# ouyangjiahong/representation-disentanglement

Hardware: AMD Instinct MI355X
Metric: MR slices/sec (train step, recon+adv+latent losses) (higher is better)
Workload: dtype f32

## Files before the change

include/mrdis.h:

```cpp
#ifndef MRDIS_H
#define MRDIS_H

#include <stddef.h>
#include <stdint.h>

#ifdef __cplusplus
extern "C" {
#endif

#define MRDIS_OK            0
#define MRDIS_EINVAL       -1
#define MRDIS_EUNSUPPORTED -2
#define MRDIS_EWORKSPACE   -3
#define MRDIS_ELAUNCH      -4
#define MRDIS_EALIGN       -5

#define MRDIS_MAX_TAPS 16

#define MRDIS_EPI_NONE   0
#define MRDIS_EPI_LRELU  1

const char* mrdis_strerror(int code);
int mrdis_version(void);

// ... 177 lines not shown
int mrdis_synth_finish(float* acc, const int* cnt, float* out, int D, int H, int W, float fill, void* stream);

#define MRDIS_SEG2D_MAX_SETS 16
#define MRDIS_SEG2D_MAX_VIEWS 2
int mrdis_seg2d_label_planes(const float* const* views, int n_sets, int n_views, const int* flips, unsigned char* planes, int B, int C, int H,
                             int W, int D, int s0, int relabel, void* stream);
int mrdis_seg2d_finish(const unsigned char* planes, unsigned char* out, int n_sets, int D, int H, int W, void* stream);

#define MRDIS_FUSE_MAX_SRC 8
#define MRDIS_FUSE_MEAN 0
#define MRDIS_FUSE_MAX 1
#define MRDIS_FUSE_MEAN_MAX_MIN 2
int mrdis_fuse_present_fwd(const float* const* srcs, const int* ld_srcs, int K, const float* mask, int method, float* out, int ldo, int B,
                           long long HW, int C, void* stream);
int mrdis_fuse_present_bwd(const float* dout, int lddo, const float* const* srcs, const int* ld_srcs, int K, const float* mask, int method,
                           float* const* dsrcs, const int* ld_dsrcs, int B, long long HW, int C, void* stream);

#define MRDIS_EDT_FAR (1 << 30)
#define MRDIS_EDT_MAX_SRC 8
#define MRDIS_SURF_MAX_REGIONS 4
int mrdis_region_surfaces(const unsigned char* labels, const void* targets, const int* region_masks, int R, unsigned char* flags, int* counts,
                          int B, int H, int W, int D, void* stream);
size_t mrdis_edt_workspace(int S, int B, int H, int W, int D);
int mrdis_edt_sq(const unsigned char* src, const unsigned char* src_masks, int S, int* out, void* workspace, size_t workspace_bytes, int B,
                 int H, int W, int D, void* stream);
int mrdis_surface_hist(const unsigned char* flags, int R, int* hist, long long bins, void* workspace, size_t workspace_bytes, int B, int H,
                       int W, int D, void* stream);

int mrdis_cc_label(const unsigned char* labels, int fg_mask, int connectivity, int* comp, int* size, int B, int H, int W, int D, void* stream);
size_t mrdis_cc_clean_workspace(int B);
int mrdis_cc_clean(const unsigned char* labels, const int* comp, const int* size, int min_voxels, int keep_largest, int et_label,
                   int et_min_voxels, int et_replace, unsigned char* out, int* stats, void* workspace, size_t workspace_bytes, int B, int H,
                   int W, int D, void* stream);

#define MRDIS_DILATE_MAX_ITERATIONS 8
int mrdis_region_planes(const unsigned char* labels, const void* targets, const int* region_masks, int R, unsigned char* planes, int B, int H,
                        int W, int D, void* stream);
size_t mrdis_dilate_workspace(int iterations, int B, int H, int W, int D);
int mrdis_dilate(const unsigned char* src, unsigned char* dst, int connectivity, int iterations, void* workspace, size_t workspace_bytes, int B,
                 int H, int W, int D, void* stream);
int mrdis_lesion_match(const unsigned char* planes, const int* comp_l, const int* rank_l, const int* comp_p, const int* rank_p,
                       const int* first_p, int words, int n_lesions, int* bits, int* tcount, int* root, int* item, int B, int R, int H, int W,
                       int D, void* stream);
int mrdis_lesion_expand(const unsigned char* planes, const int* comp_l, const int* rank_l, const int* comp_p, const int* rank_p,
                        const int* first_p, const int* bits, int words, const int* item, int n_lesions, int j0, int n, unsigned char* stack_s,
                        unsigned char* stack_t, int B, int R, int H, int W, int D, void* stream);

int mrdis_maxpool_fwd(const float* x, int ldx, float* y, int32_t* argmax, int N, int H, int W, int C,
                      int k, void* stream);
int mrdis_maxpool_bwd(const float* dy, const int32_t* argmax, float* dx, int lddx, int N, int H, int W,
                      int C, int k, void* stream);

size_t mrdis_sumsq_workspace(void);
int mrdis_sumsq_finite(const float* g, long long n, float* out, void* workspace, size_t workspace_bytes,
                       void* stream);
int mrdis_adam_amsgrad_step(float* p, const float* g, float* m, float* v, float* vmax,
                            long long n, float lr, float beta1, float beta2, float eps,
                            float weight_decay, int step_count, float* step_state, const float* norm_finite,
                            float max_norm, float grad_scale, const long long* gate_ranges, const int* gate_flag_index,
                            int n_gates, const float* gate_flags, float* gate_steps, int n_flags, void* stream);


int mrdis_conv3d_fwd(const float* x, int ldx, const float* w_tck, const float* bias, const float* residual, int ldres,
                     float* y, int ldy, int N, int D, int H, int W, int Ci, int Co,
                     int k, int stride, int pad, void* stream);
int mrdis_conv3d_bwd_data(const float* dy, int lddy, const float* w_tkc, float* dx, int lddx,
                          int N, int D, int H, int W, int Ci, int Co, int k, int stride, int pad, void* stream);
size_t mrdis_conv3d_bwd_weight_workspace(int N, int D, int H, int W, int Ci, int Co, int k, int stride, int pad);
int mrdis_conv3d_bwd_weight(const float* x, int ldx, const float* dy, int lddy, float* dw_tck, float* dbias,
                            void* workspace, size_t workspace_bytes,
                            int N, int D, int H, int W, int Ci, int Co, int k, int stride, int pad, void* stream);

size_t mrdis_groupnorm_workspace(int N, long long P, int C, int G);
int mrdis_groupnorm_relu_fwd(const float* x, int ldx, float* y, int ldy, const float* gamma, const float* beta,
                             float* save_mean, float* save_rstd, void* workspace, size_t workspace_bytes,
                             int N, long long P, int C, int G, float eps, int relu, void* stream);
int mrdis_groupnorm_relu_bwd(const float* dy, int lddy, const float* x, int ldx, const float* gamma, const float* beta,
                             const float* save_mean, const float* save_rstd, float* dx, int lddx,
                             float* dgamma, float* dbeta, void* workspace, size_t workspace_bytes,
                             int N, long long P, int C, int G, int relu, void* stream);
int mrdis_groupnorm_relu_bwd_add(const float* dy, int lddy, const float* x, int ldx, const float* gamma, const float* beta,
                                 const float* save_mean, const float* save_rstd, float* dx, int lddx,
                                 float* dgamma, float* dbeta, const float* add, int ldadd, void* workspace, size_t workspace_bytes,
                                 int N, long long P, int C, int G, int relu, void* stream);

int mrdis_upsample2x_add_fwd(const float* x, const float* skip, float* y, int N, int D, int H, int W, int C, void* stream);
int mrdis_upsample2x_bwd(const float* dy, float* dx, int N, int D, int H, int W, int C, void* stream);

size_t mrdis_cosine_top1_workspace(int N, int D, int Q);
int mrdis_cosine_top1(const float* gallery, long long ldg, const int* gallery_label, int N, int D,
                      const float* query, const int* query_label, int Q,
                      int* out_idx, float* out_cos, void* workspace, size_t workspace_bytes, void* stream);

int mrdis_conv2d_2src_fwd(const float* x, int ldx, int Cx, const float* s, int lds, int Cs, const float* w_tck, const float* bias,
                          float* y, int ldy, int N, int H, int W, int Co, int kh, int kw, int stride, int pad, int lrelu, void* stream);
int mrdis_conv2d_2src_bwd_data(const float* dy, int lddy, const float* w_tkc, float* dx, int lddx, int Cx, float* ds, int ldds, int Cs,
                               int N, int H, int W, int Co, int kh, int kw, int stride, int pad, void* stream);
size_t mrdis_conv2d_2src_bwd_weight_workspace(int N, int H, int W, int Cx, int Cs, int Co, int kh, int kw, int stride, int pad);
int mrdis_conv2d_2src_bwd_weight(const float* x, int ldx, int Cx, const float* s, int lds, int Cs, const float* dy, int lddy,
                                 float* dw_tck, float* dbias, int accumulate_bias, void* workspace, size_t workspace_bytes,
                                 int N, int H, int W, int Co, int kh, int kw, int stride, int pad, void* stream);
int mrdis_softplus_fwd(const float* x, int ldx, float* y, int ldy, long long P, int C, void* stream);
int mrdis_softplus_bwd(const float* dy, int lddy, const float* x, int ldx, float* dx, int lddx, long long P, int C, void* stream);
int mrdis_softmax_fwd(const float* s, int lds, float* out, int ldo, long long P, int C, void* stream);
int mrdis_softmax_bwd(const float* dout, int lddo, const float* out, int ldo, float* ds, int ldds, long long P, int C, void* stream);

#define MRDIS_KL_MAXM 8
int mrdis_kl_fwd(const float* const* mu, const float* const* lv, int ldmu, int ldlv, const float* pmu, const float* plv, long long ldp_m,
                 int ldp_b, const float* weight, float* loss, int M, int B, int Z, void* stream);
int mrdis_kl_bwd(const float* dloss, const float* const* mu, const float* const* lv, int ldmu, int ldlv, const float* pmu, const float* plv,
                 long long ldp_m, int ldp_b, const float* weight, float* const* dmu, float* const* dlv, int lddmu, int lddlv,
                 float* dpmu, float* dplv, int M, int B, int Z, void* stream);
int mrdis_avgpool_fwd(const float* x, int ldx, float* y, int N, int H, int W, int C, int k, void* stream);
int mrdis_avgpool_bwd(const float* dy, float* dx, int lddx, int N, int H, int W, int C, int k, void* stream);

size_t mrdis_chatt_workspace(int B, long long HW, int C, int Hd);
int mrdis_chatt_fwd(const float* x, int ldx, const float* s, int lds, const float* wd, const float* bd, const float* wu, const float* bu,
                    float* out, int ldo, float* pool, float* hid, float* a, void* ws, size_t ws_bytes, int B, long long HW, int C, int Hd,
                    void* stream);
int mrdis_chatt_bwd(const float* dy, int lddy, const float* x, int ldx, const float* a, const float* hid, const float* pool,
                    const float* wd, const float* wu, float* dx, int lddx, float* dwd, float* dbd, float* dwu, float* dbu,
                    void* ws, size_t ws_bytes, int B, long long HW, int C, int Hd, void* stream);
int mrdis_symdiff_fwd(const float* g, int ldg, float* gd, int ldo, int B, int H, int W, int C, void* stream);
int mrdis_symdiff_bwd(const float* dgd, int lddgd, const float* g, int ldg, float* dg, int lddg, int B, int H, int W, int C, void* stream);
int mrdis_rgate_fwd(const float* x, int ldx, const float* alpha, float* out, int ldo, int B, int H, int W, int C, void* stream);
int mrdis_rgate_bwd(const float* dy, int lddy, const float* x, int ldx, const float* alpha, float* dx, int lddx, float* rsum,
                    int B, int H, int W, int C, void* stream);

#define MRDIS_PREP_U8 2
#define MRDIS_PREP_I16 4
#define MRDIS_PREP_I32 8
#define MRDIS_PREP_F32 16
#define MRDIS_PREP_F64 64
#define MRDIS_PREP_U16 512
#define MRDIS_PREP_ZSCORE 0
#define MRDIS_PREP_MEAN 1
#define MRDIS_PREP_LABEL 2
#define MRDIS_PREP_DHW 0
#define MRDIS_PREP_HWD 1
size_t mrdis_prep_workspace(int H, int W, int D);
int mrdis_prep_stats(const void* raw, int dtype, long long stride_h, long long stride_w, long long stride_d, int H, int W, int D,
                     int h0, int h1, int w0, int w1, int d_lo, int d_hi, double slope, double inter, double* stats,
                     void* workspace, size_t workspace_bytes, void* stream);
int mrdis_prep_write(const void* raw, int dtype, long long stride_h, long long stride_w, long long stride_d, int H, int W, int D,
                     int h0, int h1, int w0, int w1, double slope, double inter, const double* stats, int kind, int layout,
                     float* out, void* stream);

#define MRDIS_EXPORT_COPY 0
#define MRDIS_EXPORT_UNZSCORE 1
#define MRDIS_EXPORT_UNMEAN 2
int mrdis_export_volume(const void* src, int src_dtype, int layout, int Hc, int Wc, int D, int h0, int h1, int w0, int w1, int B,
                        int kind, const double* stats, double fill, void* dst, int dst_dtype, void* stream);

#ifdef __cplusplus
}
#endif
#endif
```

representation-disentanglement_amd/__init__.py:

```python
from . import hip, ops, model, model3d, trainer
from .hip import MrdisError, MrdisLibraryError, LIB_PATH
from .model import (CondConv2d, Conv2d, HipConv2d, BatchNorm2d, Conv_BN_Act_New,
                    Act_Deconv_BN_Concat_New, AnatomyEncoderEncNew, AnatomyEncoderDecNew,
                    ModalityEncoderNew, SPADEBlockNew, SPADENewShared, SPADENewNotShared, SPADENew,
                    Discriminator, MultimodalModel, expand_type)
from .trainer import (TrainStep, GraphedTrainStep, make_train_step, regular_mask, EvalStep, ZGallery, build_z_gallery, nn_source_contrast, ArenaAdam, GradAllReduce, DEFAULT_CONFIG, load_config_yaml,
                      derive_config, build_model, synthetic_batch, fit_to_model, forward_losses,
                      save_checkpoint, load_checkpoint_model, LOSS_KEYS)

from .model3d import BasicBlock, VAEBranch, UNet3D, NVNet3D, HipConv3d, nvnet_loss, nvnet_loss_hip, seg_metrics, seg_metrics_from_counts, window_offsets, predict_volumes
from .data import VolumeStore, SliceDataset, BatchLoader, load_idx_list
from .data3d import VolumeStore3D, VolumeDataset3D, VolumeLoader3D, VolumeData3D, load_subj_list
from . import patch3d
from .patch3d import fg_block_counts, fg_prefix, patch_origins, patch_gather, patch_warp, warp_matrix
from .synth import synthesize_volumes, synth_plan, synth_source, synth_targets, SYNTH_BLOCKS
from . import synth
from . import segment
from .segment import segment_volumes, seg_patterns
from . import surfdist
from .surfdist import EDT_FAR, BRATS_REGIONS, edt3d_sq, region_scores, scores_from_counts, percentile_ranks, region_masks
from . import postproc
from .postproc import components3d, clean_labels
from . import lesion
from .lesion import dilate3d, lesion_scores, lesion_scores_from_rows
from . import prep
from .prep import read_nifti, prep_stats, prep_write, prep_volume, build_store_from_raw, write_fold_lists, write_nifti, save_nifti, export_store_volume
from . import train
from . import train3d
from .train3d import Run3D

__version__ = '0.1.0'
```

representation-disentanglement_amd/csrc/mrdis_c16.hip:

```cpp
#include "mrdis_common.h"

struct C16Params {
    const float* x; const float* w; const float* bias; float* y;
    int N, H, W, Ci, ldx, ldy, lrelu;
    int tilesY, tilesX, ntiles;
    unsigned x_bytes;
};

namespace {
constexpr int C16_TH = 8, C16_TW = 32, C16_RW = C16_TW + 2, C16_NPX = (C16_TH + 2) * C16_RW;
constexpr unsigned C16_OOB = 0xfffffff0u;
}

template <int HALVES>
__global__ __launch_bounds__(256, 2) void conv3x3_c16_kernel(const C16Params p) {
    constexpr int CI = 16 * HALVES, PP = CI + 4, Q = CI / 4;
    constexpr int XR = (C16_NPX * Q + 255) / 256;
    constexpr int NG = 9 * HALVES;
    extern __shared__ __attribute__((aligned(16))) float smem[];
    const int tid = threadIdx.x, lane = tid & 63, wave = tid >> 6, l16 = lane & 15, kq = lane >> 4;

    float a[NG][4];
#pragma unroll
    for (int g = 0; g < NG; ++g)
#pragma unroll
        for (int j = 0; j < 4; ++j) a[g][j] = p.w[((g / HALVES) * CI + 16 * (g % HALVES) + 4 * kq + j) * 16 + l16];
    const float4 bv = p.bias ? make_float4(p.bias[4 * kq], p.bias[4 * kq + 1], p.bias[4 * kq + 2], p.bias[4 * kq + 3])
                              : make_float4(0.f, 0.f, 0.f, 0.f);

    const __amdgpu_buffer_rsrc_t rs_x = mrdis_buffer_rsrc(p.x, p.x_bytes);
    int s_l[XR], s_ry[XR], s_rx[XR], s_q[XR];
#pragma unroll
    for (int it = 0; it < XR; ++it) {
        const int idx = tid + 256 * it, pi = idx / Q;
        s_q[it] = 4 * (idx - pi * Q);
        s_ry[it] = pi / C16_RW; s_rx[it] = pi - s_ry[it] * C16_RW;
        s_l[it] = idx < C16_NPX * Q ? pi * PP + s_q[it] : -1;
    }
    u32x4 xr[XR];
    auto load_tile = [&](int tile) {
        const bool on = tile < p.ntiles;
        int t = tile;
        const int tx = t % p.tilesX; t /= p.tilesX;
        const int ty = t % p.tilesY;
        const int n = t / p.tilesY;
#pragma unroll
        for (int it = 0; it < XR; ++it) {
            const int h = ty * C16_TH - 1 + s_ry[it], w_ = tx * C16_TW - 1 + s_rx[it];
            const bool ok = on && s_l[it] >= 0 && (unsigned)h < (unsigned)p.H && (unsigned)w_ < (unsigned)p.W;
            xr[it] = __builtin_amdgcn_raw_buffer_load_b128(rs_x, (int)(ok ? 4u * (unsigned)(((n * p.H + h) * p.W + w_) * p.ldx + s_q[it]) : C16_OOB), 0, 0);
        }
    };
    auto store_tile = [&]() {
#pragma unroll
        for (int it = 0; it < XR; ++it)
            if (s_l[it] >= 0) *reinterpret_cast<u32x4*>(smem + s_l[it]) = xr[it];
    };

    int boff[4];
#pragma unroll
    for (int t = 0; t < 4; ++t) boff[t] = ((2 * wave + (t >> 1)) * C16_RW + 16 * (t & 1) + l16) * PP + 4 * kq;

    int tile = mrdis_xcd_remap((int)blockIdx.x, (int)gridDim.x);
    load_tile(tile);
    store_tile();
    __syncthreads();
    for (; tile < p.ntiles; tile += gridDim.x) {
        load_tile(tile + gridDim.x);
        f32x4 acc[4];
#pragma unroll
        for (int t = 0; t < 4; ++t) acc[t] = f32x4{0.f, 0.f, 0.f, 0.f};
        float4 b[2][4];
#pragma unroll
        for (int t = 0; t < 4; ++t) b[0][t] = *reinterpret_cast<const float4*>(smem + boff[t]);
#pragma unroll
        for (int g = 0; g < NG; ++g) {
            if (g + 1 < NG) {
                const int tap = (g + 1) / HALVES, h = (g + 1) % HALVES;
                const int go = ((tap / 3) * C16_RW + (tap % 3)) * PP + 16 * h;
#pragma unroll
                for (int t = 0; t < 4; ++t) b[(g + 1) & 1][t] = *reinterpret_cast<const float4*>(smem + boff[t] + go);
            }
#pragma unroll
            for (int t = 0; t < 4; ++t) {
                const float4 v = b[g & 1][t];
                acc[t] = __builtin_amdgcn_mfma_f32_16x16x4f32(a[g][0], v.x, acc[t], 0, 0, 0);
            }
#pragma unroll
            for (int t = 0; t < 4; ++t) acc[t] = __builtin_amdgcn_mfma_f32_16x16x4f32(a[g][1], b[g & 1][t].y, acc[t], 0, 0, 0);
#pragma unroll
            for (int t = 0; t < 4; ++t) acc[t] = __builtin_amdgcn_mfma_f32_16x16x4f32(a[g][2], b[g & 1][t].z, acc[t], 0, 0, 0);
#pragma unroll
            for (int t = 0; t < 4; ++t) acc[t] = __builtin_amdgcn_mfma_f32_16x16x4f32(a[g][3], b[g & 1][t].w, acc[t], 0, 0, 0);
            __builtin_amdgcn_sched_barrier(0);
        }
        {
            int t_ = tile;
            const int tx = t_ % p.tilesX; t_ /= p.tilesX;
            const int ty = t_ % p.tilesY;
            const int n = t_ / p.tilesY;
#pragma unroll
            for (int t = 0; t < 4; ++t) {
                const int oy = ty * C16_TH + 2 * wave + (t >> 1), ox = tx * C16_TW + 16 * (t & 1) + l16;
                float4 o = make_float4(acc[t][0] + bv.x, acc[t][1] + bv.y, acc[t][2] + bv.z, acc[t][3] + bv.w);
                if (p.lrelu) { o.x = o.x > 0.f ? o.x : 0.2f * o.x; o.y = o.y > 0.f ? o.y : 0.2f * o.y; o.z = o.z > 0.f ? o.z : 0.2f * o.z; o.w = o.w > 0.f ? o.w : 0.2f * o.w; }
                if (oy < p.H && ox < p.W) *reinterpret_cast<float4*>(p.y + ((long long)(n * p.H + oy) * p.W + ox) * p.ldy + 4 * kq) = o;
            }
        }
        __syncthreads();
        store_tile();
        __syncthreads();
    }
}

__global__ __launch_bounds__(256, 2) void conv3x3_c16_split6_kernel(const C16Params p) {
    constexpr int CI = 32, Q = CI / 4, PB = 208;
    constexpr int XR = (C16_NPX * Q + 255) / 256;
    extern __shared__ __attribute__((aligned(16))) unsigned char smem_b[];
    const int tid = threadIdx.x, lane = tid & 63, wave = tid >> 6, l16 = lane & 15, kq = lane >> 4;

    bf16x8 a[9][3];
#pragma unroll
    for (int g = 0; g < 9; ++g)
#pragma unroll
        for (int j = 0; j < 8; ++j) {
            const float v = p.w[(g * CI + 8 * kq + j) * 16 + l16];
            mrdis_split3(v, a[g][0], a[g][1], a[g][2], j);
        }
    const float4 bv = p.bias ? make_float4(p.bias[4 * kq], p.bias[4 * kq + 1], p.bias[4 * kq + 2], p.bias[4 * kq + 3]) : make_float4(0.f, 0.f, 0.f, 0.f);

    const __amdgpu_buffer_rsrc_t rs_x = mrdis_buffer_rsrc(p.x, p.x_bytes);
    int s_l[XR], s_ry[XR], s_rx[XR], s_q[XR];
#pragma unroll
    for (int it = 0; it < XR; ++it) {
        const int idx = tid + 256 * it, pi = idx / Q;
        s_q[it] = 4 * (idx - pi * Q);
        s_ry[it] = pi / C16_RW; s_rx[it] = pi - s_ry[it] * C16_RW;
        s_l[it] = idx < C16_NPX * Q ? pi * PB + 2 * s_q[it] : -1;
    }
    u32x4 xr[XR];
    auto load_tile = [&](int tile) {
        const bool on = tile < p.ntiles;
        int t = tile;
        const int tx = t % p.tilesX; t /= p.tilesX;
        const int ty = t % p.tilesY;
        const int n = t / p.tilesY;
#pragma unroll
        for (int it = 0; it < XR; ++it) {
            const int h = ty * C16_TH - 1 + s_ry[it], w_ = tx * C16_TW - 1 + s_rx[it];
            const bool ok = on && s_l[it] >= 0 && (unsigned)h < (unsigned)p.H && (unsigned)w_ < (unsigned)p.W;
            xr[it] = __builtin_amdgcn_raw_buffer_load_b128(rs_x, (int)(ok ? 4u * (unsigned)(((n * p.H + h) * p.W + w_) * p.ldx + s_q[it]) : C16_OOB), 0, 0);
        }
    };
    auto store_tile = [&]() {
#pragma unroll
        for (int it = 0; it < XR; ++it) {
            if (s_l[it] < 0) continue;
            const float xv[4] = {__uint_as_float(xr[it].x), __uint_as_float(xr[it].y), __uint_as_float(xr[it].z), __uint_as_float(xr[it].w)};
            bf16x4 hi, mid, lo; mrdis_split3(xv, hi, mid, lo);
            *reinterpret_cast<bf16x4*>(smem_b + s_l[it]) = hi;
            *reinterpret_cast<bf16x4*>(smem_b + s_l[it] + 64) = mid;
            *reinterpret_cast<bf16x4*>(smem_b + s_l[it] + 128) = lo;
        }
    };

    int boff[4];
#pragma unroll
    for (int t = 0; t < 4; ++t) boff[t] = ((2 * wave + (t >> 1)) * C16_RW + 16 * (t & 1) + l16) * PB + 16 * kq;

    int tile = mrdis_xcd_remap((int)blockIdx.x, (int)gridDim.x);
    load_tile(tile);
    store_tile();
    __syncthreads();
    for (; tile < p.ntiles; tile += gridDim.x) {
        load_tile(tile + gridDim.x);
        f32x4 acc[4];
#pragma unroll
        for (int t = 0; t < 4; ++t) acc[t] = f32x4{0.f, 0.f, 0.f, 0.f};
#pragma unroll
        for (int g = 0; g < 9; ++g) {
            const int go = ((g / 3) * C16_RW + (g % 3)) * PB;
            bf16x8 xh[4], xm[4], xl[4];
#pragma unroll
            for (int t = 0; t < 4; ++t) {
                xh[t] = *reinterpret_cast<const bf16x8*>(smem_b + boff[t] + go);
                xm[t] = *reinterpret_cast<const bf16x8*>(smem_b + boff[t] + go + 64);
                xl[t] = *reinterpret_cast<const bf16x8*>(smem_b + boff[t] + go + 128);
            }
#pragma unroll
            for (int t = 0; t < 4; ++t) acc[t] = __builtin_amdgcn_mfma_f32_16x16x32_bf16(a[g][1], xm[t], acc[t], 0, 0, 0);
#pragma unroll
            for (int t = 0; t < 4; ++t) acc[t] = __builtin_amdgcn_mfma_f32_16x16x32_bf16(a[g][0], xl[t], acc[t], 0, 0, 0);
#pragma unroll
            for (int t = 0; t < 4; ++t) acc[t] = __builtin_amdgcn_mfma_f32_16x16x32_bf16(a[g][2], xh[t], acc[t], 0, 0, 0);
#pragma unroll
            for (int t = 0; t < 4; ++t) acc[t] = __builtin_amdgcn_mfma_f32_16x16x32_bf16(a[g][0], xm[t], acc[t], 0, 0, 0);
#pragma unroll
            for (int t = 0; t < 4; ++t) acc[t] = __builtin_amdgcn_mfma_f32_16x16x32_bf16(a[g][1], xh[t], acc[t], 0, 0, 0);
#pragma unroll
            for (int t = 0; t < 4; ++t) acc[t] = __builtin_amdgcn_mfma_f32_16x16x32_bf16(a[g][0], xh[t], acc[t], 0, 0, 0);
        }
        {
            int t_ = tile;
            const int tx = t_ % p.tilesX; t_ /= p.tilesX;
            const int ty = t_ % p.tilesY;
            const int n = t_ / p.tilesY;
#pragma unroll
            for (int t = 0; t < 4; ++t) {
                const int oy = ty * C16_TH + 2 * wave + (t >> 1), ox = tx * C16_TW + 16 * (t & 1) + l16;
                float4 o = make_float4(acc[t][0] + bv.x, acc[t][1] + bv.y, acc[t][2] + bv.z, acc[t][3] + bv.w);
                if (p.lrelu) { o.x = o.x > 0.f ? o.x : 0.2f * o.x; o.y = o.y > 0.f ? o.y : 0.2f * o.y; o.z = o.z > 0.f ? o.z : 0.2f * o.z; o.w = o.w > 0.f ? o.w : 0.2f * o.w; }
                if (oy < p.H && ox < p.W) *reinterpret_cast<float4*>(p.y + ((long long)(n * p.H + oy) * p.W + ox) * p.ldy + 4 * kq) = o;
            }
        }
        __syncthreads();
        store_tile();
        __syncthreads();
    }
}

__global__ __launch_bounds__(256, 2) void conv3x3_c16t_split6_kernel(const C16Params p) {
    constexpr int CI = 16, Q = CI / 4, PB = 112;
    constexpr int XR = (C16_NPX * Q + 255) / 256;
    extern __shared__ __attribute__((aligned(16))) unsigned char smem_t[];
    const int tid = threadIdx.x, lane = tid & 63, wave = tid >> 6, e = lane & 31, half = lane >> 5;

    bf16x8 a[9][3];
#pragma unroll
    for (int g = 0; g < 9; ++g)
#pragma unroll
        for (int j = 0; j < 8; ++j) {
            const int gf = p.lrelu ? 8 - g : g;
            const float v = p.w[(gf * CI + 8 * half + j) * 32 + e];
            mrdis_split3(v, a[g][0], a[g][1], a[g][2], j);
        }
    const __amdgpu_buffer_rsrc_t rs_x = mrdis_buffer_rsrc(p.x, p.x_bytes);
    int s_l[XR], s_ry[XR], s_rx[XR], s_q[XR];
#pragma unroll
    for (int it = 0; it < XR; ++it) {
        const int idx = tid + 256 * it, pi = idx / Q;
        s_q[it] = 4 * (idx - pi * Q);
        s_ry[it] = pi / C16_RW; s_rx[it] = pi - s_ry[it] * C16_RW;
        s_l[it] = idx < C16_NPX * Q ? pi * PB + 2 * s_q[it] : -1;
    }
    u32x4 xr[XR];
    auto load_tile = [&](int tile) {
        const bool on = tile < p.ntiles;
        int t = tile;
        const int tx = t % p.tilesX; t /= p.tilesX;
        const int ty = t % p.tilesY;
        const int n = t / p.tilesY;
#pragma unroll
        for (int it = 0; it < XR; ++it) {
            const int h = ty * C16_TH - 1 + s_ry[it], w_ = tx * C16_TW - 1 + s_rx[it];
            const bool ok = on && s_l[it] >= 0 && (unsigned)h < (unsigned)p.H && (unsigned)w_ < (unsigned)p.W;
            xr[it] = __builtin_amdgcn_raw_buffer_load_b128(rs_x, (int)(ok ? 4u * (unsigned)(((n * p.H + h) * p.W + w_) * p.ldx + s_q[it]) : C16_OOB), 0, 0);
        }
    };
    auto store_tile = [&]() {
#pragma unroll
        for (int it = 0; it < XR; ++it) {
            if (s_l[it] < 0) continue;
            const float xv[4] = {__uint_as_float(xr[it].x), __uint_as_float(xr[it].y), __uint_as_float(xr[it].z), __uint_as_float(xr[it].w)};
            bf16x4 hi, mid, lo; mrdis_split3(xv, hi, mid, lo);
            *reinterpret_cast<bf16x4*>(smem_t + s_l[it]) = hi;
            *reinterpret_cast<bf16x4*>(smem_t + s_l[it] + 32) = mid;
            *reinterpret_cast<bf16x4*>(smem_t + s_l[it] + 64) = lo;
        }
    };
    int boff[2];
#pragma unroll
    for (int t = 0; t < 2; ++t) boff[t] = ((2 * wave + t) * C16_RW + e) * PB + 16 * half;

    int tile = mrdis_xcd_remap((int)blockIdx.x, (int)gridDim.x);
    load_tile(tile);
    store_tile();
    __syncthreads();
    for (; tile < p.ntiles; tile += gridDim.x) {
        load_tile(tile + gridDim.x);
        f32x16 acc[2];
#pragma unroll
        for (int t = 0; t < 2; ++t)
#pragma unroll
            for (int r = 0; r < 16; ++r) acc[t][r] = 0.f;
#pragma unroll
        for (int g = 0; g < 9; ++g) {
            const int go = ((g / 3) * C16_RW + (g % 3)) * PB;
            bf16x8 xh[2], xm[2], xl[2];
#pragma unroll
            for (int t = 0; t < 2; ++t) {
                xh[t] = *reinterpret_cast<const bf16x8*>(smem_t + boff[t] + go);
                xm[t] = *reinterpret_cast<const bf16x8*>(smem_t + boff[t] + go + 32);
                xl[t] = *reinterpret_cast<const bf16x8*>(smem_t + boff[t] + go + 64);
            }
#pragma unroll
            for (int t = 0; t < 2; ++t) acc[t] = __builtin_amdgcn_mfma_f32_32x32x16_bf16(a[g][1], xm[t], acc[t], 0, 0, 0);
#pragma unroll
            for (int t = 0; t < 2; ++t) acc[t] = __builtin_amdgcn_mfma_f32_32x32x16_bf16(a[g][0], xl[t], acc[t], 0, 0, 0);
#pragma unroll
            for (int t = 0; t < 2; ++t) acc[t] = __builtin_amdgcn_mfma_f32_32x32x16_bf16(a[g][2], xh[t], acc[t], 0, 0, 0);
#pragma unroll
            for (int t = 0; t < 2; ++t) acc[t] = __builtin_amdgcn_mfma_f32_32x32x16_bf16(a[g][0], xm[t], acc[t], 0, 0, 0);
#pragma unroll
            for (int t = 0; t < 2; ++t) acc[t] = __builtin_amdgcn_mfma_f32_32x32x16_bf16(a[g][1], xh[t], acc[t], 0, 0, 0);
#pragma unroll
            for (int t = 0; t < 2; ++t) acc[t] = __builtin_amdgcn_mfma_f32_32x32x16_bf16(a[g][0], xh[t], acc[t], 0, 0, 0);
        }
        {
            int t_ = tile;
            const int tx = t_ % p.tilesX; t_ /= p.tilesX;
            const int ty = t_ % p.tilesY;
            const int n = t_ / p.tilesY;
#pragma unroll
            for (int t = 0; t < 2; ++t) {
                const int oy = ty * C16_TH + 2 * wave + t, ox = tx * C16_TW + e;
                if (oy < p.H && ox < p.W) {
                    float* dst = p.y + ((long long)(n * p.H + oy) * p.W + ox) * p.ldy + 4 * half;
#pragma unroll
                    for (int g4 = 0; g4 < 4; ++g4)
                        *reinterpret_cast<float4*>(dst + 8 * g4) = make_float4(acc[t][4 * g4], acc[t][4 * g4 + 1], acc[t][4 * g4 + 2], acc[t][4 * g4 + 3]);
                }
            }
        }
        __syncthreads();
        store_tile();
        __syncthreads();
    }
}

int mrdis_run_c16t_split6(const float* x, int ldx, const float* w_t_ci_co, float* y, int ldy, int N, int H, int W, int flip, hipStream_t s) {
    if (ldx % 4 != 0 || ldy % 4 != 0 || ((((uintptr_t)x) | ((uintptr_t)y)) & 15) != 0) return MRDIS_EUNSUPPORTED;
    if ((long long)N * H * W < 65536 || mrdis_opt(MRDIS_OPT_NOW16)) return MRDIS_EUNSUPPORTED;
    if (mrdis_opt(MRDIS_OPT_SPLIT6) != 7) return MRDIS_EUNSUPPORTED;
    const long long xb = 4LL * (((long long)N * H * W - 1) * ldx + 16);
    if (xb >= 0x7fffffffLL) return MRDIS_EUNSUPPORTED;
    C16Params p{};
    p.x = x; p.w = w_t_ci_co; p.bias = nullptr; p.y = y; p.N = N; p.H = H; p.W = W; p.Ci = 16; p.ldx = ldx; p.ldy = ldy; p.lrelu = flip;
    p.tilesY = mrdis_cdiv(H, C16_TH); p.tilesX = mrdis_cdiv(W, C16_TW);
    const long long nt = (long long)N * p.tilesY * p.tilesX;
    if (nt > 0x7fffffffLL) return MRDIS_EUNSUPPORTED;
    p.ntiles = (int)nt; p.x_bytes = (unsigned)xb;
    const int grid = p.ntiles < 512 ? p.ntiles : 512;
    MRDIS_LAUNCH(conv3x3_c16t_split6_kernel, dim3(grid), dim3(256), (size_t)C16_NPX * 112, s, p);
    MRDIS_CHECK_LAUNCH();
    return MRDIS_OK;
}

int mrdis_run_c16(const float* x, int ldx, const float* w_tck, const float* bias, float* y, int ldy, int N, int H, int W, int Ci, int Co,
                  int lrelu, hipStream_t s) {
    if (Co != 16 || (Ci != 16 && Ci != 32) || ldx % 4 != 0 || ldy % 4 != 0) return MRDIS_EUNSUPPORTED;
    if (((((uintptr_t)x) | ((uintptr_t)y)) & 15) != 0) return MRDIS_EUNSUPPORTED;
    if ((long long)N * H * W < 65536 || mrdis_opt(MRDIS_OPT_NOW16)) return MRDIS_EUNSUPPORTED;
    const long long xb = 4LL * (((long long)N * H * W - 1) * ldx + Ci);
    if (xb >= 0x7fffffffLL) return MRDIS_EUNSUPPORTED;
    C16Params p{};
    p.x = x; p.w = w_tck; p.bias = bias; p.y = y; p.N = N; p.H = H; p.W = W; p.Ci = Ci; p.ldx = ldx; p.ldy = ldy; p.lrelu = lrelu;
    p.tilesY = mrdis_cdiv(H, C16_TH); p.tilesX = mrdis_cdiv(W, C16_TW);
    const long long nt = (long long)N * p.tilesY * p.tilesX;
    if (nt > 0x7fffffffLL) return MRDIS_EUNSUPPORTED;
    p.ntiles = (int)nt; p.x_bytes = (unsigned)xb;
    const int grid = p.ntiles < 512 ? p.ntiles : 512;
    const size_t lds = sizeof(float) * (size_t)C16_NPX * (Ci + 4);
    if (Ci == 32 && (mrdis_opt(MRDIS_OPT_SPLIT6) == 1 || mrdis_opt(MRDIS_OPT_SPLIT6) == 5)) {
        if (!mrdis_lds_optin((const void*)conv3x3_c16_split6_kernel, 72 * 1024)) return MRDIS_ELAUNCH;
        mrdis_count(MRDIS_CNT_SPLIT6_C16);
        MRDIS_LAUNCH(conv3x3_c16_split6_kernel, dim3(grid), dim3(256), (size_t)C16_NPX * 208, s, p);
    } else
    if (Ci == 32) MRDIS_LAUNCH((conv3x3_c16_kernel<2>), dim3(grid), dim3(256), lds, s, p);
    else MRDIS_LAUNCH((conv3x3_c16_kernel<1>), dim3(grid), dim3(256), lds, s, p);
    MRDIS_CHECK_LAUNCH();
    return MRDIS_OK;
}
```

representation-disentanglement_amd/csrc/mrdis_common.h:

```cpp
#pragma once
#include <hip/hip_runtime.h>
#include <stdint.h>
#include "../../include/mrdis.h"
#include "mrdis_device.h"
#include "mrdis_launchers.h"

#define MRDIS_CHECK_LAUNCH()                                     \
    do {                                                         \
        hipError_t e_ = hipGetLastError();                       \
        if (e_ != hipSuccess) return MRDIS_ELAUNCH;              \
    } while (0)

#define MRDIS_OPTIONS(X) \
    X(WINO, "wino", "MRDIS_WINO", 0, 1)  \
    X(NT_MB, "nt_mb", "MRDIS_NT_MB", 0, 128)  \
    X(WINO_PIPE, "wino_pipe", "MRDIS_WINO_PIPE", 0, 1)  \
    X(WINO_U, "wino_u", "MRDIS_WINO_U", 0, 1)  \
    X(WINO4, "wino4", "MRDIS_WINO4", 0, 1)  \
    X(WINO4R, "wino4r", "MRDIS_WINO4R", 0, 1)  \
    X(BCONV4, "bconv4", "MRDIS_BCONV4", 0, 1)  \
    X(SPLIT6, "split6", "MRDIS_SPLIT6", 0, 1)  \
    X(NO16, "debug_no16", "MRDIS_DEBUG_NO16", 1, 0) \
    X(NOTHIN, "debug_nothin", "MRDIS_DEBUG_NOTHIN", 1, 0) \
    X(NOC4, "debug_noc4", "MRDIS_DEBUG_NOC4", 1, 0) \
    X(NODMA, "debug_nodma", "MRDIS_DEBUG_NODMA", 1, 0) \
    X(NO16_3D, "debug_no16_3d", "MRDIS_DEBUG_NO16_3D", 1, 0) \
    X(BILGEN, "debug_bilgen", "MRDIS_DEBUG_BILGEN", 1, 0) \
    X(NOW16, "debug_now16", "MRDIS_DEBUG_NOW16", 1, 0) \
    X(NOPACK, "debug_nopack", "MRDIS_DEBUG_NOPACK", 1, 0)  \
    X(MODE, "debug_mode", "MRDIS_DEBUG_MODE", 0, -1) \
    X(BN, "debug_bn", "MRDIS_DEBUG_BN", 0, -1) \
    X(KC, "debug_kc", "MRDIS_DEBUG_KC", 0, -1) \
    X(BM, "debug_bm", "MRDIS_DEBUG_BM", 0, -1) \
    X(C4_TW, "debug_c4_tw", "MRDIS_DEBUG_C4_TW", 0, -1) \
    X(WGSPLIT, "debug_wgsplit", "MRDIS_DEBUG_WGSPLIT", 0, -1) \
    X(BN3, "debug_bn3", "MRDIS_DEBUG_BN3", 0, -1) \
    X(KC3, "debug_kc3", "MRDIS_DEBUG_KC3", 0, -1) \
    X(C4_GRID, "c4_grid", "MRDIS_C4_GRID", 0, 0)  \
    X(C4_BLOCKS, "debug_c4_blocks", "MRDIS_DEBUG_C4_BLOCKS", 0, -1)  \
    X(ZS_GRID, "zsearch_grid", "MRDIS_ZSEARCH_GRID", 0, 0)  \
    X(VOLGEN, "debug_volgen", "MRDIS_DEBUG_VOLGEN", 1, 0)
#define MRDIS_X_OPT_ID(id, name, env, is_flag, dflt) MRDIS_OPT_##id,
enum { MRDIS_OPTIONS(MRDIS_X_OPT_ID) MRDIS_OPT_COUNT };
long long mrdis_opt(int id);
void mrdis_opt_note(int id, long long value);

#define MRDIS_COUNTERS(X) \
    X(WINO, "wino") X(WINO_SPADE, "wino_spade") X(WINO2, "wino2") X(WINO2_SPADE, "wino2_spade") X(WINO4, "wino4") X(WINO4_SPADE, "wino4_spade") X(WINO4N, "wino4n") \
    X(WINO4R, "wino4r") X(WINO_WGRAD, "wino_wgrad") X(WINO_WGRAD2, "wino_wgrad2") X(WINO4_WGRAD, "wino4_wgrad") X(BCONV3, "bconv3") X(BCONV3_SPADE, "bconv3_spade") \
    X(BCONV4, "bconv4") X(BCONV4_SPADE, "bconv4_spade") X(SPLIT6_C4, "split6_c4") X(SPLIT6_C16, "split6_c16") X(SPLIT6_WGRAD16, "split6_wgrad16") X(SPLIT6_CO4, "split6_co4") \
    X(SPLIT6_C3D, "split6_c3d") X(SPLIT6_W3D, "split6_w3d") X(SPLIT6_TAP, "split6_tap") X(ZSEARCH, "zsearch") \
    X(CONV2SRC, "conv2src") X(ANA_ACT, "ana_act")  \
    X(KL, "kl") X(AVGPOOL, "avgpool")  \
    X(CHATT, "chatt") X(SYMDIFF, "symdiff") X(RGATE, "rgate")  \
    X(DIRECT3D, "direct3d") X(C3D16, "c3d16") X(WGRAD3D, "wgrad3d") X(WGRAD3D16, "wgrad3d16") X(WINO_WGRAD3D, "wino_wgrad3d")  \
    X(VOLGATHER, "volgather")  \
    X(FGCOUNT, "fgcount") X(PATCHORIGIN, "patchorigin") X(PATCHGATHER, "patchgather")  \
    X(PATCHWARP, "patchwarp")  \
    X(LOSS3D, "loss3d") X(SEGCOUNTS, "segcounts")  \
    X(SEGACCUM, "segaccum") X(SEGLABELS, "seglabels")  \
    X(SYNTHACCUM, "synthaccum") X(SYNTHFINISH, "synthfinish")  \
    X(SEG2DLABELS, "seg2dlabels") X(SEG2DFINISH, "seg2dfinish")  \
    X(FUSE, "fuse")  \
    X(REGSURF, "regsurf") X(EDT, "edt") X(SURFHIST, "surfhist")  \
    X(CCLABEL, "cclabel") X(CCCLEAN, "ccclean")  \
    X(PREPSTATS, "prepstats") X(PREPWRITE, "prepwrite")  \
    X(EXPORT, "export")  \
    X(DILATE, "dilate") X(LESMATCH, "lesmatch") X(LESEXPAND, "lesexpand")  \
    X(STAT_VEC, "stat_vec") X(STAT_SCALAR, "stat_scalar") X(STAT_INTERP, "stat_interp")  \
    X(SPADE_UP2_ONEPASS, "spade_up2_onepass") X(SPADE_UP2_TWOPASS, "spade_up2_twopass")  \
    X(BIL_FWD_X2, "bil_fwd_x2") X(BIL_FWD_GENERAL, "bil_fwd_general")  \
    X(BIL_BWD_X2, "bil_bwd_x2") X(BIL_BWD_TIGHT3, "bil_bwd_tight3") X(BIL_BWD_TIGHT5, "bil_bwd_tight5") X(BIL_BWD_GENERAL, "bil_bwd_general")  \
    X(ELEM_V1, "elem_v1")  \
    X(ALL, "all")
#define MRDIS_X_CNT_ID(id, name) MRDIS_CNT_##id,
enum { MRDIS_COUNTERS(MRDIS_X_CNT_ID) MRDIS_CNT_COUNT };
void mrdis_count(int id);

void mrdis_note_lds(const char* kernel_expr, size_t bytes);
#define MRDIS_LAUNCH(kernel, grid, block, lds, s, ...) do { mrdis_count(MRDIS_CNT_ALL); if ((size_t)(lds) != 0) mrdis_note_lds(#kernel, (size_t)(lds)); hipLaunchKernelGGL(kernel, grid, block, lds, s, __VA_ARGS__); } while (0)

int mrdis_cu_count();
bool mrdis_lds_optin(const void* kernel, int bytes);
int mrdis_occupancy(const void* kernel, int block, size_t lds);

static inline int mrdis_cdiv(long long a, long long b) { return (int)((a + b - 1) / b); }

__device__ __forceinline__ int mrdis_xcd_remap(int bid, int nblk) {
    const int q = nblk >> 3, r = nblk & 7, xcd = bid & 7;
    const int base = (xcd < r) ? xcd * (q + 1) : r * (q + 1) + (xcd - r) * q;
    return base + (bid >> 3);
}

__device__ __forceinline__ float mrdis_wave_sum(float v) {
#pragma unroll
    for (int o = 32; o > 0; o >>= 1) v += __shfl_down(v, o, 64);
    return v;
}
__device__ __forceinline__ double mrdis_wave_sum_d(double v) {
#pragma unroll
    for (int o = 32; o > 0; o >>= 1) v += __shfl_down(v, o, 64);
    return v;
}
```

representation-disentanglement_amd/csrc/mrdis_launchers.h:

```cpp
#pragma once
#include <hip/hip_runtime.h>
#include <stddef.h>

int mrdis_run_wino(const float* x, int ldx, const float* w, const float* bias, float* y, int ldy,
                   int N, int H, int W, int Ci, int Co, int flip, int lrelu, hipStream_t s);
int mrdis_run_wino3d(const float* x, int ldx, const float* w, const float* bias, const float* res, int ldres, float* y, int ldy,
                     int N, int D, int H, int W, int Ci, int Co, int flip, hipStream_t s);
size_t mrdis_wino_wgrad_workspace(int N, int H, int W, int Ci, int Co);
int mrdis_run_wino_wgrad(const float* x, int ldx, const float* dy, int lddy, float* dw_tck, float* dbias, void* workspace,
                         size_t workspace_bytes, int N, int H, int W, int Ci, int Co, int accumulate_bias, hipStream_t s);
size_t mrdis_wino_wgrad3d_workspace(int N, int D, int H, int W, int Ci, int Co);
int mrdis_run_wino_wgrad3d(const float* x, int ldx, const float* dy, int lddy, float* dw_tck, float* dbias, void* workspace,
                           size_t workspace_bytes, int N, int D, int H, int W, int Ci, int Co, hipStream_t s);

int mrdis_run_wino2(const float* x, int ldx, const float* w, const float* bias, float* y, int ldy,
                    int N, int H, int W, int Ci, int Co, int flip, int lrelu, hipStream_t s, const float* u_img);
int mrdis_run_wino2_spade(const float* x, int ldx, const float* w, const float* bias, const float* z, int ldz, const float* mean, const float* rstd,
                          float* mix, int ldmix, float* gamma, int ldg, int N, int H, int W, int Ci, int C, hipStream_t s, const float* u_img);

int mrdis_run_wino4(const float* x, int ldx, const float* bias, float* y, int ldy, int N, int H, int W, int Ci, int Co, int lrelu,
                    hipStream_t s, const float* u_img);
int mrdis_run_wino4n(const float* x, int ldx, const float* bias, float* y, int ldy, int N, int H, int W, int Ci, int Co, int lrelu,
                     hipStream_t s, const float* u_img);
int mrdis_run_wino4_spade(const float* x, int ldx, const float* bias, const float* z, int ldz, const float* mean, const float* rstd,
                          float* mix, int ldmix, float* gamma, int ldg, int N, int H, int W, int Ci, int C, hipStream_t s, const float* u_img);

int mrdis_run_wino4r(const float* x, int ldx, const float* bias, float* y, int ldy, int N, int H, int W, int Ci, int Co, int lrelu,
                     hipStream_t s, const float* u_img);

size_t mrdis_bwgrad_workspace(int N, int H, int W, int Ci, int Co, int kh, int kw, int stride, int pad);
int mrdis_run_bwgrad(const void* x, int ldx, const void* dy, int lddy, float* dw_tck, float* dbias, void* workspace, size_t workspace_bytes,
                     int N, int H, int W, int Ci, int Co, int kh, int kw, int stride, int pad, int accumulate_bias, int dtype, hipStream_t s);

int mrdis_run_bconv3_spade(const void* x, int ldx, const void* w_bf16, const float* bias, const void* z, int ldz, const float* mean, const float* rstd,
                           void* mix, int ldmix, void* gamma, int ldg, int N, int H, int W, int Ci, int C, hipStream_t s);

int mrdis_run_bconv4_spade(const void* x, int ldx, const void* w_bf16, const float* bias, const void* z, int ldz, const float* mean, const float* rstd,
                           void* mix, int ldmix, void* gamma, int ldg, int N, int H, int W, int Ci, int C, hipStream_t s);

int mrdis_run_pw_fwd(const void* x, int ldx, const float* w_tck, const float* bias, float* y, int ldy, long long npix, int Ci, int Co, int lrelu, int x16_bf16, hipStream_t s);
int mrdis_run_pw_dgrad(const float* dy, int lddy, const float* w_tkc, void* dx, int lddx, long long npix, int Ci, int Co, int x16_bf16, hipStream_t s);
size_t mrdis_pw_wgrad_workspace(long long npix, int Ci, int Co, int x16_bf16);
int mrdis_run_pw_wgrad(const void* x, int ldx, const float* dy, int lddy, float* dw_tck, float* dbias, void* workspace, size_t workspace_bytes,
                       long long npix, int Ci, int Co, int accumulate_bias, int x16_bf16, hipStream_t s);

int mrdis_launch_slab_reduce(const float* slab, float* dw, int total, int Co, int nslab, const float* bslab, float* dbias, int accumulate_bias,
                             hipStream_t s);
int mrdis_run_conv_s2_fwd(const float* x, int ldx, const float* w_tck, const float* bias, float* y, int ldy, int N, int H, int W, int Ci, int Co,
                          int kh, int kw, int stride, int pad, int lrelu, hipStream_t s);
int mrdis_run_dgrad_s2(const float* dy, int lddy, const float* w_tkc, float* dx, int lddx, int N, int H, int W, int Ci, int Co,
                       int kh, int kw, int stride, int pad, hipStream_t s);
size_t mrdis_wgrad_s2_workspace(int N, int H, int W, int Ci, int Co, int kh, int kw, int stride, int pad);
int mrdis_run_wgrad_s2(const float* x, int ldx, const float* dy, int lddy, float* dw_tck, float* dbias, void* workspace, size_t workspace_bytes,
                       int N, int H, int W, int Ci, int Co, int kh, int kw, int stride, int pad, int accumulate_bias, hipStream_t s);
size_t mrdis_wgrad_c4_workspace(int N, int H, int W, int Ci, int Co);
int mrdis_run_wgrad_c4(const float* x, int ldx, const void* dy, int lddy, float* dw_tck, float* dbias, void* workspace, size_t workspace_bytes,
                       int N, int H, int W, int Ci, int Co, int accumulate_bias, int dy_bf16, hipStream_t s, int pad16 = 0);
size_t mrdis_wgrad_co4b_workspace(int N, int H, int W, int Ci, int Co);
int mrdis_run_wgrad_co4b(const void* x_bf16, int ldx, const float* dy, int lddy, float* dw_tck, float* dbias, void* workspace, size_t workspace_bytes,
                         int N, int H, int W, int Ci, int Co, int accumulate_bias, hipStream_t s, int pad16);

size_t mrdis_wgrad16_workspace(int N, int H, int W, int Ci, int Co);
int mrdis_run_wgrad16(const float* x, int ldx, const float* dy, int lddy, float* dw_tck, float* dbias, void* workspace,
                      size_t workspace_bytes, int N, int H, int W, int Ci, int Co, int accumulate_bias, hipStream_t s);
int mrdis_run_wgrad16_bf16(const void* x, int ldx, const void* dy, int lddy, float* dw_tck, float* dbias, void* workspace, size_t workspace_bytes,
                           int N, int H, int W, int Ci, int Co, int accumulate_bias, hipStream_t s);

int mrdis_run_co4(const void* x, int ldx, const float* w, const float* bias, float* y, int ldy, int N, int H, int W, int Ci, int Co, int flip, int lrelu, hipStream_t s,
                  int x_bf16 = 0, int wld = 4);

int mrdis_run_c16(const float* x, int ldx, const float* w_tck, const float* bias, float* y, int ldy, int N, int H, int W, int Ci, int Co, int lrelu, hipStream_t s);
int mrdis_run_c16t_split6(const float* x, int ldx, const float* w_t_ci_co, float* y, int ldy, int N, int H, int W, int flip, hipStream_t s);
```

representation-disentanglement_amd/csrc/mrdis_wgrad16.hip:

```cpp
#include "mrdis_common.h"
#include <stdlib.h>

struct Wgrad16Params {
    const float* x; const float* dy; float* slab; float* bias_slab;
    int N, H, W, Ci, ldx, Co, lddy;
    int tilesA, tilesB, numTiles, nCi, splits;
};

#define W16_TH 8
#define W16_TW 16
#define W16_RW (W16_TW + 2)
#define W16_NPX ((W16_TH + 2) * W16_RW)

template <int NS>
__global__ __launch_bounds__(256, 2) void wgrad16_kernel(const Wgrad16Params p) {
    constexpr int S = NS == 1 ? 16 : 48, QX = 4 * NS;
    constexpr int XR = (W16_NPX * QX + 255) / 256;
    extern __shared__ __attribute__((aligned(16))) float smem[];
    float* dys = smem;
    float* xs = smem + 2048;
    const int tid = threadIdx.x, lane = tid & 63, wave = tid >> 6, l16 = lane & 15, kq = lane >> 4;
    const int lb = mrdis_xcd_remap((int)blockIdx.x, (int)gridDim.x);
    const int ncol = p.nCi / NS;
    const int cic = lb % ncol, split = lb / ncol;
    const int c_lo = cic * 16 * NS;

    int loff[9];
#pragma unroll
    for (int t = 0; t < 9; ++t) loff[t] = ((t / 3) * W16_RW + (t % 3)) * S + l16;
    bool ci_ok[NS];
#pragma unroll
    for (int sl = 0; sl < NS; ++sl) ci_ok[sl] = (c_lo + 16 * sl + l16) < p.Ci;
    int tin[8];
#pragma unroll
    for (int g = 0; g < 8; ++g) {
        const int m = wave * 32 + g * 4 + kq;
        tin[g] = ((m / W16_TW) * W16_RW + (m % W16_TW)) * S;
    }
    int xl[XR], xc[XR];
#pragma unroll
    for (int it = 0; it < XR; ++it) {
        const int idx = tid + it * 256;
        xl[it] = -1; xc[it] = 0;
        if (idx < W16_NPX * QX) { const int pi = idx / QX, q = idx % QX; xl[it] = pi * S + 4 * q; xc[it] = ((pi / W16_RW) << 10) | (pi % W16_RW); }
    }
    const int qx = c_lo + (tid % QX) * 4;
    const bool qx_ok = qx < p.Ci;
    int yc[2];
#pragma unroll
    for (int it = 0; it < 2; ++it) { const int m = (tid + it * 256) >> 2; yc[it] = ((m / W16_TW) << 10) | (m % W16_TW); }
    const int qy = (tid & 3) * 4;
    const bool qy_ok = qy < p.Co;

    f32x4 acc[NS][9];
#pragma unroll
    for (int sl = 0; sl < NS; ++sl)
#pragma unroll
        for (int t = 0; t < 9; ++t) acc[sl][t] = f32x4{0.f, 0.f, 0.f, 0.f};
    float bsum = 0.f;
    float4 xr[XR], yr[2];
    auto load_box = [&](int box) {
        int tt = box;
        const int tb = tt % p.tilesB; tt /= p.tilesB;
        const int ta = tt % p.tilesA;
        const int n = tt / p.tilesA;
        const int a0 = ta * W16_TH, b0 = tb * W16_TW;
        const float* __restrict__ xn = p.x + (long long)n * p.H * p.W * p.ldx + qx;
#pragma unroll
        for (int it = 0; it < XR; ++it) {
            xr[it] = make_float4(0.f, 0.f, 0.f, 0.f);
            const int h = a0 - 1 + (xc[it] >> 10), w_ = b0 - 1 + (xc[it] & 1023);
            if (xl[it] >= 0 && qx_ok && (unsigned)h < (unsigned)p.H && (unsigned)w_ < (unsigned)p.W)
                xr[it] = *reinterpret_cast<const float4*>(xn + ((long long)h * p.W + w_) * p.ldx);
        }
        const float* __restrict__ dyn = p.dy + (long long)n * p.H * p.W * p.lddy + qy;
#pragma unroll
        for (int it = 0; it < 2; ++it) {
            yr[it] = make_float4(0.f, 0.f, 0.f, 0.f);
            const int a = a0 + (yc[it] >> 10), b = b0 + (yc[it] & 1023);
            if (qy_ok && a < p.H && b < p.W) yr[it] = *reinterpret_cast<const float4*>(dyn + ((long long)a * p.W + b) * p.lddy);
        }
    };
    auto store_box = [&]() {
#pragma unroll
        for (int it = 0; it < XR; ++it)
            if (xl[it] >= 0) *reinterpret_cast<float4*>(xs + xl[it]) = xr[it];
#pragma unroll
        for (int it = 0; it < 2; ++it) *reinterpret_cast<float4*>(dys + 4 * (tid + it * 256)) = yr[it];
    };

    int box = split;
    if (box < p.numTiles) load_box(box);
    store_box();
    __syncthreads();
    for (; box < p.numTiles; box += p.splits) {
        const int nxt = box + p.splits;
        if (nxt < p.numTiles) load_box(nxt);
#pragma unroll
        for (int g = 0; g < 8; ++g) {
            const float bv = dys[(wave * 32 + g * 4 + kq) * 16 + l16];
            bsum += bv;
            const float* xa = xs + tin[g];
#pragma unroll
            for (int sl = 0; sl < NS; ++sl) {
                float av[9];
#pragma unroll
                for (int t = 0; t < 9; ++t) av[t] = ci_ok[sl] ? xa[loff[t] + 16 * sl] : 0.f;
#pragma unroll
                for (int t = 0; t < 9; ++t) acc[sl][t] = __builtin_amdgcn_mfma_f32_16x16x4f32(av[t], bv, acc[sl][t], 0, 0, 0);
            }
        }
        if (nxt < p.numTiles) { __syncthreads(); store_box(); __syncthreads(); }
    }
    float* red = smem;
#pragma unroll
    for (int sl = 0; sl < NS; ++sl) {
        float* out = p.slab + (((long long)split * p.nCi + cic * NS + sl) * 9) * 256;
        __syncthreads();
#pragma unroll
        for (int t = 0; t < 9; ++t)
#pragma unroll
            for (int r = 0; r < 4; ++r) red[(wave * 9 + t) * 256 + (4 * kq + r) * 16 + l16] = acc[sl][t][r];
        __syncthreads();
        for (int i = tid; i < 9 * 256; i += 256)
            out[i] = (red[i] + red[9 * 256 + i]) + (red[2 * 9 * 256 + i] + red[3 * 9 * 256 + i]);
    }
    if (p.bias_slab != nullptr && cic == 0) {
        bsum += __shfl_xor(bsum, 16, 64);
        bsum += __shfl_xor(bsum, 32, 64);
        __syncthreads();
        if (kq == 0) red[wave * 16 + l16] = bsum;
        __syncthreads();
        if (tid < 16) p.bias_slab[(long long)split * 16 + tid] = (red[tid] + red[16 + tid]) + (red[32 + tid] + red[48 + tid]);
    }
}

struct Wgrad16SParams {
    const float* x; const float* dy; float* slab; float* bias_slab;
    int N, H, W, ldx, lddy;
    int tilesA, tilesB, numTiles, splits;
    unsigned x_bytes, dy_bytes;
};
#define W6_TH 8
#define W6_TW 32
#define W6_YW (W6_TW + 2)
#define W6_YPX ((W6_TH + 2) * W6_YW)
__global__ __launch_bounds__(256, 2) void wgrad16_split6_kernel(const Wgrad16SParams p) {
    constexpr int XPX = W6_TH * W6_TW;
    constexpr int XPLANE = XPX * 64, YPLANE = W6_YPX * 32;
    constexpr int XR = 8, YR = 6;
    constexpr unsigned OOB = 0xfffffff0u;
    extern __shared__ __attribute__((aligned(16))) unsigned char smem6[];
    unsigned char* xs = smem6;
    unsigned char* ys = smem6 + 3 * XPLANE;
    const int tid = threadIdx.x, lane = tid & 63, wave = tid >> 6, l16 = lane & 15, kq = lane >> 4;
    const int split = mrdis_xcd_remap((int)blockIdx.x, (int)gridDim.x);
    const __amdgpu_buffer_rsrc_t rs_x = mrdis_buffer_rsrc(p.x, p.x_bytes);
    const __amdgpu_buffer_rsrc_t rs_y = mrdis_buffer_rsrc(p.dy, p.dy_bytes);

    const int q4 = l16 >> 2, p4 = l16 & 3;
    const int xoff = (8 * kq + q4) * 64 + 8 * p4;
    const int yoff = (8 * kq + q4) * 32 + 8 * p4;

    f32x4 acc[9][2];
#pragma unroll
    for (int t = 0; t < 9; ++t) { acc[t][0] = f32x4{0.f, 0.f, 0.f, 0.f}; acc[t][1] = f32x4{0.f, 0.f, 0.f, 0.f}; }
    float bs4[4] = {0.f, 0.f, 0.f, 0.f};

    u32x4 xr[XR], yr[YR];
    auto load_box = [&](int box) {
        const bool on = box < p.numTiles;
        int tt = box;
        const int tb = tt % p.tilesB; tt /= p.tilesB;
        const int ta = tt % p.tilesA;
        const int n = tt / p.tilesA;
        const int a0 = ta * W6_TH, b0 = tb * W6_TW;
#pragma unroll
        for (int it = 0; it < XR; ++it) {
            const int idx = tid + 256 * it, px = idx >> 3, q = idx & 7;
            const int h = a0 + (px >> 5), w_ = b0 + (px & 31);
            const bool ok = on && h < p.H && w_ < p.W;
            xr[it] = __builtin_amdgcn_raw_buffer_load_b128(rs_x, (int)(ok ? 4u * (unsigned)(((n * p.H + h) * p.W + w_) * p.ldx + 4 * q) : OOB), 0, 0);
        }
#pragma unroll
        for (int it = 0; it < YR; ++it) {
            const int idx = tid + 256 * it, px = idx >> 2, q = idx & 3;
            const int ly = px / W6_YW, lx = px - ly * W6_YW;
            const int h = a0 - 1 + ly, w_ = b0 - 1 + lx;
            const bool ok = on && px < W6_YPX && (unsigned)h < (unsigned)p.H && (unsigned)w_ < (unsigned)p.W;
            yr[it] = __builtin_amdgcn_raw_buffer_load_b128(rs_y, (int)(ok ? 4u * (unsigned)(((n * p.H + h) * p.W + w_) * p.lddy + 4 * q) : OOB), 0, 0);
        }
    };
    auto split4 = [](const u32x4& v, bf16x4& hi, bf16x4& mid, bf16x4& lo) {
        const float f[4] = {__uint_as_float(v.x), __uint_as_float(v.y), __uint_as_float(v.z), __uint_as_float(v.w)};
        mrdis_split3(f, hi, mid, lo);
    };
    auto store_box = [&]() {
#pragma unroll
        for (int it = 0; it < XR; ++it) {
            const int idx = tid + 256 * it, px = idx >> 3, q = idx & 7;
            bf16x4 hi, mid, lo; split4(xr[it], hi, mid, lo);
            unsigned char* d = xs + px * 64 + 8 * q;
            *reinterpret_cast<bf16x4*>(d) = hi; *reinterpret_cast<bf16x4*>(d + XPLANE) = mid; *reinterpret_cast<bf16x4*>(d + 2 * XPLANE) = lo;
        }
#pragma unroll
        for (int it = 0; it < YR; ++it) {
            const int idx = tid + 256 * it, px = idx >> 2, q = idx & 3;
            if (px >= W6_YPX) continue;
            const int ly = px / W6_YW, lx = px - ly * W6_YW;
            if (ly >= 1 && ly <= W6_TH && lx >= 1 && lx <= W6_TW) {
                bs4[0] += __uint_as_float(yr[it].x); bs4[1] += __uint_as_float(yr[it].y); bs4[2] += __uint_as_float(yr[it].z); bs4[3] += __uint_as_float(yr[it].w);
            }
            bf16x4 hi, mid, lo; split4(yr[it], hi, mid, lo);
            unsigned char* d = ys + px * 32 + 8 * q;
            *reinterpret_cast<bf16x4*>(d) = hi; *reinterpret_cast<bf16x4*>(d + YPLANE) = mid; *reinterpret_cast<bf16x4*>(d + 2 * YPLANE) = lo;
        }
    };
    int box = split;
    load_box(box);
    store_box();
    __syncthreads();
    for (; box < p.numTiles; box += p.splits) {
        load_box(box + p.splits);
#pragma unroll
        for (int rr = 0; rr < 2; ++rr) {
            const int row = wave + 4 * rr;
            bf16x8 ax[2][3];
#pragma unroll
            for (int mt = 0; mt < 2; ++mt)
#pragma unroll
                for (int term = 0; term < 3; ++term) {
                    const unsigned char* a = xs + term * XPLANE + row * (32 * 64) + xoff + 32 * mt;
                    union { bf16x8 v; s16x4 h[2]; } u;
                    u.h[0] = __builtin_amdgcn_ds_read_tr16_b64_v4i16((s16x4 __attribute__((address_space(3)))*)(a));
                    u.h[1] = __builtin_amdgcn_ds_read_tr16_b64_v4i16((s16x4 __attribute__((address_space(3)))*)(a + 4 * 64));
                    ax[mt][term] = u.v;
                }
#pragma unroll
            for (int t = 0; t < 9; ++t) {
                const int ty = t / 3, tx = t % 3;
                bf16x8 by[3];
#pragma unroll
                for (int term = 0; term < 3; ++term) {
                    const unsigned char* b = ys + term * YPLANE + ((row - ty + 2) * W6_YW + 2 - tx) * 32 + yoff;
                    union { bf16x8 v; s16x4 h[2]; } u;
                    u.h[0] = __builtin_amdgcn_ds_read_tr16_b64_v4i16((s16x4 __attribute__((address_space(3)))*)(b));
                    u.h[1] = __builtin_amdgcn_ds_read_tr16_b64_v4i16((s16x4 __attribute__((address_space(3)))*)(b + 4 * 32));
                    by[term] = u.v;
                }
#pragma unroll
                for (int mt = 0; mt < 2; ++mt) {
                    acc[t][mt] = __builtin_amdgcn_mfma_f32_16x16x32_bf16(ax[mt][1], by[1], acc[t][mt], 0, 0, 0);
                    acc[t][mt] = __builtin_amdgcn_mfma_f32_16x16x32_bf16(ax[mt][2], by[0], acc[t][mt], 0, 0, 0);
                    acc[t][mt] = __builtin_amdgcn_mfma_f32_16x16x32_bf16(ax[mt][0], by[2], acc[t][mt], 0, 0, 0);
                }
#pragma unroll
                for (int mt = 0; mt < 2; ++mt) {
                    acc[t][mt] = __builtin_amdgcn_mfma_f32_16x16x32_bf16(ax[mt][1], by[0], acc[t][mt], 0, 0, 0);
                    acc[t][mt] = __builtin_amdgcn_mfma_f32_16x16x32_bf16(ax[mt][0], by[1], acc[t][mt], 0, 0, 0);
                    acc[t][mt] = __builtin_amdgcn_mfma_f32_16x16x32_bf16(ax[mt][0], by[0], acc[t][mt], 0, 0, 0);
                }
            }
        }
        __syncthreads();
        store_box();
        __syncthreads();
    }
    float* red = reinterpret_cast<float*>(smem6);
#pragma unroll
    for (int mt = 0; mt < 2; ++mt) {
        float* out = p.slab + (((long long)split * 2 + mt) * 9) * 256;
        __syncthreads();
#pragma unroll
        for (int t = 0; t < 9; ++t)
#pragma unroll
            for (int r = 0; r < 4; ++r) red[(wave * 9 + t) * 256 + (4 * kq + r) * 16 + l16] = acc[t][mt][r];
        __syncthreads();
        for (int i = tid; i < 9 * 256; i += 256)
            out[i] = (red[i] + red[9 * 256 + i]) + (red[2 * 9 * 256 + i] + red[3 * 9 * 256 + i]);
    }
    if (p.bias_slab != nullptr) {
        __syncthreads();
#pragma unroll
        for (int c = 0; c < 4; ++c) red[c * 256 + tid] = bs4[c];
        __syncthreads();
        if (tid < 16) {
            const int qd = tid >> 2, c = tid & 3;
            float t_ = 0.f;
            for (int k = qd; k < 256; k += 4) t_ += red[c * 256 + k];
            p.bias_slab[(long long)split * 16 + tid] = t_;
        }
    }
}

__global__ __launch_bounds__(256, 2) void wgrad16_bf16_kernel(const Wgrad16SParams p) {
    constexpr int XPX = W6_TH * W6_TW;
    constexpr int XR = 4, YR = 3;
    constexpr unsigned OOB = 0xfffffff0u;
    extern __shared__ __attribute__((aligned(16))) unsigned char smem7[];
    unsigned char* xs = smem7;
    unsigned char* ys = smem7 + XPX * 64;
    const int tid = threadIdx.x, lane = tid & 63, wave = tid >> 6, l16 = lane & 15, kq = lane >> 4;
    const int split = mrdis_xcd_remap((int)blockIdx.x, (int)gridDim.x);
    const __amdgpu_buffer_rsrc_t rs_x = mrdis_buffer_rsrc(p.x, p.x_bytes);
    const __amdgpu_buffer_rsrc_t rs_y = mrdis_buffer_rsrc(p.dy, p.dy_bytes);
    const int q4 = l16 >> 2, p4 = l16 & 3;
    const int xoff = (8 * kq + q4) * 64 + 8 * p4;
    const int yoff = (8 * kq + q4) * 32 + 8 * p4;

    f32x4 acc[9][2];
#pragma unroll
    for (int t = 0; t < 9; ++t) { acc[t][0] = f32x4{0.f, 0.f, 0.f, 0.f}; acc[t][1] = f32x4{0.f, 0.f, 0.f, 0.f}; }
    float bs8[8] = {0.f, 0.f, 0.f, 0.f, 0.f, 0.f, 0.f, 0.f};

    u32x4 xr[XR], yr[YR];
    auto load_box = [&](int box) {
        const bool on = box < p.numTiles;
        int tt = box;
        const int tb = tt % p.tilesB; tt /= p.tilesB;
        const int ta = tt % p.tilesA;
        const int n = tt / p.tilesA;
        const int a0 = ta * W6_TH, b0 = tb * W6_TW;
#pragma unroll
        for (int it = 0; it < XR; ++it) {
            const int idx = tid + 256 * it, px = idx >> 2, q = idx & 3;
            const int h = a0 + (px >> 5), w_ = b0 + (px & 31);
            const bool ok = on && h < p.H && w_ < p.W;
            xr[it] = __builtin_amdgcn_raw_buffer_load_b128(rs_x, (int)(ok ? 2u * (unsigned)(((n * p.H + h) * p.W + w_) * p.ldx + 8 * q) : OOB), 0, 0);
        }
#pragma unroll
        for (int it = 0; it < YR; ++it) {
            const int idx = tid + 256 * it, px = idx >> 1, q = idx & 1;
            const int ly = px / W6_YW, lx = px - ly * W6_YW;
            const int h = a0 - 1 + ly, w_ = b0 - 1 + lx;
            const bool ok = on && px < W6_YPX && (unsigned)h < (unsigned)p.H && (unsigned)w_ < (unsigned)p.W;
            yr[it] = __builtin_amdgcn_raw_buffer_load_b128(rs_y, (int)(ok ? 2u * (unsigned)(((n * p.H + h) * p.W + w_) * p.lddy + 8 * q) : OOB), 0, 0);
        }
    };
    auto store_box = [&]() {
#pragma unroll
        for (int it = 0; it < XR; ++it) {
            const int idx = tid + 256 * it, px = idx >> 2, q = idx & 3;
            *reinterpret_cast<u32x4*>(xs + px * 64 + 16 * q) = xr[it];
        }
#pragma unroll
        for (int it = 0; it < YR; ++it) {
            const int idx = tid + 256 * it, px = idx >> 1, q = idx & 1;
            if (px >= W6_YPX) continue;
            const int ly = px / W6_YW, lx = px - ly * W6_YW;
            if (ly >= 1 && ly <= W6_TH && lx >= 1 && lx <= W6_TW) {
                const unsigned u[4] = {yr[it].x, yr[it].y, yr[it].z, yr[it].w};
#pragma unroll
                for (int k = 0; k < 4; ++k) { bs8[2 * k] += __uint_as_float(u[k] << 16); bs8[2 * k + 1] += __uint_as_float(u[k] & 0xffff0000u); }
            }
            *reinterpret_cast<u32x4*>(ys + px * 32 + 16 * q) = yr[it];
        }
    };

    int box = split;
    load_box(box);
    store_box();
    __syncthreads();
    for (; box < p.numTiles; box += p.splits) {
        load_box(box + p.splits);
#pragma unroll
        for (int rr = 0; rr < 2; ++rr) {
            const int row = wave + 4 * rr;
            bf16x8 ax[2];
#pragma unroll
            for (int mt = 0; mt < 2; ++mt) {
                const unsigned char* a = xs + row * (32 * 64) + xoff + 32 * mt;
                union { bf16x8 v; s16x4 h[2]; } u;
                u.h[0] = __builtin_amdgcn_ds_read_tr16_b64_v4i16((s16x4 __attribute__((address_space(3)))*)(a));
                u.h[1] = __builtin_amdgcn_ds_read_tr16_b64_v4i16((s16x4 __attribute__((address_space(3)))*)(a + 4 * 64));
                ax[mt] = u.v;
            }
#pragma unroll
            for (int t = 0; t < 9; ++t) {
                const int ty = t / 3, tx = t % 3;
                const unsigned char* b = ys + ((row - ty + 2) * W6_YW + 2 - tx) * 32 + yoff;
                union { bf16x8 v; s16x4 h[2]; } u;
                u.h[0] = __builtin_amdgcn_ds_read_tr16_b64_v4i16((s16x4 __attribute__((address_space(3)))*)(b));
                u.h[1] = __builtin_amdgcn_ds_read_tr16_b64_v4i16((s16x4 __attribute__((address_space(3)))*)(b + 4 * 32));
                acc[t][0] = __builtin_amdgcn_mfma_f32_16x16x32_bf16(ax[0], u.v, acc[t][0], 0, 0, 0);
                acc[t][1] = __builtin_amdgcn_mfma_f32_16x16x32_bf16(ax[1], u.v, acc[t][1], 0, 0, 0);
            }
        }
        __syncthreads();
        store_box();
        __syncthreads();
    }
    float* red = reinterpret_cast<float*>(smem7);
#pragma unroll
    for (int mt = 0; mt < 2; ++mt) {
        float* out = p.slab + (((long long)split * 2 + mt) * 9) * 256;
        __syncthreads();
#pragma unroll
        for (int t = 0; t < 9; ++t)
#pragma unroll
            for (int r = 0; r < 4; ++r) red[(wave * 9 + t) * 256 + (4 * kq + r) * 16 + l16] = acc[t][mt][r];
        __syncthreads();
        for (int i = tid; i < 9 * 256; i += 256)
            out[i] = (red[i] + red[9 * 256 + i]) + (red[2 * 9 * 256 + i] + red[3 * 9 * 256 + i]);
    }
    if (p.bias_slab != nullptr) {
        __syncthreads();
#pragma unroll
        for (int c = 0; c < 8; ++c) red[c * 256 + tid] = bs8[c];
        __syncthreads();
        if (tid < 16) {
            const int hf = tid >> 3, c = tid & 7;
            float t_ = 0.f;
            for (int k = hf; k < 256; k += 2) t_ += red[c * 256 + k];
            p.bias_slab[(long long)split * 16 + tid] = t_;
        }
    }
}

__global__ void wgrad16_reduce_kernel(const float* __restrict__ slab, float* __restrict__ dw, int Ci, int Co, int nCi, int nslab,
                                      const float* __restrict__ bslab, float* __restrict__ dbias, int accumulate_bias) {
    __shared__ float red[16][65];
    const int total = 9 * Ci * Co;
    const int nout = total + (dbias != nullptr ? Co : 0);
    const int i = blockIdx.x * 64 + threadIdx.x;
    const int SL = blockDim.y, y = threadIdx.y;
    float s_ = 0.f;
    if (i < total) {
        const int co = i % Co;
        const int r = i / Co;
        const int ci = r % Ci, t = r / Ci;
        const long long stride = (long long)nCi * 9 * 256;
        const float* src = slab + ((long long)(ci >> 4) * 9 + t) * 256 + (ci & 15) * 16 + co + (long long)y * stride;
        for (int k = y; k < nslab; k += SL, src += (long long)SL * stride) s_ += *src;
    } else if (i < nout) {
        const int co = i - total;
        for (int k = y; k < nslab; k += SL) s_ += bslab[(long long)k * 16 + co];
    }
    red[y][threadIdx.x] = s_;
    __syncthreads();
    if (y == 0 && i < nout) {
        float t = 0.f;
        for (int k = 0; k < SL; ++k) t += red[k][threadIdx.x];
        if (i < total) dw[i] = t;
        else { const int co = i - total; dbias[co] = accumulate_bias ? dbias[co] + t : t; }
    }
}

static bool plan_wgrad16(Wgrad16Params& p, int N, int H, int W, int Ci, int Co) {
    if (Co > 16 || Co <= 4 || Co % 4 != 0 || Ci % 16 != 0) return false;
    if ((long long)N * H * W < 100000 || mrdis_opt(MRDIS_OPT_NOW16)) return false;
    p = Wgrad16Params{};
    p.N = N; p.H = H; p.W = W; p.Ci = Ci; p.Co = Co;
    p.tilesA = mrdis_cdiv(H, W16_TH); p.tilesB = mrdis_cdiv(W, W16_TW);
    const long long nt = (long long)N * p.tilesA * p.tilesB;
    if (nt > 0x7fffffffLL) return false;
    p.numTiles = (int)nt;
    p.nCi = Ci / 16;
    int splits = 1024 / p.nCi;
    if (splits > p.numTiles) splits = p.numTiles;
    if (splits < 1) splits = 1;
    p.splits = splits;
    return true;
}

size_t mrdis_wgrad16_workspace(int N, int H, int W, int Ci, int Co) {
    Wgrad16Params p;
    if (!plan_wgrad16(p, N, H, W, Ci, Co)) return 0;
    return sizeof(float) * ((size_t)p.splits * p.nCi * 9 * 256 + (size_t)p.splits * 16) + 256;
}

int mrdis_run_wgrad16(const float* x, int ldx, const float* dy, int lddy, float* dw_tck, float* dbias, void* workspace,
                      size_t workspace_bytes, int N, int H, int W, int Ci, int Co, int accumulate_bias, hipStream_t s) {
    Wgrad16Params p;
    if (!plan_wgrad16(p, N, H, W, Ci, Co)) return MRDIS_EUNSUPPORTED;
    if (ldx % 4 != 0 || lddy % 4 != 0 || ((((uintptr_t)x) | ((uintptr_t)dy)) & 15) != 0) return MRDIS_EUNSUPPORTED;
    if (workspace_bytes + 256 < mrdis_wgrad16_workspace(N, H, W, Ci, Co)) return MRDIS_EUNSUPPORTED;
    p.x = x; p.dy = dy; p.ldx = ldx; p.lddy = lddy;
    p.slab = reinterpret_cast<float*>(workspace);
    p.bias_slab = dbias ? p.slab + (size_t)p.splits * p.nCi * 9 * 256 : nullptr;
    if (Ci == 32 && Co == 16 && (mrdis_opt(MRDIS_OPT_SPLIT6) == 1 || mrdis_opt(MRDIS_OPT_SPLIT6) == 6)) {
        const long long xb = 4LL * (((long long)N * H * W - 1) * ldx + Ci), yb = 4LL * (((long long)N * H * W - 1) * lddy + Co);
        if (xb < 0x7fffffffLL && yb < 0x7fffffffLL) {
            Wgrad16SParams q{};
            q.x = x; q.dy = dy; q.slab = p.slab; q.bias_slab = p.bias_slab; q.N = N; q.H = H; q.W = W; q.ldx = ldx; q.lddy = lddy;
            q.tilesA = mrdis_cdiv(H, W6_TH); q.tilesB = mrdis_cdiv(W, W6_TW);
            const long long nt6 = (long long)N * q.tilesA * q.tilesB;
            q.numTiles = (int)nt6; q.splits = p.splits < q.numTiles ? p.splits : q.numTiles;
            q.x_bytes = (unsigned)xb; q.dy_bytes = (unsigned)yb;
            const size_t lds6 = 3 * (size_t)(W6_TH * W6_TW * 64) + 3 * (size_t)(W6_YPX * 32);
            if (!mrdis_lds_optin((const void*)wgrad16_split6_kernel, 96 * 1024)) return MRDIS_ELAUNCH;
            mrdis_count(MRDIS_CNT_SPLIT6_WGRAD16);
            MRDIS_LAUNCH(wgrad16_split6_kernel, dim3(q.splits), dim3(256), lds6, s, q);
            MRDIS_CHECK_LAUNCH();
            const long long nout6 = 9LL * Ci * Co + (dbias ? Co : 0);
            int SL6 = 1;
            while (SL6 < 16 && SL6 * 8 <= q.splits) SL6 <<= 1;
            MRDIS_LAUNCH(wgrad16_reduce_kernel, dim3(mrdis_cdiv(nout6, 64)), dim3(64, SL6), 0, s, p.slab, dw_tck, Ci, Co, 2, q.splits, p.bias_slab, dbias, accumulate_bias);
            MRDIS_CHECK_LAUNCH();
            return MRDIS_OK;
        }
    }
    const size_t lds = sizeof(float) * (size_t)(4 * 9 * 256);
    MRDIS_LAUNCH(wgrad16_kernel<1>, dim3(p.splits * p.nCi), dim3(256), lds, s, p);
    MRDIS_CHECK_LAUNCH();
    const long long nout = 9LL * Ci * Co + (dbias ? Co : 0);
    int SL = 1;
    while (SL < 16 && SL * 8 <= p.splits) SL <<= 1;
    MRDIS_LAUNCH(wgrad16_reduce_kernel, dim3(mrdis_cdiv(nout, 64)), dim3(64, SL), 0, s, p.slab, dw_tck, Ci, Co, p.nCi, p.splits,
                       p.bias_slab, dbias, accumulate_bias);
    MRDIS_CHECK_LAUNCH();
    return MRDIS_OK;
}

int mrdis_run_wgrad16_bf16(const void* x, int ldx, const void* dy, int lddy, float* dw_tck, float* dbias, void* workspace, size_t workspace_bytes,
                           int N, int H, int W, int Ci, int Co, int accumulate_bias, hipStream_t s) {
    Wgrad16Params p;
    if (Ci != 32 || Co != 16 || !plan_wgrad16(p, N, H, W, Ci, Co) || mrdis_opt(MRDIS_OPT_MODE) == 3030) return MRDIS_EUNSUPPORTED;
    if (ldx % 8 != 0 || lddy % 8 != 0 || ((((uintptr_t)x) | ((uintptr_t)dy)) & 15) != 0) return MRDIS_EUNSUPPORTED;
    if (workspace_bytes + 256 < mrdis_wgrad16_workspace(N, H, W, Ci, Co)) return MRDIS_EUNSUPPORTED;
    const long long xb = 2LL * (((long long)N * H * W - 1) * ldx + Ci), yb = 2LL * (((long long)N * H * W - 1) * lddy + Co);
    if (xb >= 0x7fffffffLL || yb >= 0x7fffffffLL) return MRDIS_EUNSUPPORTED;
    Wgrad16SParams q{};
    q.x = reinterpret_cast<const float*>(x); q.dy = reinterpret_cast<const float*>(dy);
    q.slab = reinterpret_cast<float*>(workspace); q.bias_slab = dbias ? q.slab + (size_t)p.splits * p.nCi * 9 * 256 : nullptr;
    q.N = N; q.H = H; q.W = W; q.ldx = ldx; q.lddy = lddy;
    q.tilesA = mrdis_cdiv(H, W6_TH); q.tilesB = mrdis_cdiv(W, W6_TW);
    const long long nt = (long long)N * q.tilesA * q.tilesB;
    q.numTiles = (int)nt; q.splits = p.splits < q.numTiles ? p.splits : q.numTiles;
    q.x_bytes = (unsigned)xb; q.dy_bytes = (unsigned)yb;
    size_t lds = (size_t)(W6_TH * W6_TW * 64) + (size_t)(W6_YPX * 32);
    const size_t red = sizeof(float) * (size_t)(4 * 9 * 256);
    if (lds < red) lds = red;
    MRDIS_LAUNCH(wgrad16_bf16_kernel, dim3(q.splits), dim3(256), lds, s, q);
    MRDIS_CHECK_LAUNCH();
    const long long nout = 9LL * Ci * Co + (dbias ? Co : 0);
    int SL = 1;
    while (SL < 16 && SL * 8 <= q.splits) SL <<= 1;
    MRDIS_LAUNCH(wgrad16_reduce_kernel, dim3(mrdis_cdiv(nout, 64)), dim3(64, SL), 0, s, q.slab, dw_tck, Ci, Co, 2, q.splits, q.bias_slab, dbias, accumulate_bias);
    MRDIS_CHECK_LAUNCH();
    return MRDIS_OK;
}
```

representation-disentanglement_amd/hip.py:

```python
import collections
import ctypes
import os

import torch

_HERE = os.path.dirname(os.path.abspath(__file__))
LIB_PATH = os.path.join(_HERE, 'csrc', 'libmrdis_hip.so')


class MrdisLibraryError(RuntimeError):
    pass


class MrdisError(RuntimeError):
    pass


_lib = None
_c = ctypes
_P, _I, _L, _F, _Z = _c.c_void_p, _c.c_int, _c.c_longlong, _c.c_float, _c.c_size_t

_SIGS = {
    'mrdis_strerror': (_c.c_char_p, [_I]),
    'mrdis_version': (_I, []),
    'mrdis_set_option': (_I, [_c.c_char_p, _L]),
    'mrdis_get_option': (_L, [_c.c_char_p]),
    'mrdis_launch_count': (_L, [_c.c_char_p]),
    'mrdis_launch_count_reset': (None, []),
    'mrdis_dynamic_lds_table': (_I, [_c.c_char_p, _I]),
    'mrdis_mix_experts_fwd': (_I, [_P, _P, _P, _P, _I, _I, _I, _I, _P]),
    'mrdis_mix_experts_bwd_workspace': (_Z, [_I, _I, _I, _I]),
    'mrdis_mix_experts_bwd': (_I, [_P, _P, _P, _P, _P, _P, _Z, _I, _I, _I, _I, _P]),
    'mrdis_mix_experts_routed_fwd': (_I, [_P, _P, _P, _P, _I, _P, _P, _P, _I, _I, _I, _I, _P]),
    'mrdis_mix_experts_routed_bwd': (_I, [_P, _P, _P, _P, _I, _P, _P, _P, _P, _Z, _I, _I, _I, _I, _P]),
    'mrdis_copy_bytes': (_I, [_P, _P, _L, _P]),
    'mrdis_stream_fill': (_I, [_P, _L, _F, _P]),
    'mrdis_instnorm_stats': (_I, [_P, _I, _P, _P, _P, _Z, _I, _L, _I, _F, _I, _P]),
    'mrdis_conv2d_fwd_spade': (_I, [_P, _I, _P, _P, _P, _P, _I, _P, _P, _P, _I, _P, _I, _I, _I, _I, _I, _I, _I, _P, _I, _P]),
    'mrdis_wino_u_job_bytes': (_Z, []),
    'mrdis_wino_u_format': (_I, [_I, _I, _I]),
    'mrdis_wino_u_image_floats': (_L, [_I, _I, _I]),
    'mrdis_s6_filter_image_bytes': (ctypes.c_size_t, [_I, _I, _I]),
    'mrdis_s6_filter_image': (_I, [_P, _I, _I, _I, _P, ctypes.c_size_t, _P]),
    'mrdis_wino_u_image_floats_fmt': (_L, [_I, _I, _I, _I]),
    'mrdis_wino_u_job_blocks': (_I, [_I, _I, _I]),
    'mrdis_wino_u_jobs': (_I, [_P, _I, _I, _P]),
    'mrdis_mix_experts_routed_multi_fwd': (_I, [_P, _P, _P, _P, _I, _I, _P, _P, _P, _P, _P, _I, _L, _I, _I, _I, _I, _P]),
    'mrdis_mix_experts_routed_multi_bwd_workspace': (_Z, [_I, _I, _I, _I, _I]),
    'mrdis_mix_experts_routed_multi_bwd': (_I, [_P, _P, _P, _P, _I, _I, _P, _P, _P, _I, _I, _P, _Z, _I, _I, _I, _I, _P]),
    'mrdis_mix_job_bytes': (_Z, []),
    'mrdis_mix_job_blocks': (_I, [_I, _I, _I]),
    'mrdis_mix_jobs_fwd': (_I, [_P, _I, _I, _P, _I, _I, _P]),
    'mrdis_mix_jobs_bwd': (_I, [_P, _I, _I, _P, _P, _I, _I, _P]),
    'mrdis_conv2d_fwd': (_I, [_P, _I, _P, _P, _P, _P, _I] + [_I] * 11 + [_P, _I, _P]),
    'mrdis_conv2d_bwd_data': (_I, [_P, _I, _P, _P, _P, _I] + [_I] * 10 + [_P, _I, _P]),
    'mrdis_cast_bf16': (_I, [_P, _P, _L, _P]),
    'mrdis_cast_view': (_I, [_P, _I, _I, _I, _P, _I, _I, _I, _L, _P]),
    'mrdis_conv2d_bwd_weight_workspace': (_Z, [_I] * 9),
    'mrdis_conv2d_bwd_weight': (_I, [_P, _I, _P, _I, _P, _P, _P, _Z] + [_I] * 11 + [_P]),
    'mrdis_lrelu_bwd': (_I, [_P, _I, _P, _I, _P, _I, _L, _I, _F, _I, _P]),
    'mrdis_norm_workspace': (_Z, [_I, _L, _I]),
    'mrdis_bn_train_fwd': (_I, [_P, _I, _P, _I, _P, _P, _P, _P, _P, _P, _P, _Z, _L, _I, _F, _F, _I, _I, _P]),
    'mrdis_bn_eval_fwd': (_I, [_P, _I, _P, _I, _P, _P, _P, _P, _L, _I, _F, _I, _P]),
    'mrdis_bn_train_bwd': (_I, [_P, _I, _P, _I, _P, _P, _P, _P, _I, _P, _P, _P, _P, _P, _Z, _L, _I, _I, _I, _P]),
    'mrdis_instnorm_spade_fwd': (_I, [_P, _I, _P, _I, _P, _I, _P, _I, _P, _P, _P, _Z, _I, _L, _I, _F, _I, _P]),
    'mrdis_instnorm_spade_bwd_workspace': (_Z, [_I, _L, _I]),
    'mrdis_instnorm_spade_bwd': (_I, [_P, _I, _P, _I, _P, _I, _P, _P, _P, _I, _P, _I, _P, _I, _P, _Z, _I, _L, _I, _I, _P]),
    'mrdis_instnorm_spade_bwd_up2_workspace': (_Z, [_I, _I, _I, _I, _I]),
    'mrdis_instnorm_spade_bwd_up2': (_I, [_P, _I, _P, _I, _P, _I, _P, _P, _P, _I, _P, _I, _P, _I, _P, _Z, _I, _I, _I, _I, _P, _I, _I, _P]),
    'mrdis_bilinear_fwd': (_I, [_P, _I, _P, _I] + [_I] * 8 + [_P]),
    'mrdis_bilinear_bwd': (_I, [_P, _I, _P, _I] + [_I] * 8 + [_P]),
    'mrdis_bilinear_up2_stats_workspace': (_Z, [_I, _I, _I]),
    'mrdis_bilinear_up2_stats_applies': (_I, [_I, _I, _I]),
    'mrdis_bilinear_up2_stats_fwd': (_I, [_P, _I, _P, _I, _I, _I, _I, _I, _I, _L, _P, _P, _F, _P, _Z, _I, _P]),
    'mrdis_softmax_mask_drop_fwd': (_I, [_P, _I, _P, _P, _I, _L, _I, _F, _P]),
    'mrdis_softmax_mask_drop_bwd': (_I, [_P, _I, _P, _I, _P, _I, _L, _I, _P]),
    'mrdis_recon_err_workspace': (_Z, [_I, _L, _I]),
    'mrdis_recon_err_fwd': (_I, [_P, _I, _P, _I, _P, _P, _Z, _I, _L, _I, _I, _P]),
    'mrdis_recon_err_bwd': (_I, [_P, _I, _P, _I, _P, _P, _I, _I, _L, _I, _I, _P]),
    'mrdis_recon_metrics_workspace': (_Z, [_I, _I]),
    'mrdis_recon_metrics': (_I, [_P, _I, _P, _I, _P, _P, _Z, _I, _I, _I, _P]),
    'mrdis_slice_gather': (_I, [_P, _P, _P, _P, _I, _P, _P, _I, _I, _I, _I, _I, _I, _P]),
    'mrdis_volume_gather': (_I, [_P, _I, _P, _P, _I, _I, _I, _I, _I, _I, _I, _I, _I, _I, _P]),
    'mrdis_fg_block_counts': (_I, [_P, _P, _I, _P, _I, _I, _I, _P]),
    'mrdis_patch_origins': (_I, [_P, _I, _P, _P, _I] + [_I] * 8 + [_P]),
    'mrdis_patch_gather': (_I, [_P, _I, _P, _P, _P] + [_I] * 11 + [_P]),
    'mrdis_patch_warp': (_I, [_P, _I, _P, _P, _P] + [_I] * 11 + [_P]),
    'mrdis_nvnet_loss_workspace': (_Z, [_L, _L]),
    'mrdis_nvnet_loss_fwd': (_I, [_P, _P, _P, _P, _P, _I, _P, _P, _P, _P, _P, _I, _c.c_double, _P, _P, _P, _Z, _P]),
    'mrdis_nvnet_loss_bwd': (_I, [_P, _P, _P, _P, _P, _I, _P, _P, _P, _P, _P, _I, _c.c_double, _P, _P, _P, _P, _P]),
    'mrdis_seg_counts': (_I, [_P, _P, _P, _I, _L, _I, _I, _P]),
    'mrdis_seg_accum': (_I, [_P, _P, _I, _I, _I, _I, _I, _I, _I, _I, _P]),
    'mrdis_seg_label_volume': (_I, [_P, _P, _P, _P, _P, _I, _I, _I, _I, _I, _I, _P]),
    'mrdis_synth_accum': (_I, [_P, _I, _P, _P, _I, _I, _I, _I, _I, _I, _I, _I, _P]),
    'mrdis_synth_finish': (_I, [_P, _P, _P, _I, _I, _I, _F, _P]),
    'mrdis_seg2d_label_planes': (_I, [_P, _I, _I, _P, _P, _I, _I, _I, _I, _I, _I, _I, _P]),
    'mrdis_seg2d_finish': (_I, [_P, _P, _I, _I, _I, _I, _P]),
    'mrdis_fuse_present_fwd': (_I, [_P, _P, _I, _P, _I, _P, _I, _I, _L, _I, _P]),
    'mrdis_fuse_present_bwd': (_I, [_P, _I, _P, _P, _I, _P, _I, _P, _P, _I, _L, _I, _P]),
    'mrdis_region_surfaces': (_I, [_P, _P, _P, _I, _P, _P, _I, _I, _I, _I, _P]),
    'mrdis_edt_workspace': (_Z, [_I, _I, _I, _I, _I]),
    'mrdis_edt_sq': (_I, [_P, _c.c_char_p, _I, _P, _P, _Z, _I, _I, _I, _I, _P]),
    'mrdis_surface_hist': (_I, [_P, _I, _P, _L, _P, _Z, _I, _I, _I, _I, _P]),
    'mrdis_cc_label': (_I, [_P, _I, _I, _P, _P, _I, _I, _I, _I, _P]),
    'mrdis_cc_clean_workspace': (_Z, [_I]),
    'mrdis_cc_clean': (_I, [_P, _P, _P, _I, _I, _I, _I, _I, _P, _P, _P, _Z, _I, _I, _I, _I, _P]),
    'mrdis_region_planes': (_I, [_P, _P, _P, _I, _P, _I, _I, _I, _I, _P]),
    'mrdis_dilate_workspace': (_Z, [_I, _I, _I, _I, _I]),
    'mrdis_dilate': (_I, [_P, _P, _I, _I, _P, _Z, _I, _I, _I, _I, _P]),
    'mrdis_lesion_match': (_I, [_P, _P, _P, _P, _P, _P, _I, _I, _P, _P, _P, _P, _I, _I, _I, _I, _I, _P]),
    'mrdis_lesion_expand': (_I, [_P, _P, _P, _P, _P, _P, _P, _I, _P, _I, _I, _I, _P, _P, _I, _I, _I, _I, _I, _P]),
    'mrdis_maxpool_fwd': (_I, [_P, _I, _P, _P, _I, _I, _I, _I, _I, _P]),
    'mrdis_maxpool_bwd': (_I, [_P, _P, _P, _I, _I, _I, _I, _I, _I, _P]),
    'mrdis_sumsq_workspace': (_Z, []),
    'mrdis_sumsq_finite': (_I, [_P, _L, _P, _P, _Z, _P]),
    'mrdis_adam_amsgrad_step': (_I, [_P, _P, _P, _P, _P, _L, _F, _F, _F, _F, _F, _I, _P, _P, _F, _F, _P, _P, _I, _P, _P, _I, _P]),
    'mrdis_conv3d_fwd': (_I, [_P, _I, _P, _P, _P, _I, _P, _I] + [_I] * 9 + [_P]),
    'mrdis_conv3d_bwd_data': (_I, [_P, _I, _P, _P, _I] + [_I] * 9 + [_P]),
    'mrdis_conv3d_bwd_weight_workspace': (_Z, [_I] * 9),
    'mrdis_conv3d_bwd_weight': (_I, [_P, _I, _P, _I, _P, _P, _P, _Z] + [_I] * 9 + [_P]),
    'mrdis_groupnorm_workspace': (_Z, [_I, _L, _I, _I]),
    'mrdis_groupnorm_relu_fwd': (_I, [_P, _I, _P, _I, _P, _P, _P, _P, _P, _Z, _I, _L, _I, _I, _F, _I, _P]),
    'mrdis_groupnorm_relu_bwd': (_I, [_P, _I, _P, _I, _P, _P, _P, _P, _P, _I, _P, _P, _P, _Z, _I, _L, _I, _I, _I, _P]),
    'mrdis_groupnorm_relu_bwd_add': (_I, [_P, _I, _P, _I, _P, _P, _P, _P, _P, _I, _P, _P, _P, _I, _P, _Z, _I, _L, _I, _I, _I, _P]),
    'mrdis_upsample2x_add_fwd': (_I, [_P, _P, _P, _I, _I, _I, _I, _I, _P]),
    'mrdis_upsample2x_bwd': (_I, [_P, _P, _I, _I, _I, _I, _I, _P]),
    'mrdis_cosine_top1_workspace': (_Z, [_I, _I, _I]),
    'mrdis_cosine_top1': (_I, [_P, _L, _P, _I, _I, _P, _P, _I, _P, _P, _P, _Z, _P]),
    'mrdis_conv2d_2src_fwd': (_I, [_P, _I, _I, _P, _I, _I, _P, _P, _P, _I] + [_I] * 9 + [_P]),
    'mrdis_conv2d_2src_bwd_data': (_I, [_P, _I, _P, _P, _I, _I, _P, _I, _I] + [_I] * 8 + [_P]),
    'mrdis_conv2d_2src_bwd_weight_workspace': (_Z, [_I] * 10),
    'mrdis_conv2d_2src_bwd_weight': (_I, [_P, _I, _I, _P, _I, _I, _P, _I, _P, _P, _I, _P, _Z] + [_I] * 8 + [_P]),
    'mrdis_softplus_fwd': (_I, [_P, _I, _P, _I, _L, _I, _P]),
    'mrdis_softplus_bwd': (_I, [_P, _I, _P, _I, _P, _I, _L, _I, _P]),
    'mrdis_softmax_fwd': (_I, [_P, _I, _P, _I, _L, _I, _P]),
    'mrdis_softmax_bwd': (_I, [_P, _I, _P, _I, _P, _I, _L, _I, _P]),
    'mrdis_kl_fwd': (_I, [_P, _P, _I, _I, _P, _P, _L, _I, _P, _P, _I, _I, _I, _P]),
    'mrdis_kl_bwd': (_I, [_P, _P, _P, _I, _I, _P, _P, _L, _I, _P, _P, _P, _I, _I, _P, _P, _I, _I, _I, _P]),
    'mrdis_avgpool_fwd': (_I, [_P, _I, _P, _I, _I, _I, _I, _I, _P]),
    'mrdis_avgpool_bwd': (_I, [_P, _P, _I, _I, _I, _I, _I, _I, _P]),
    'mrdis_chatt_workspace': (_Z, [_I, _L, _I, _I]),
    'mrdis_chatt_fwd': (_I, [_P, _I, _P, _I, _P, _P, _P, _P, _P, _I, _P, _P, _P, _P, _Z, _I, _L, _I, _I, _P]),
    'mrdis_chatt_bwd': (_I, [_P, _I, _P, _I, _P, _P, _P, _P, _P, _P, _I, _P, _P, _P, _P, _P, _Z, _I, _L, _I, _I, _P]),
    'mrdis_symdiff_fwd': (_I, [_P, _I, _P, _I, _I, _I, _I, _I, _P]),
    'mrdis_symdiff_bwd': (_I, [_P, _I, _P, _I, _P, _I, _I, _I, _I, _I, _P]),
    'mrdis_rgate_fwd': (_I, [_P, _I, _P, _P, _I, _I, _I, _I, _I, _P]),
    'mrdis_rgate_bwd': (_I, [_P, _I, _P, _I, _P, _P, _I, _P, _I, _I, _I, _I, _P]),
    'mrdis_prep_workspace': (_Z, [_I, _I, _I]),
    'mrdis_prep_stats': (_I, [_P, _I, _L, _L, _L] + [_I] * 9 + [_c.c_double, _c.c_double, _P, _P, _Z, _P]),
    'mrdis_prep_write': (_I, [_P, _I, _L, _L, _L] + [_I] * 7 + [_c.c_double, _c.c_double, _P, _I, _I, _P, _P]),
    'mrdis_export_volume': (_I, [_P] + [_I] * 11 + [_P, _c.c_double, _P, _I, _P]),
}
EXPORTED_SYMBOLS = tuple(_SIGS)


def load(path=None):
    global _lib
    if _lib is not None:
        return _lib
    path = path or LIB_PATH
    if not os.path.exists(path):
        raise MrdisLibraryError(
            f'{path} not found: build it with `python __graft_entry__.py` / `make -C '
            f'{os.path.dirname(path)}`.  There is no CPU or eager fallback for the hot path.')
    lib = ctypes.CDLL(path)
    for name, (res, args) in _SIGS.items():
        fn = getattr(lib, name)
        fn.restype, fn.argtypes = res, args
    _lib = lib
    return lib


def _chk(rc, what):
    if rc != 0:
        raise MrdisError(f'{what}: {load().mrdis_strerror(rc).decode()} ({rc})')


def set_option(name, value):
    _chk(load().mrdis_set_option(name.encode(), int(value)), f'set_option({name})')


def get_option(name):
    return int(load().mrdis_get_option(name.encode()))


OPTION_NAMES = ('wino', 'nt_mb', 'wino_pipe', 'wino_u', 'wino4', 'wino4r', 'bconv4', 'split6', 'debug_no16', 'debug_nothin', 'debug_noc4', 'debug_nodma',
                'debug_no16_3d', 'debug_bilgen', 'debug_now16', 'debug_nopack', 'debug_mode', 'debug_bn', 'debug_kc', 'debug_bm', 'debug_c4_tw',
                'debug_wgsplit', 'debug_bn3', 'debug_kc3', 'c4_grid', 'debug_c4_blocks', 'zsearch_grid', 'debug_volgen')


def options_snapshot():
    return {n: get_option(n) for n in OPTION_NAMES}


def options_restore(snap):
    for n, v in snap.items():
        if get_option(n) != v:
            set_option(n, v)


KERNEL_FAMILIES = WINO_FAMILIES = ('wino', 'wino_spade', 'wino2', 'wino2_spade', 'wino4', 'wino4_spade', 'wino4n', 'wino4r', 'wino_wgrad', 'wino_wgrad2', 'wino4_wgrad', 'bconv3', 'bconv3_spade', 'bconv4', 'bconv4_spade',
                                   'split6_c4', 'split6_c16', 'split6_wgrad16', 'split6_co4', 'split6_c3d', 'split6_w3d', 'split6_tap',
                                   'all',
                                   'zsearch')
VARIANT_FAMILIES = ('conv2src', 'ana_act')
LATENT_FAMILIES = ('kl', 'avgpool')
OUTDEC_FAMILIES = ('chatt', 'symdiff', 'rgate')
CONV3D_FAMILIES = ('direct3d', 'c3d16', 'wgrad3d', 'wgrad3d16', 'wino_wgrad3d')
DATA_FAMILIES = ('volgather',)
PATCH_FAMILIES = ('fgcount', 'patchorigin', 'patchgather')
PATCH_MAX_CLASSES = 8
WARP_FAMILIES = ('patchwarp',)
LOSS3D_FAMILIES = ('loss3d', 'segcounts')
SEGVOL_FAMILIES = ('segaccum', 'seglabels')
SYNTH_FAMILIES = ('synthaccum', 'synthfinish')
SEG2D_FAMILIES = ('seg2dlabels', 'seg2dfinish')
FUSE_FAMILIES = ('fuse',)
SURFDIST_FAMILIES = ('regsurf', 'edt', 'surfhist')
CC_FAMILIES = ('cclabel', 'ccclean')
LESION_FAMILIES = ('dilate', 'lesmatch', 'lesexpand')
PREP_FAMILIES = ('prepstats', 'prepwrite')
EXPORT_FAMILIES = ('export',)
ELEM_FAMILIES = ('stat_vec', 'stat_scalar', 'stat_interp', 'spade_up2_onepass', 'spade_up2_twopass', 'bil_fwd_x2', 'bil_fwd_general',
                 'bil_bwd_x2', 'bil_bwd_tight3', 'bil_bwd_tight5', 'bil_bwd_general', 'elem_v1')
LAUNCH_COUNTERS = (WINO_FAMILIES + VARIANT_FAMILIES + LATENT_FAMILIES + OUTDEC_FAMILIES + CONV3D_FAMILIES + DATA_FAMILIES + PATCH_FAMILIES + WARP_FAMILIES + LOSS3D_FAMILIES + SEGVOL_FAMILIES
                    + SYNTH_FAMILIES + SEG2D_FAMILIES + FUSE_FAMILIES + SURFDIST_FAMILIES + CC_FAMILIES + PREP_FAMILIES + EXPORT_FAMILIES + LESION_FAMILIES)
ALL_COUNTERS = LAUNCH_COUNTERS + ELEM_FAMILIES
SYNTH_MAX_SRC = 8
SEG2D_MAX_SETS = 16
SEG2D_MAX_VIEWS = 2
SEG2D_FLIPS = {'': 0, 'h': 1, 'w': 2}
FUSE_MAX_SRC = 8
FUSE_METHODS = ('mean', 'max', 'mean-max-min')
EDT_FAR = 1 << 30
EDT_MAX_SRC = 8
EDT_MAX_EXTENT = 1024
SURF_MAX_REGIONS = 4
CC_MAX_EXTENT = 1024
CC_LABEL_LAUNCHES = 3
CC_CONNECTIVITIES = (6, 18, 26)
DILATE_MAX_ITERATIONS = 8


def stream_fill(t, value=0.0):
    if (t.dtype is not torch.float32 or t.numel() % 4 != 0
            or not (t.is_contiguous() or t.is_contiguous(memory_format=torch.channels_last))): _refuse('stream_fill', 'vec dtype dense', t)
    _chk(load().mrdis_stream_fill(t.data_ptr(), t.numel(), float(value), _stream()), 'stream_fill')
    return t


def dynamic_lds():
    import re
    buf = _c.create_string_buffer(16384)
    load().mrdis_dynamic_lds_table(buf, 16384)
    out = {}
    for line in buf.value.decode().splitlines():
        expr, _, b = line.rpartition('=')
        if not expr or not b.isdigit():
            continue
        name = re.sub(r'<.*', '', expr.strip().lstrip('(')).strip()
        out[name] = max(out.get(name, 0), int(b))
    return out


def launch_counts(reset=False, elem=False):
    lib = load()
    out = {f: int(lib.mrdis_launch_count(f.encode())) for f in (ALL_COUNTERS if elem else LAUNCH_COUNTERS)}
    if reset:
        lib.mrdis_launch_count_reset()
    return out


class option:

    def __init__(self, name, value):
        self.name, self.value = name, value

    def __enter__(self):
        self.prev = get_option(self.name)
        set_option(self.name, self.value)

    def __exit__(self, *exc):
        set_option(self.name, self.prev)


_DEV_INDEX = None


def _stream():
    global _DEV_INDEX
    if _DEV_INDEX is None:
        _DEV_INDEX = torch.cuda.current_device()
    return torch._C._cuda_getCurrentRawStream(_DEV_INDEX)


def _ptr(t):
    return None if t is None else t.data_ptr()


_WS = {}


def _ws(nbytes, device):
    n = max(int(nbytes), 16)
    key = (device, _stream())
    buf = _WS.get(key)
    if buf is None or buf.numel() < n:
        size = max(n, 1 << 20) if buf is None else max(n, 2 * buf.numel())
        buf = _WS[key] = torch.empty(size, dtype=torch.uint8, device=device)
    return buf


_WS_BYTES = {}


def _ws_bytes(fn, *args):
    key = (fn.__name__, args)
    v = _WS_BYTES.get(key)
    if v is None:
        v = _WS_BYTES[key] = fn(*args)
    return v


def nhwc(t):
    if t.dim() != 4 or not (t.dtype is torch.float32 or t.dtype is torch.bfloat16): _refuse('nhwc', 'dtype', t)
    if t.is_contiguous(memory_format=torch.channels_last) and t.shape[1] > 1 and t.shape[3] > 1:
        return t, t.shape[1]
    N, C, H, W = t.shape
    s = t.stride()
    ld = s[3] if W > 1 else (s[2] if H > 1 else (s[0] if N > 1 else C))
    ok = (ld >= C and (C == 1 or s[1] == 1) and (W == 1 or s[3] == ld) and
          (H == 1 or s[2] == W * ld) and (N == 1 or s[0] == H * W * ld))
    if not ok:
        t = t.contiguous(memory_format=torch.channels_last)
        if t.stride()[1] != 1 and C > 1:
            t = t.permute(0, 2, 3, 1).contiguous().permute(0, 3, 1, 2)
        ld = C
    return t, ld


def empty_nhwc(N, C, H, W, device, dtype=torch.float32):
    return torch.empty((N, C, H, W), dtype=dtype, device=device, memory_format=torch.channels_last)


def _dt(*tensors):
    kind = None
    for t in tensors:
        if t is None:
            continue
        d = t.dtype
        if kind is None:
            kind = d
        elif d is not kind:
            raise MrdisError(f'activation views must be all fp32 or all bf16, got {kind} and {d}')
    if kind is torch.float32:
        return 0
    if kind is torch.bfloat16:
        return 2
    raise MrdisError(f'activation views must be fp32 or bf16, got {kind}')


_CLAIMS = {'like': 'operands of one shape', 'layer': 'the shape the layer\'s kernel, stride and padding make of the input', 'filter': 'a (taps, reduce, out) filter for the layer',
           'out': 'an output view of the result\'s shape, written in place', 'vec': 'vectors, tables and buffers of the element count the shapes and integers imply',
           'dtype': 'the dtype the entry point reads', 'dense': 'dense memory (contiguous, NHWC or NDHWC as documented)', 'arg': 'arguments in their documented range'}


def _refuse(what, claims, *ts):
    raise MrdisError(f'{what} wants ' + '; '.join(_CLAIMS[c] for c in claims.split()) + ', ' + _got(*ts))


def _got(*ts):
    return 'got ' + ', '.join(f'{t.dtype} {tuple(t.shape)} strides {t.stride()} on {t.device}' if isinstance(t, torch.Tensor) else repr(t) for t in ts)


def _want(t, what, dtype, shape=None, device=None, cl=False, dense=True):
    ok = isinstance(t, torch.Tensor) and t.dtype is dtype and (device is None or t.device == device)
    if ok and shape is not None:
        ok = t.dim() == len(shape) and all(isinstance(w, str) or w == n for w, n in zip(shape, t.shape))
    if not (ok and (not dense or (t.movedim(1, -1) if cl else t).is_contiguous())):
# ... 1633 lines not shown
```

representation-disentanglement_amd/model.py:

```python
import copy
import weakref

import numpy as np
import torch
import torch.nn as nn
import torch.nn.functional as F

from . import ops


def _pair(v):
    return (v, v) if isinstance(v, int) else tuple(v)


def _groups(inputs_type):
    return len(inputs_type) if isinstance(inputs_type, (list, tuple)) else 0


class _routing(nn.Module):

    def __init__(self, in_channels, num_experts):
        super().__init__()
        self.fc = nn.Linear(in_channels, num_experts)

# ... 191 lines not shown
            if (skip and self.training and x.is_cuda and ops.cat_elision() and isinstance(self.act, nn.Sequential) and len(self.act) == 0):
                N, C, H, W = x.shape
                buf = ops.hip.empty_nhwc(N, 2 * C, H, W, x.device, x.dtype)
                x = self.bn(x, into=(buf, 0), groups=G)
                x._mrdis_catbuf = buf
                return x
            x = self.bn(x, groups=G)
        return self.act(x)


class Act_Deconv_BN_Concat_New(nn.Module):

    def __init__(self, in_num_ch, out_num_ch, filter_size=3, stride=1, padding=1, activation='relu', upsample=True,
                 is_last=False, is_bn=True, is_cond=False):
        super().__init__()
        if not upsample:
            raise NotImplementedError('ConvTranspose2d variant is not on the path (model.py:2178)')
        self.is_bn, self.is_cond, self.is_last = is_bn, is_cond, is_last
        self.act = nn.ELU(inplace=True) if activation == 'elu' else nn.Sequential()
        self.conv = Conv2d(is_cond)(in_num_ch, out_num_ch, filter_size, stride, padding=padding)
        self.bn = BatchNorm2d(out_num_ch)

    def forward(self, x_down, x_up, inputs_type=None):
        x_up = self.act(x_up)
        x_up = ops.bilinear(x_up, (2 * x_up.shape[2], 2 * x_up.shape[3]), True)
        x_up = self.conv(x_up, inputs_type) if self.is_cond else self.conv(x_up)
        if self.is_last:
            return x_up
        G = max(_groups(inputs_type), 1)
        if self.is_bn and self.training and x_up.is_cuda and ops.cat_elision() and x_down.dtype == x_up.dtype and isinstance(self.act, nn.Sequential) \
                and x_down.shape[0] == x_up.shape[0] and x_down.shape[2:] == x_up.shape[2:]:
            Cd, Cu = x_down.shape[1], x_up.shape[1]
            buf = getattr(x_down, '_mrdis_catbuf', None)
            if buf is not None and buf.shape[1] == Cd + Cu and buf.dtype == x_up.dtype:
                x_down._mrdis_catbuf = None
                x_up = self.bn(x_up, into=(buf, Cd), groups=G)
                return ops.cat_join(x_down, x_up, buf)
        if self.is_bn:
            x_up = self.bn(x_up, groups=G)
        return torch.cat([x_down, x_up], 1)


class AnatomyEncoderEncNew(nn.Module):

    def __init__(self, in_num_ch=7, first_num_ch=32, is_cond=False):
        super().__init__()
        self.is_cond = is_cond
        c = first_num_ch
        self.down_1 = Conv2d(is_cond)(in_num_ch, c, 4, 2, padding=1)
        self.act_1 = nn.LeakyReLU(0.2, inplace=True)
        self.down_2 = Conv_BN_Act_New(c, 2 * c, is_cond=is_cond)
        self.down_3 = Conv_BN_Act_New(2 * c, 4 * c, is_cond=is_cond)
        self.down_4 = Conv_BN_Act_New(4 * c, 8 * c, is_cond=is_cond)
        self.down_5 = Conv_BN_Act_New(8 * c, 8 * c, activation='no', is_cond=is_cond)

    def forward(self, x, inputs_type=None):
        d1 = self.down_1(x, inputs_type, lrelu=True) if self.is_cond else self.down_1(x, lrelu=True)
        d2 = self.down_2(d1, inputs_type, skip=True)
        d3 = self.down_3(d2, inputs_type, skip=True)
        d4 = self.down_4(d3, inputs_type, skip=True)
        d5 = self.down_5(d4, inputs_type)
        return [d1, d2, d3, d4, d5]


class AnatomyEncoderDecNew(nn.Module):

    def __init__(self, first_num_ch=32, out_num_ch=8, output_act='softmax', is_cond=False):
        super().__init__()
        c = first_num_ch
        self.up_4 = Act_Deconv_BN_Concat_New(8 * c, 8 * c, is_cond=is_cond)
        self.up_3 = Act_Deconv_BN_Concat_New(16 * c, 4 * c, is_cond=is_cond)
        self.up_2 = Act_Deconv_BN_Concat_New(8 * c, 2 * c, is_cond=is_cond)
        self.up_1 = Act_Deconv_BN_Concat_New(4 * c, c, is_cond=is_cond)
        self.output = Act_Deconv_BN_Concat_New(2 * c, out_num_ch, is_last=True, is_cond=is_cond)

    def forward(self, down_list, inputs_type=None, need_out=True):
        if inputs_type is None:
            inputs_type = expand_type(1.0, down_list[0].shape[0], down_list[0].device)
        u4 = self.up_4(down_list[3], down_list[4], inputs_type)
        u3 = self.up_3(down_list[2], u4, inputs_type)
        u2 = self.up_2(down_list[1], u3, inputs_type)
        u1 = self.up_1(down_list[0], u2, inputs_type)
        if not need_out:
            return None, None
        out = self.output(None, u1, inputs_type)
        return out, out


class ModalityEncoderNew(nn.Module):

    def __init__(self, img_num_ch=7, s_num_ch=8, first_num_ch=16, z_size=16, is_cond=False, feat_hw=30):
        super().__init__()
        self.s_num_ch, self.is_cond = s_num_ch, is_cond
        c = first_num_ch
        ch = [img_num_ch + s_num_ch, c, 2 * c, 4 * c, 8 * c, 8 * c]
        conv2d = Conv2d(is_cond)
        for i in range(5):
            setattr(self, f'conv{i + 1}', conv2d(ch[i], ch[i + 1], 3, 2, padding=1))
        dead = []
        for i in range(5):
            dead += [nn.Conv2d(ch[i], ch[i + 1], 3, 2, padding=1), nn.LeakyReLU(0.2, inplace=True)]
        self.convs = nn.Sequential(*dead)
        self.fcs = nn.Sequential(nn.Linear(feat_hw * 8 * c, 2 * z_size), nn.LeakyReLU(0.2, inplace=True))
        self.mean = nn.Linear(2 * c, z_size)
        self.log_var = nn.Linear(2 * c, z_size)

    def forward(self, xi, si, inputs_type=None):
        if _groups(inputs_type) and not (self.s_num_ch == 0 and self.is_cond):
            raise ValueError('a grouped call takes a conditional modality encoder that does not read the anatomy maps (s_num_ch == 0)')
        t = (inputs_type,) if self.is_cond else ()
        if self.s_num_ch == 0:
            x = self.conv1(xi, *t, lrelu=True)
        else:
            if si is None or si.shape[1] != self.s_num_ch:
                raise ValueError(f'the modality encoder reads the {self.s_num_ch}-channel anatomy maps (others.mod_enc_s); got '
                                 f'{None if si is None else tuple(si.shape)}')
            x = self.conv1.forward_2src(xi, si, *t, lrelu=True)
        for i in range(1, 5):
            x = getattr(self, f'conv{i + 1}')(x, *t, lrelu=True)
        x = x.contiguous(memory_format=torch.contiguous_format).reshape(x.shape[0], -1).float()
        x = self.fcs(x)
        return self.mean(x), self.log_var(x)


class SPADEBlockNew(nn.Module):

    def __init__(self, input_size, in_num_ch=128, out_num_ch=128, s_num_ch=8, is_cond=False):
        super().__init__()
        self.is_cond, self.input_size = is_cond, tuple(input_size)
        conv2d = Conv2d(is_cond)
        self.zi_layers = nn.InstanceNorm2d(in_num_ch)
        self.si_layers = conv2d(s_num_ch, in_num_ch, 3, 1, padding=1)
        self.gamma = conv2d(in_num_ch, in_num_ch, 3, 1, padding=1)
        self.beta = conv2d(in_num_ch, in_num_ch, 3, 1, padding=1)
        self.out = conv2d(in_num_ch, out_num_ch, 3, 1, padding=1)

    def _fused_gb(self, inputs_type):
        hit = ops.lookup_type_row(inputs_type) if ops.mix_cache_active() else None
        if hit is not None and self.gamma.weight.shape == self.beta.weight.shape:
            table, row = hit
            allw = ops.cached_mix((id(self), 'gb_all', table.data_ptr(), table._version),
                                  lambda: ops.mix_pair_fused_all(self.gamma, self.beta, table))
            bias = ops.cached_mix((id(self), 'gb_bias'), lambda: torch.cat([self.gamma.bias, self.beta.bias]))
            return (allw[2 * row], allw[2 * row + 1]), bias

        def fused():
            g_tck, g_tkc = self.gamma.mixed_uniform(inputs_type)
            b_tck, b_tkc = self.beta.mixed_uniform(inputs_type)
            return ((torch.cat([g_tck, b_tck], 2), torch.cat([g_tkc, b_tkc], 1)),
                    torch.cat([self.gamma.bias, self.beta.bias]))
        return ops.step_cache((id(self), 'gb', inputs_type.data_ptr(), inputs_type._version), fused)

    def forward(self, si, zi, inputs_type=None):
        size = self.input_size
        src = si
        si = ops.step_cache(('bil', id(src), size), lambda: (src, ops.bilinear(src, size, False)))[1]
        kh, kw = self.gamma.kernel_size
        if _groups(inputs_type):
            pad = self.gamma.padding[0]
            si_out = ops.conv2d_grouped(si, [self.si_layers.mixed_uniform(t) for t in inputs_type], self.si_layers.bias, kh, kw, pad, share_x=True,
                                        co=self.si_layers.out_channels)
            fused = [self._fused_gb(t) for t in inputs_type]
            mix = ops.gb_spade(si_out, zi, [f[0] for f in fused], fused[0][1], self.zi_layers.eps)
            return self.out(mix, inputs_type)
        t = (inputs_type,) if self.is_cond else ()
        si_out = self.si_layers(si, *t)
        if self.is_cond and (si_out.shape[0] == 1 or inputs_type.stride(0) == 0):
            (w_tck, w_tkc), bias = self._fused_gb(inputs_type)
            if ((kh, kw) == (3, 3) and self.gamma.padding[0] == 1 and type(si_out) is torch.Tensor and si_out.is_cuda
                    and ops.mix_cache_active() and torch.is_grad_enabled()):
                mix = ops.gb_spade(si_out, zi, [(w_tck, w_tkc)], bias, self.zi_layers.eps)
            else:
                gb = ops.conv2d(si_out, w_tck, w_tkc, bias, kh, kw, 1, self.gamma.padding[0])
                mix = ops.instnorm_spade_gb(zi, gb, self.zi_layers.eps)
        else:
            gamma = self.gamma(si_out, *t)
            beta = self.beta(si_out, *t)
            mix = ops.instnorm_spade(zi, gamma, beta, self.zi_layers.eps)
        return self.out(mix, *t)


def _up2(x, norm=None):
    return ops.bilinear_up2(x, None if norm is None else norm.eps)


class SPADENewShared(nn.Module):

    def __init__(self, image_size=(192, 160), in_num_ch=7, z_size=16, z_num_ch=128, s_num_ch=8, is_cond=False):
        super().__init__()
        self.z_num_ch, self.image_size, self.is_cond = z_num_ch, tuple(image_size), is_cond
        H, W = image_size
        self.zi_scaler = nn.Linear(z_size, H * W * z_num_ch // 1024)
        self.sp1 = SPADEBlockNew((H // 32, W // 32), z_num_ch, z_num_ch, s_num_ch, is_cond)
        self.sp2 = SPADEBlockNew((H // 16, W // 16), z_num_ch, z_num_ch, s_num_ch, is_cond)
        self.sp3 = SPADEBlockNew((H // 8, W // 8), z_num_ch, z_num_ch, s_num_ch, is_cond)

    def forward(self, si, zi, inputs_type=None, scatter=None):
        H, W = self.image_size
        x = ops.to_storage(self.zi_scaler(zi).reshape(-1, self.z_num_ch, H // 32, W // 32))
        x = self.sp1(si, x, inputs_type)
        x = self.sp2(si, _up2(x, self.sp2.zi_layers), inputs_type)
        x = self.sp3(si, _up2(x, self.sp3.zi_layers), inputs_type)
        if scatter is not None and ops.up2_scatter_applies(x):
            return ops.bilinear_up2_scatter(x, scatter[0], scatter[1], scatter[2], self.sp3.zi_layers.eps)
        return _up2(x, self.sp3.zi_layers)


class SPADENewNotShared(nn.Module):

    def __init__(self, image_size=(192, 160), in_num_ch=7, z_size=16, z_num_ch=128, s_num_ch=8, is_cond=False,
                 output_activation='softplus'):
        super().__init__()
        self.is_cond = is_cond
        H, W = image_size
        self.sp4 = SPADEBlockNew((H // 4, W // 4), z_num_ch, z_num_ch // 2, s_num_ch, is_cond)
        self.sp5 = SPADEBlockNew((H // 2, W // 2), z_num_ch // 2, z_num_ch // 4, s_num_ch, is_cond)
        self.sp6 = SPADEBlockNew((H, W), z_num_ch // 4, z_num_ch // 8, s_num_ch, is_cond)
        self.out = Conv2d(is_cond)(z_num_ch // 8, in_num_ch, 1, 1)
        if output_activation == 'softplus':
            self.out_act = nn.Softplus()
        elif output_activation == 'no':
            self.out_act = nn.Sequential()
        else:
            raise ValueError('No activation in SPADENotShared')

    def forward(self, si, zi_sp4_input, inputs_type=None):
        x = self.sp4(si, zi_sp4_input, inputs_type)
        x = self.sp5(si, _up2(x, self.sp5.zi_layers), inputs_type)
        x = self.sp6(si, _up2(x, self.sp6.zi_layers), inputs_type)
        x = self.out(x, inputs_type) if self.is_cond else self.out(x)
        return self.out_act(x)

    def grouped_ok(self):
        blocks = (self.sp4, self.sp5, self.sp6)
        return (self.is_cond and all(b.si_layers.stride == (1, 1) and b.gamma.kernel_size == b.out.kernel_size == b.si_layers.kernel_size
                                     and b.gamma.weight.shape == b.beta.weight.shape for b in blocks)
                and self.out.stride == (1, 1))


class SPADENew(nn.Module):

    def __init__(self, image_size=(192, 160), in_num_ch=7, z_size=16, z_num_ch=128, s_num_ch=8, is_cond=False,
                 output_activation='softplus'):
        super().__init__()
        self.z_num_ch, self.image_size, self.is_cond = z_num_ch, tuple(image_size), is_cond
        H, W = image_size
        self.zi_scaler = nn.Linear(z_size, H * W * z_num_ch // 1024)
        self.sp1 = SPADEBlockNew((H // 32, W // 32), z_num_ch, z_num_ch, s_num_ch, is_cond)
        self.sp2 = SPADEBlockNew((H // 16, W // 16), z_num_ch, z_num_ch, s_num_ch, is_cond)
        self.sp3 = SPADEBlockNew((H // 8, W // 8), z_num_ch, z_num_ch, s_num_ch, is_cond)
        self.sp4 = SPADEBlockNew((H // 4, W // 4), z_num_ch, z_num_ch // 2, s_num_ch, is_cond)
        self.sp5 = SPADEBlockNew((H // 2, W // 2), z_num_ch // 2, z_num_ch // 4, s_num_ch, is_cond)
        self.sp6 = SPADEBlockNew((H, W), z_num_ch // 4, z_num_ch // 8, s_num_ch, is_cond)
        self.out = Conv2d(is_cond)(z_num_ch // 8, in_num_ch, 1, 1)
        if output_activation == 'softplus':
            self.out_act = nn.Softplus()
        elif output_activation == 'no':
            self.out_act = nn.Sequential()
        else:
            raise ValueError('No activation in SPADENotShared')

    head = SPADENewShared.forward
    tail = SPADENewNotShared.forward

    def forward(self, si, zi, inputs_type=None):
        return self.tail(si, self.head(si, zi, inputs_type), inputs_type)


class Discriminator(nn.Module):

    def __init__(self, in_num_ch=8, inter_num_ch=16, input_shape=(160, 192), is_patch_gan=False):
        super().__init__()
        c = inter_num_ch
        L = [HipConv2d(in_num_ch, c, 4, 2, padding=1), nn.LeakyReLU(0.2)]
        for a, b in ((c, 2 * c), (2 * c, 4 * c), (4 * c, 8 * c), (8 * c, 4 * c)):
            L += [HipConv2d(a, b, 4, 2, padding=1), BatchNorm2d(b), nn.LeakyReLU(0.2)]
        self.discrim = nn.Sequential(*L)
        self.is_patch_gan = is_patch_gan
        if is_patch_gan:
            self.fc = HipConv2d(4 * c, 1, 3, 1, padding=1)
        else:
            self.fc = nn.Sequential(
                nn.Flatten(),
                nn.Linear(int(input_shape[0] * input_shape[1] * 4 * c / (32 * 32)), c * 16),
                nn.LeakyReLU(0.2),
                nn.Linear(c * 16, 1))

    def forward(self, x):
        mods = list(self.discrim)
        i = 0
        while i < len(mods):
            m = mods[i]
            if isinstance(m, HipConv2d) and isinstance(mods[i + 1], nn.LeakyReLU):
                x = m(x, lrelu=True); i += 2
            else:
                x = m(x); i += 1
        if self.is_patch_gan:
            return self.fc(x)
        return self.fc(x.contiguous(memory_format=torch.contiguous_format).float())


class ModalityDistribution(nn.Module):

    def __init__(self, z_size=16, inter_num_ch=128):
        super().__init__()
        self.z_size = z_size
        self.linear = nn.Sequential(nn.Linear(1, inter_num_ch), nn.LeakyReLU(0.2), nn.Linear(inter_num_ch, 2 * z_size))

    def forward(self, x):
        feat = self.linear(x.float())
        return feat[:, :self.z_size], feat[:, self.z_size:]


class LegacyConvBNAct(nn.Module):

    def __init__(self, in_num_ch, out_num_ch, activation='lrelu'):
        super().__init__()
        self.conv = nn.Sequential(HipConv2d(in_num_ch, out_num_ch, 4, 2, padding=1), BatchNorm2d(out_num_ch))
        self.act = nn.ELU(inplace=True) if activation == 'elu' else nn.Sequential()

    def forward(self, x):
        return self.act(self.conv(x))


class LegacyUpConcat(nn.Module):

    def __init__(self, in_num_ch, out_num_ch, is_last=False):
        super().__init__()
        self.act = nn.Sequential()
        self.is_last = is_last
        self.up = nn.Sequential(nn.Upsample(scale_factor=2, mode='bilinear', align_corners=True),
                                HipConv2d(in_num_ch, out_num_ch, 3, 1, padding=1))
        self.bn = BatchNorm2d(out_num_ch)

    def forward(self, x_down, x_up, buf=None):
        x_up = ops.bilinear(self.act(x_up), (2 * x_up.shape[2], 2 * x_up.shape[3]), True)
        x_up = self.up[1](x_up)
        if self.is_last:
            return x_up
        if buf is not None:
            return ops.cat_join(x_down, self.bn(x_up, into=(buf, x_down.shape[1])), buf)
        return torch.cat([x_down, self.bn(x_up)], 1)


class SpatialAttentionLayer(nn.Module):

    def __init__(self, in_num_ch, gate_num_ch, inter_num_ch, sample_factor=(2, 2)):
        super().__init__()
        self.W_x = HipConv2d(in_num_ch, inter_num_ch, sample_factor, sample_factor, bias=False)
        self.W_g = HipConv2d(gate_num_ch, inter_num_ch, 1, 1)
        self.W_psi = HipConv2d(inter_num_ch, 1, 1, 1)
        self.W_out = nn.Sequential(HipConv2d(in_num_ch, in_num_ch, 1, 1), BatchNorm2d(in_num_ch))

    def forward(self, x, g):
        x_post = self.W_x(x)
        g_post = ops.bilinear(self.W_g(g), tuple(x_post.shape[2:]), False)
        alpha = torch.sigmoid(self.W_psi(F.relu(x_post + g_post)))
        alpha_up = ops.bilinear(alpha, tuple(x.shape[2:]), False)
        return self.W_out(alpha_up * x), alpha_up


def _target_act(output_activation):
    if output_activation == 'no':
        return nn.Sequential()
    if output_activation == 'softplus':
        return nn.Softplus()
    raise NotImplementedError(f"target_output_act {output_activation!r}: only 'no' and 'softplus' (main_missing.py:75-80) are built")


def _apply_target_act(act, y):
    return ops.softplus(y) if isinstance(act, nn.Softplus) else act(y)


class GANShortGeneratorWithSpatialAttention(nn.Module):

    def __init__(self, in_num_ch, out_num_ch, first_num_ch=64, output_activation='no'):
        super().__init__()
        act = _target_act(output_activation)
        c = first_num_ch
        self.down_1 = nn.Sequential(HipConv2d(in_num_ch, c, 4, 2, padding=1), nn.LeakyReLU(0.2, inplace=True))
        self.down_2 = LegacyConvBNAct(c, 2 * c)
        self.down_3 = LegacyConvBNAct(2 * c, 4 * c)
        self.down_4 = LegacyConvBNAct(4 * c, 8 * c)
        self.down_5 = LegacyConvBNAct(8 * c, 8 * c, activation='no')
        self.att_4 = SpatialAttentionLayer(8 * c, 8 * c, 8 * c)
        self.up_4 = LegacyUpConcat(8 * c, 8 * c)
        self.att_3 = SpatialAttentionLayer(4 * c, 16 * c, 4 * c)
        self.up_3 = LegacyUpConcat(16 * c, 4 * c)
        self.att_2 = SpatialAttentionLayer(2 * c, 8 * c, 2 * c)
        self.up_2 = LegacyUpConcat(8 * c, 2 * c)
        self.att_1 = SpatialAttentionLayer(c, 4 * c, c)
        self.up_1 = LegacyUpConcat(4 * c, c)
        self.output = LegacyUpConcat(2 * c, out_num_ch, is_last=True)
        self.output_act = act

    def forward(self, x):
        d1 = self.down_1[0](x, lrelu=True)
        d2 = self.down_2(d1); d3 = self.down_3(d2); d4 = self.down_4(d3); d5 = self.down_5(d4)
        c4, a4 = self.att_4(d4, d5); u4 = self.up_4(c4, d5)
        c3, a3 = self.att_3(d3, u4); u3 = self.up_3(c3, u4)
        c2, a2 = self.att_2(d2, u3); u2 = self.up_2(c2, u3)
        c1, a1 = self.att_1(d1, u2); u1 = self.up_1(c1, u2)
        return _apply_target_act(self.output_act, self.output(None, u1)), {'alpha_4': a4, 'alpha_3': a3, 'alpha_2': a2, 'alpha_1': a1}


def _down_path(c, in_num_ch):
    return [('down_1', nn.Sequential(HipConv2d(in_num_ch, c, 4, 2, padding=1), nn.LeakyReLU(0.2, inplace=True))),
            ('down_2', LegacyConvBNAct(c, 2 * c)), ('down_3', LegacyConvBNAct(2 * c, 4 * c)),
            ('down_4', LegacyConvBNAct(4 * c, 8 * c)), ('down_5', LegacyConvBNAct(8 * c, 8 * c, activation='no'))]


class GANShortGenerator(nn.Module):

    def __init__(self, in_num_ch, out_num_ch, first_num_ch=64, output_activation='softplus'):
        super().__init__()
        c = first_num_ch
# ... 689 lines not shown
```

representation-disentanglement_amd/ops.py:

```python
import contextlib
import numpy as _np
import os as _os

import torch
from torch.autograd import Function

from . import hip


class _MixExperts(Function):

    @staticmethod
    def forward(ctx, W, r):
        w_tck, w_tkc = hip.mix_experts_fwd(W, r)
        ctx.save_for_backward(W, r)
        ctx.mark_non_differentiable(w_tkc)
        return w_tck, w_tkc

    @staticmethod
    def backward(ctx, g_tck, _g_tkc):
        W, r = ctx.saved_tensors
        dW, dr = hip.mix_experts_bwd(g_tck, W, r)
        return dW, dr


def mix_experts(W, r):
    return _MixExperts.apply(W, r)


class _MixExpertsRouted(Function):

    @staticmethod
    def forward(ctx, W, fcw, fcb, t_row):
        w_tck, w_tkc, r = hip.mix_experts_routed_fwd(W, fcw, fcb, t_row)
        ctx.save_for_backward(W, r, t_row)
        ctx.emb = fcw.shape[1]
        ctx.mark_non_differentiable(w_tkc)
        return w_tck, w_tkc

    @staticmethod
    def backward(ctx, g_tck, _g_tkc):
        W, r, t_row = ctx.saved_tensors
        dW, dfcw, dfcb = hip.mix_experts_routed_bwd(g_tck, W, r, t_row, ctx.emb)
        return dW, dfcw, dfcb, None


def mix_experts_routed(W, fcw, fcb, t_row):
    return _MixExpertsRouted.apply(W, fcw, fcb, t_row)


class _MixExpertsRoutedAll(Function):

    @staticmethod
    def forward(ctx, W, fcw, fcb, types):
        if _COMPUTE_DTYPE != hip.DT_F32:
            tck, tkc, r, btck, btkc = hip.mix_experts_routed_multi_fwd(W, fcw, fcb, types, want_bf16=True)
            if _MIX_CACHE is not None:
                for a, ba, bb in zip(tck, btck, btkc):
                    _MIX_CACHE[('bf16w', id(a))] = (a, bb, ba)
        else:
            tck, tkc, r = hip.mix_experts_routed_multi_fwd(W, fcw, fcb, types)
        ctx.save_for_backward(W, r, types)
        ctx.params = (W, fcw, fcb)
        ctx.set_materialize_grads(False)
        ctx.mark_non_differentiable(*tkc)
        out = []
        for a, b in zip(tck, tkc):
            out += [a, b]
        return tuple(out)

    @staticmethod
    def backward(ctx, *grads):
        W, r, types = ctx.saved_tensors
        sinks = tuple(_grad_sink(q) for q in ctx.params)
        if all(g is not None for g in sinks) and sinks[0].shape == W.shape:
            hip.mix_experts_routed_multi_bwd(list(grads[0::2]), W, r, types, sinks=sinks)
            return None, None, None, None
        dW, dfcw, dfcb = hip.mix_experts_routed_multi_bwd(list(grads[0::2]), W, r, types)
        return dW, dfcw, dfcb, None


def mix_experts_routed_all(W, fcw, fcb, types):
    return _MixExpertsRoutedAll.apply(W, fcw, fcb, types)


class _MixPairFusedAll(Function):

    @staticmethod
    def forward(ctx, Wg, fwg, fbg, Wb, fwb, fbb, types):
        E, C, Ci, kh, kw = Wg.shape
        T, M = kh * kw, types.shape[0]
        dev_ = Wg.device
        tck = [torch.empty((T, Ci, 2 * C), dtype=torch.float32, device=dev_) for _ in range(M)]
        tkc = [torch.empty((T, 2 * C, Ci), dtype=torch.float32, device=dev_) for _ in range(M)]
        btck = btkc = None
        if _COMPUTE_DTYPE != hip.DT_F32:
            btck = [torch.empty((T, Ci, 2 * C), dtype=torch.bfloat16, device=dev_) for _ in range(M)]
            btkc = [torch.empty((T, 2 * C, Ci), dtype=torch.bfloat16, device=dev_) for _ in range(M)]
        rg = hip.mix_experts_routed_multi_fwd(Wg, fwg, fbg, types, into=(tck, tkc, btck, btkc, 0, 2 * C))
        rb = hip.mix_experts_routed_multi_fwd(Wb, fwb, fbb, types, into=(tck, tkc, btck, btkc, C, 2 * C))
        if btck is not None and _MIX_CACHE is not None:
            for a, ba, bb in zip(tck, btck, btkc):
                _MIX_CACHE[('bf16w', id(a))] = (a, bb, ba)
        ctx.save_for_backward(Wg, rg, Wb, rb, types)
        ctx.params = (Wg, fwg, fbg, Wb, fwb, fbb)
        ctx.C = C
        ctx.set_materialize_grads(False)
        ctx.mark_non_differentiable(*tkc)
        out = []
        for a, b in zip(tck, tkc):
            out += [a, b]
        return tuple(out)

    @staticmethod
    def backward(ctx, *grads):
        Wg, rg, Wb, rb, types = ctx.saved_tensors
        C = ctx.C
        g = list(grads[0::2])
        res = []
        for W, r, prm, col0 in ((Wg, rg, ctx.params[0:3], 0), (Wb, rb, ctx.params[3:6], C)):
            sinks = tuple(_grad_sink(q) for q in prm)
            if all(x is not None for x in sinks) and sinks[0].shape == W.shape:
                hip.mix_experts_routed_multi_bwd(g, W, r, types, sinks=sinks, col0=col0, ld=2 * C)
                res += [None, None, None]
            else:
                res += list(hip.mix_experts_routed_multi_bwd(g, W, r, types, col0=col0, ld=2 * C))
        return tuple(res) + (None,)


def mix_pair_fused_all(gamma, beta, types):
    return _MixPairFusedAll.apply(gamma.weight, gamma._routing_fn.fc.weight, gamma._routing_fn.fc.bias,
                                  beta.weight, beta._routing_fn.fc.weight, beta._routing_fn.fc.bias, types)


def native_head(kh, kw, Ci, Co):
    return kh == 1 and kw == 1 and Ci == 16 and 1 <= Co <= 8


class MixPlan:

    def __init__(self, singles, pairs, M, want_bf16, device, pad16=False, group=None):
        self.singles, self.pairs, self.M, self.want_bf16 = singles, pairs, M, want_bf16
        self.group = group
        self.params = []
        self.probe = singles[0].weight if singles else (pairs[0][1].weight if pairs else None)
        shapes = []
        specs = []
        self.padded = {}
        for m in singles:
            E, Co, Ci, kh, kw = m.weight.shape
            Ci_p, Co_p = Ci, Co
            if pad16 and m.stride[0] == 1 and (Ci < 16 or Co < 16) and hip.bconv_eligible(max(Ci, 16), max(Co, 16)) and not native_head(kh, kw, Ci, Co):
                Ci_p, Co_p = max(Ci, 16), max(Co, 16)
                self.padded[id(m)] = (Ci, Co)
            shapes.append((kh * kw, Ci_p, Co_p)); specs.append((len(shapes) - 1, m, 0, Co_p))
        for blk, g, b in pairs:
            E, C, Ci, kh, kw = g.weight.shape
            shapes.append((kh * kw, Ci, 2 * C))
            specs.append((len(shapes) - 1, g, 0, 2 * C)); specs.append((len(shapes) - 1, b, C, 2 * C))
        self.shapes = shapes
# ... 577 lines not shown
                res = hip.conv2d_bwd_weight(x32 if share_x else x32[g * B:(g + 1) * B], dyg, kh, kw, 1, pad, need_bias=bias is not None, bias_sink=sink, may_decline=True,
                                            pad16=(Cif == 16 and Ci == 4 and dyg.dtype == torch.bfloat16))
                if res is None:
                    res = hip.conv2d_bwd_weight(x32 if share_x else x32[g * B:(g + 1) * B], hip.cast_view(dyg, torch.float32), kh, kw, 1, pad,
                                                need_bias=bias is not None, bias_sink=sink)
                if Cif > res[0].shape[1]:
                    res = (torch.nn.functional.pad(res[0], (0, 0, 0, Cif - Ci)), res[1])
            if res is None:
                if xin is None:
                    xin = hip.cast_view(x32, torch.bfloat16, Ci_p)
                xg = xin if share_x else xin[g * B:(g + 1) * B]
                if dyg is None:
                    dyg = dy_pad()[g * B:(g + 1) * B]
                res = hip.conv2d_bwd_weight(xg, dyg, kh, kw, ctx.stride, pad, need_bias=bias is not None, bias_sink=sink, dtype=dt)
                if padded:
                    res = (res[0][:, :Cif, :Cof].contiguous(), res[1])
            dw, db = res
            dws += [dw, None]
            if db is not None:
                db_total = db if db_total is None else db_total + db
        if db_total is not None and Co_p != Co:
            db_total = db_total[:Co]
            s_ = _grad_sink(bias)
            if s_ is not None:
                s_.add_(db_total); db_total = None
        dx = None
        if need_x and dx4 is not None:
            dx = dx4.permute(0, 2, 3, 1).reshape(G, B, H, W, 4).sum(0).permute(0, 3, 1, 2) if (share_x and G > 1) else dx4
        elif need_x:
            dx = dxb.permute(0, 2, 3, 1).reshape(G, B, H, W, Ci_p).sum(0).permute(0, 3, 1, 2) if share_x else dxb
            if dx.dtype != x_dtype or Ci_p != Ci:
                dx = hip.cast_view(dx, x_dtype, Ci)
        return (dx, db_total, None, None, None, None, None, None, None, None) + tuple(dws)


class _GbSpadeFn(Function):

    @staticmethod
    def forward(ctx, si_out, z, bias, G, eps, smean, srstd, up2_src, *filt):
        bm = _COMPUTE_DTYPE == hip.DT_F32_BF16M
        B = z.shape[0] // G
        C, H, W = z.shape[1], z.shape[2], z.shape[3]
        mix = gamma = mean = rstd = None
        wbs = [None] * G
        fusable = (_COMPUTE_DTYPE == hip.DT_F32 and si_out.dtype == torch.float32 and z.dtype == torch.float32) or \
                  (_COMPUTE_DTYPE == hip.DT_BF16 and si_out.dtype == torch.bfloat16 and z.dtype == torch.bfloat16)
        if _GB_SPADE and fusable:
            mix = hip.empty_nhwc(G * B, C, H, W, z.device, z.dtype); gamma = hip.empty_nhwc(G * B, C, H, W, z.device, z.dtype)
            if smean is not None:
                mean, rstd = smean, srstd
            else:
                mean = torch.empty(G * B * C, dtype=torch.float32, device=z.device); rstd = torch.empty_like(mean)
            for g in range(G):
                sl = slice(g * B, (g + 1) * B)
                wb = bf16_filters(filt[2 * g], filt[2 * g + 1]) if _COMPUTE_DTYPE == hip.DT_BF16 else (None, None)
                im = wino_images(filt[2 * g])
                wbs[g] = wb[1] if wb[1] is not None else im.get('dgrad')
                ok = hip.gb_spade_fwd(si_out[sl], filt[2 * g], bias, z[sl], eps, w_bf16=wb[0], stats_ready=smean is not None, w_wino=im.get('spade'),
                                      out=(mix[sl], gamma[sl], mean[g * B * C:(g + 1) * B * C], rstd[g * B * C:(g + 1) * B * C]))
                if ok is None:
                    assert g == 0
                    mix = None
                    break
        if mix is None:
            zs = z
            if _COMPUTE_DTYPE == hip.DT_BF16 and z.dtype == torch.float32:
                zs = hip.cast_view(z, torch.bfloat16)
            gb = hip.empty_nhwc(G * B, 2 * C, H, W, z.device, si_out.dtype)
            for g in range(G):
                wb = bf16_filters(filt[2 * g], filt[2 * g + 1]) if _COMPUTE_DTYPE != hip.DT_F32 else (None, wino_images(filt[2 * g]).get('dgrad'))
                wbs[g] = wb[1]
                hip.conv2d_fwd(si_out[g * B:(g + 1) * B], filt[2 * g], bias, 3, 3, 1, 1, out=gb[g * B:(g + 1) * B], w_bf16=wb[0])
            mix, mean, rstd = hip.instnorm_spade_fwd(zs, gb[:, :C], gb[:, C:], eps, stats=(smean, srstd) if (smean is not None and zs is z) else None)
            gamma = gb[:, :C]
            ctx.z_cast = zs is not z
            z = zs
        else:
            ctx.z_cast = False
        ctx.meta = (G, B, hip.DT_F32_BF16M if _COMPUTE_DTYPE != hip.DT_F32 else hip.DT_F32)
        ctx.wbs = wbs
        ctx.up2 = up2_src is not None
        ctx.z_is_src = ctx.up2 and not ctx.z_cast and up2_src.dtype == z.dtype
        ctx.save_for_backward(si_out, up2_src if ctx.z_is_src else z, gamma, mean, rstd, *[filt[2 * g + 1] for g in range(G)])
        return mix

    @staticmethod
    def backward(ctx, dmix):
        G, B, dt = ctx.meta
        si_out, z, gamma, mean, rstd = ctx.saved_tensors[:5]
        tkcs = ctx.saved_tensors[5:]
        H, W = gamma.shape[2], gamma.shape[3]
        dxs = None
        if ctx.up2:
            if ctx.z_is_src:
                res = hip.instnorm_spade_bwd(dmix, None, gamma, mean, rstd, fused_gb=True, up2=True, xlo=z)
                if res is None:
                    z = hip.bilinear_fwd(z, (H, W), False)
            else:
                res = hip.instnorm_spade_bwd(dmix, z, gamma, mean, rstd, fused_gb=True, up2=True) if not ctx.z_cast else None
            if res is not None:
                dxs, dgb = res
                dz = None
        if dxs is None:
            dz, dgb = hip.instnorm_spade_bwd(dmix, z, gamma, mean, rstd, fused_gb=True)
            if ctx.z_cast:
                dz = hip.cast_view(dz, torch.float32)
            if ctx.up2:
                dxs = hip.bilinear_bwd(dz, (H // 2, W // 2), False)
                dz = None
        need_x = ctx.needs_input_grad[0]
        dx = hip.empty_nhwc(G * B, si_out.shape[1], H, W, gamma.device, si_out.dtype) if need_x else None
        dws, db_total = [], None
        for g in range(G):
            sl = slice(g * B, (g + 1) * B)
            if need_x:
                hip.conv2d_bwd_data(dgb[sl], tkcs[g], (H, W), 3, 3, 1, 1, w_bf16=ctx.wbs[g], out=dx[sl])
            dw, db = hip.conv2d_bwd_weight(si_out[sl], dgb[sl], 3, 3, 1, 1, need_bias=True, dtype=dt)
            dws += [dw, None]
            db_total = db if db_total is None else db_total + db
        return (dx, dz, db_total, None, None, None, None, dxs) + tuple(dws)


_GB_SPADE = _os.environ.get('MRDIS_GB_SPADE', '1') != '0'
_UP2_BWD_FUSED = _os.environ.get('MRDIS_UP2_BWD_FUSED', '1') != '0'
_UP2_BWD_FUSED_BF16 = _os.environ.get('MRDIS_UP2_BWD_FUSED_BF16', '1') != '0'


def set_up2_bwd_fused(enabled):
    global _UP2_BWD_FUSED
    _UP2_BWD_FUSED = bool(enabled)

_GB_INPLACE = _os.environ.get('MRDIS_GB_INPLACE', '1') != '0'


def set_gb_spade(enabled):
    global _GB_SPADE
    _GB_SPADE = bool(enabled)


def gb_spade(si_out, z, filters, bias, eps):
    flat = []
    for a, b in filters:
        flat += [a, b]
    smean, srstd = in_stats_of(z, eps)
    src = getattr(z, '_mrdis_up2_src', None) if _UP2_BWD_FUSED else None
    if src is not None and src.requires_grad and torch.is_grad_enabled() and src.shape[0] == z.shape[0] and src.dtype == z.dtype and (z.dtype == torch.float32 or _UP2_BWD_FUSED_BF16):
        mix = _GbSpadeFn.apply(si_out, z.detach(), bias, len(filters), eps, smean, srstd, src, *flat)
    else:
        mix = _GbSpadeFn.apply(si_out, z, bias, len(filters), eps, smean, srstd, None, *flat)
    mix._mrdis_want_dgb = True
    return mix


def conv2d_grouped(x, filters, bias, kh, kw, pad, lrelu=False, share_x=False, co=None, stride=1):
    flat = []
    for a, b in filters:
        flat += [a, b]
    return _GroupedConvFn.apply(x, bias, len(filters), bool(share_x), kh, kw, pad, bool(lrelu), co, int(stride), *flat)


class _BatchNormTrain(Function):

    @staticmethod
    def forward(ctx, x, gamma, beta, running_mean, running_var, eps, momentum, into=None, groups=1):
        out = None
        if into is not None:
            out = into[0][:, into[1]:into[1] + x.shape[1]]
        y, mean, rstd = hip.bn_train_fwd(x, gamma, beta, running_mean, running_var, eps, momentum, out=out, groups=groups)
        ctx.save_for_backward(x, gamma, mean, rstd)
        ctx.params = (gamma, beta)
        ctx.groups = groups
        return y

    @staticmethod
    def backward(ctx, dy):
        x, gamma, mean, rstd = ctx.saved_tensors
        sg, sb = _grad_sink(ctx.params[0]), _grad_sink(ctx.params[1])
        if sg is not None and sb is not None and ctx.needs_input_grad[1] and ctx.needs_input_grad[2]:
            dx, _, _ = hip.bn_train_bwd(dy, x, gamma, mean, rstd, sink=(sg, sb), groups=ctx.groups)
            return dx, None, None, None, None, None, None, None, None
        dx, dg, db = hip.bn_train_bwd(dy, x, gamma, mean, rstd, groups=ctx.groups)
        return dx, dg, db, None, None, None, None, None, None


def batch_norm_train(x, gamma, beta, running_mean, running_var, eps=1e-5, momentum=0.1, into=None, groups=1):
    return _BatchNormTrain.apply(x, gamma, beta, running_mean, running_var, eps, momentum, into, groups)


class _CatJoin(Function):

    @staticmethod
    def forward(ctx, a, b, buf):
        Ca = a.shape[1]
        ctx.Ca = Ca
        if a.data_ptr() != buf.data_ptr():
            buf[:, :Ca].copy_(a)
        if b.data_ptr() != buf[:, Ca:].data_ptr():
            buf[:, Ca:].copy_(b)
        return buf[:, :]

    @staticmethod
    def backward(ctx, g):
        return g[:, :ctx.Ca], g[:, ctx.Ca:], None


def cat_join(a, b, buf):
    return _CatJoin.apply(a, b, buf)


_CAT_ELISION = _os.environ.get('MRDIS_CAT_ELISION', '1') != '0'


def cat_elision():
    return _CAT_ELISION and torch.is_grad_enabled()


class _InstNormSpade(Function):

    @staticmethod
    def forward(ctx, z, gamma, beta, eps):
        out, mean, rstd = hip.instnorm_spade_fwd(z, gamma, beta, eps)
        ctx.save_for_backward(z, gamma, mean, rstd)
        return out

    @staticmethod
    def backward(ctx, dout):
        z, gamma, mean, rstd = ctx.saved_tensors
        dz, dg = hip.instnorm_spade_bwd(dout, z, gamma, mean, rstd)
        return dz, dg, dout, None


def instnorm_spade(z, gamma, beta, eps=1e-5):
    return _InstNormSpade.apply(z, gamma, beta, eps)


class _InstNormSpadeGB(Function):

    @staticmethod
    def forward(ctx, z, gb, eps):
        C = z.shape[1]
        gamma, beta = gb[:, :C], gb[:, C:]
        out, mean, rstd = hip.instnorm_spade_fwd(z, gamma, beta, eps)
        ctx.save_for_backward(z, gb, mean, rstd)
        return out

    @staticmethod
    def backward(ctx, dout):
        z, gb, mean, rstd = ctx.saved_tensors
        dz, dgb = hip.instnorm_spade_bwd(dout, z, gb[:, :z.shape[1]], mean, rstd, fused_gb=True)
        return dz, dgb, None


def instnorm_spade_gb(z, gb, eps=1e-5):
    return _InstNormSpadeGB.apply(z, gb, eps)


class _Bilinear(Function):
    @staticmethod
    def forward(ctx, x, out_hw, align_corners):
        ctx.geom = (x.shape[2], x.shape[3], align_corners)
        return hip.bilinear_fwd(x, out_hw, align_corners)

    @staticmethod
    def backward(ctx, dy):
        Hi, Wi, ac = ctx.geom
        return hip.bilinear_bwd(dy, (Hi, Wi), ac), None, None


def bilinear(x, out_hw, align_corners):
    return _Bilinear.apply(x, tuple(out_hw), bool(align_corners))


class _BilinearUp2Stats(Function):

    @staticmethod
    def forward(ctx, x, eps):
        ctx.geom = (x.shape[2], x.shape[3])
        res = hip.bilinear_up2_stats(x, eps)
        if res is None:
            y = hip.bilinear_fwd(x, (2 * x.shape[2], 2 * x.shape[3]), False)
            mean = rstd = torch.empty(0, dtype=torch.float32, device=x.device)
        else:
            y, mean, rstd = res
        ctx.mark_non_differentiable(mean, rstd)
        return y, mean, rstd

    @staticmethod
    def backward(ctx, dy, _gm, _gr):
        return hip.bilinear_bwd(dy, ctx.geom, False), None


class _Up2ScatterFn(Function):

    @staticmethod
    def forward(ctx, x, zbuf, j, eps):
        M = zbuf.shape[0]
        B = x.shape[0] // M
        ctx.geom = (x.shape[2], x.shape[3]); ctx.M = M; ctx.B = B
        blocks = zbuf[:, j * B:(j + 1) * B]
        res = hip.bilinear_up2_stats(x, eps, out_blocks=blocks)
        if res is None:
            raise hip.MrdisError('bilinear_up2 (scatter): unsupported geometry')
        _, mean, rstd = res
        ctx.mark_non_differentiable(mean, rstd)
        return tuple(blocks[i] for i in range(M)) + (mean, rstd)

# ... 730 lines not shown
```

Baseline: 248.5.

## Fold SPADE output 3x3 conv and 1x1 head conv into one composed conv

Composes the final SPADE block's 3x3 conv with the following 1x1 output conv into a single 3x3 conv with fewer output channels. The composed weights are built in double precision on the GPU each step. New narrow-output forward, data-grad and weight-grad kernels run the fused conv, and a compose-backward kernel maps the gradients back to the original weights. This removes the wide intermediate activation and one conv pass in both forward and backward. The cost is extra compose kernels, narrow-Co kernels that leave part of the MFMA tile idle, and a slightly different rounding order.

```diff
diff --git a/include/mrdis.h b/include/mrdis.h
--- a/include/mrdis.h
+++ b/include/mrdis.h
@@ -353,6 +353,18 @@
 int mrdis_export_volume(const void* src, int src_dtype, int layout, int Hc, int Wc, int D, int h0, int h1, int w0, int w1, int B,
                         int kind, const double* stats, double fill, void* dst, int dst_dtype, void* stream);
 
+int mrdis_head_fold_applies(int N, int H, int W, int Ci, int Cm, int Co);
+long long mrdis_head_compose_floats(int Ci, int Co);
+int mrdis_head_compose_fwd(const void* const* w3_tck, const void* const* w1_tck, const float* b3, const float* b1, float* out,
+                           int G, int Ci, int Cm, int Co, void* stream);
+int mrdis_head_compose_bwd(const float* dout, const void* const* w3_tck, const void* const* w1_tck, const float* b3, float* dw3_tck, float* dw1_tck,
+                           float* db3, float* db1, int accumulate_bias, int G, int Ci, int Cm, int Co, void* stream);
+int mrdis_head_conv_fwd(const float* x, int ldx, const float* w_tck, const float* bias, float* y, int ldy, int N, int H, int W, int Ci, int Co, void* stream);
+int mrdis_head_conv_bwd_data(const float* dy, int lddy, const float* w_tkc, float* dx, int lddx, int N, int H, int W, int Ci, int Co, void* stream);
+size_t mrdis_head_conv_bwd_weight_workspace(int N, int H, int W, int Ci, int Co);
+int mrdis_head_conv_bwd_weight(const float* x, int ldx, const float* dy, int lddy, float* dw_tck, float* dbias, void* workspace, size_t workspace_bytes,
+                               int N, int H, int W, int Ci, int Co, void* stream);
+
 #ifdef __cplusplus
 }
 #endif
diff --git a/representation-disentanglement_amd/__init__.py b/representation-disentanglement_amd/__init__.py
--- a/representation-disentanglement_amd/__init__.py
+++ b/representation-disentanglement_amd/__init__.py
@@ -1,4 +1,4 @@
-from . import hip, ops, model, model3d, trainer
+from . import hip, headfold, ops, model, model3d, trainer
 from .hip import MrdisError, MrdisLibraryError, LIB_PATH
 from .model import (CondConv2d, Conv2d, HipConv2d, BatchNorm2d, Conv_BN_Act_New,
                     Act_Deconv_BN_Concat_New, AnatomyEncoderEncNew, AnatomyEncoderDecNew,
diff --git a/representation-disentanglement_amd/csrc/mrdis_c16.hip b/representation-disentanglement_amd/csrc/mrdis_c16.hip
--- a/representation-disentanglement_amd/csrc/mrdis_c16.hip
+++ b/representation-disentanglement_amd/csrc/mrdis_c16.hip
@@ -5,6 +5,7 @@
     int N, H, W, Ci, ldx, ldy, lrelu;
     int tilesY, tilesX, ntiles;
     unsigned x_bytes;
+    int Co;
 };
 
 namespace {
@@ -113,6 +114,7 @@
     }
 }
 
+template <bool FULL>
 __global__ __launch_bounds__(256, 2) void conv3x3_c16_split6_kernel(const C16Params p) {
     constexpr int CI = 32, Q = CI / 4, PB = 208;
     constexpr int XR = (C16_NPX * Q + 255) / 256;
@@ -124,10 +126,18 @@
     for (int g = 0; g < 9; ++g)
 #pragma unroll
         for (int j = 0; j < 8; ++j) {
-            const float v = p.w[(g * CI + 8 * kq + j) * 16 + l16];
+            float v;
+            if constexpr (FULL) v = p.w[(g * CI + 8 * kq + j) * 16 + l16];
+            else v = l16 < p.Co ? p.w[(g * CI + 8 * kq + j) * p.Co + l16] : 0.f;
             mrdis_split3(v, a[g][0], a[g][1], a[g][2], j);
         }
-    const float4 bv = p.bias ? make_float4(p.bias[4 * kq], p.bias[4 * kq + 1], p.bias[4 * kq + 2], p.bias[4 * kq + 3]) : make_float4(0.f, 0.f, 0.f, 0.f);
+    float4 bv = make_float4(0.f, 0.f, 0.f, 0.f);
+    if constexpr (FULL) {
+        if (p.bias) bv = make_float4(p.bias[4 * kq], p.bias[4 * kq + 1], p.bias[4 * kq + 2], p.bias[4 * kq + 3]);
+    } else if (p.bias) {
+        bv.x = 4 * kq < p.Co ? p.bias[4 * kq] : 0.f; bv.y = 4 * kq + 1 < p.Co ? p.bias[4 * kq + 1] : 0.f;
+        bv.z = 4 * kq + 2 < p.Co ? p.bias[4 * kq + 2] : 0.f; bv.w = 4 * kq + 3 < p.Co ? p.bias[4 * kq + 3] : 0.f;
+    }
 
     const __amdgpu_buffer_rsrc_t rs_x = mrdis_buffer_rsrc(p.x, p.x_bytes);
     int s_l[XR], s_ry[XR], s_rx[XR], s_q[XR];
@@ -210,7 +220,15 @@
                 const int oy = ty * C16_TH + 2 * wave + (t >> 1), ox = tx * C16_TW + 16 * (t & 1) + l16;
                 float4 o = make_float4(acc[t][0] + bv.x, acc[t][1] + bv.y, acc[t][2] + bv.z, acc[t][3] + bv.w);
                 if (p.lrelu) { o.x = o.x > 0.f ? o.x : 0.2f * o.x; o.y = o.y > 0.f ? o.y : 0.2f * o.y; o.z = o.z > 0.f ? o.z : 0.2f * o.z; o.w = o.w > 0.f ? o.w : 0.2f * o.w; }
-                if (oy < p.H && ox < p.W) *reinterpret_cast<float4*>(p.y + ((long long)(n * p.H + oy) * p.W + ox) * p.ldy + 4 * kq) = o;
+                if constexpr (FULL) {
+                    if (oy < p.H && ox < p.W) *reinterpret_cast<float4*>(p.y + ((long long)(n * p.H + oy) * p.W + ox) * p.ldy + 4 * kq) = o;
+                } else if (oy < p.H && ox < p.W) {
+                    float* dst = p.y + ((long long)(n * p.H + oy) * p.W + ox) * p.ldy + 4 * kq;
+                    if (4 * kq < p.Co) dst[0] = o.x;
+                    if (4 * kq + 1 < p.Co) dst[1] = o.y;
+                    if (4 * kq + 2 < p.Co) dst[2] = o.z;
+                    if (4 * kq + 3 < p.Co) dst[3] = o.w;
+                }
             }
         }
         __syncthreads();
@@ -362,12 +380,31 @@
     const int grid = p.ntiles < 512 ? p.ntiles : 512;
     const size_t lds = sizeof(float) * (size_t)C16_NPX * (Ci + 4);
     if (Ci == 32 && (mrdis_opt(MRDIS_OPT_SPLIT6) == 1 || mrdis_opt(MRDIS_OPT_SPLIT6) == 5)) {
-        if (!mrdis_lds_optin((const void*)conv3x3_c16_split6_kernel, 72 * 1024)) return MRDIS_ELAUNCH;
+        if (!mrdis_lds_optin((const void*)conv3x3_c16_split6_kernel<true>, 72 * 1024)) return MRDIS_ELAUNCH;
         mrdis_count(MRDIS_CNT_SPLIT6_C16);
-        MRDIS_LAUNCH(conv3x3_c16_split6_kernel, dim3(grid), dim3(256), (size_t)C16_NPX * 208, s, p);
+        MRDIS_LAUNCH(conv3x3_c16_split6_kernel<true>, dim3(grid), dim3(256), (size_t)C16_NPX * 208, s, p);
     } else
     if (Ci == 32) MRDIS_LAUNCH((conv3x3_c16_kernel<2>), dim3(grid), dim3(256), lds, s, p);
     else MRDIS_LAUNCH((conv3x3_c16_kernel<1>), dim3(grid), dim3(256), lds, s, p);
     MRDIS_CHECK_LAUNCH();
     return MRDIS_OK;
 }
+
+int mrdis_run_c16_narrow(const float* x, int ldx, const float* w_tck, const float* bias, float* y, int ldy, int N, int H, int W, int Ci, int Co, hipStream_t s) {
+    if (Ci != 32 || Co < 1 || Co >= 16 || ldx % 4 != 0 || ldx < Ci || ldy < Co || (((uintptr_t)x) & 15) != 0 || (((uintptr_t)y) & 3) != 0) return MRDIS_EUNSUPPORTED;
+    if ((long long)N * H * W < 65536 || mrdis_opt(MRDIS_OPT_NOW16) || mrdis_opt(MRDIS_OPT_SPLIT6) != 1) return MRDIS_EUNSUPPORTED;
+    const long long xb = 4LL * (((long long)N * H * W - 1) * ldx + Ci);
+    if (xb >= 0x7fffffffLL) return MRDIS_EUNSUPPORTED;
+    C16Params p{};
+    p.x = x; p.w = w_tck; p.bias = bias; p.y = y; p.N = N; p.H = H; p.W = W; p.Ci = Ci; p.ldx = ldx; p.ldy = ldy; p.lrelu = 0; p.Co = Co;
+    p.tilesY = mrdis_cdiv(H, C16_TH); p.tilesX = mrdis_cdiv(W, C16_TW);
+    const long long nt = (long long)N * p.tilesY * p.tilesX;
+    if (nt > 0x7fffffffLL) return MRDIS_EUNSUPPORTED;
+    p.ntiles = (int)nt; p.x_bytes = (unsigned)xb;
+    const int grid = p.ntiles < 512 ? p.ntiles : 512;
+    if (!mrdis_lds_optin((const void*)conv3x3_c16_split6_kernel<false>, 72 * 1024)) return MRDIS_ELAUNCH;
+    mrdis_count(MRDIS_CNT_SPLIT6_C16);
+    MRDIS_LAUNCH(conv3x3_c16_split6_kernel<false>, dim3(grid), dim3(256), (size_t)C16_NPX * 208, s, p);
+    MRDIS_CHECK_LAUNCH();
+    return MRDIS_OK;
+}
diff --git a/representation-disentanglement_amd/csrc/mrdis_common.h b/representation-disentanglement_amd/csrc/mrdis_common.h
--- a/representation-disentanglement_amd/csrc/mrdis_common.h
+++ b/representation-disentanglement_amd/csrc/mrdis_common.h
@@ -67,6 +67,7 @@
     X(PREPSTATS, "prepstats") X(PREPWRITE, "prepwrite")  \
     X(EXPORT, "export")  \
     X(DILATE, "dilate") X(LESMATCH, "lesmatch") X(LESEXPAND, "lesexpand")  \
+    X(HEAD_DGRAD, "head_dgrad") X(HEAD_COMPOSE, "head_compose")  \
     X(STAT_VEC, "stat_vec") X(STAT_SCALAR, "stat_scalar") X(STAT_INTERP, "stat_interp")  \
     X(SPADE_UP2_ONEPASS, "spade_up2_onepass") X(SPADE_UP2_TWOPASS, "spade_up2_twopass")  \
     X(BIL_FWD_X2, "bil_fwd_x2") X(BIL_FWD_GENERAL, "bil_fwd_general")  \
diff --git a/representation-disentanglement_amd/csrc/mrdis_headfold.hip b/representation-disentanglement_amd/csrc/mrdis_headfold.hip
--- /dev/null
+++ b/representation-disentanglement_amd/csrc/mrdis_headfold.hip
@@ -0,0 +1,314 @@
+#include "mrdis_common.h"
+
+#define MRDIS_HEAD_MAXG 8
+
+struct HeadComposeParams {
+    const float* w3[MRDIS_HEAD_MAXG];
+    const float* w1[MRDIS_HEAD_MAXG];
+    const float* b3; const float* b1;
+    float* out; long long stride;
+    int Ci, Cm, Co;
+};
+
+__global__ __launch_bounds__(256) void head_compose_fwd_kernel(const HeadComposeParams p) {
+    const int g = blockIdx.y, i = blockIdx.x * 256 + threadIdx.x;
+    const int n = 9 * p.Ci * p.Co;
+    const float* __restrict__ w3 = p.w3[g];
+    const float* __restrict__ w1 = p.w1[g];
+    float* out = p.out + (long long)g * p.stride;
+    if (i < n) {
+        const int t = i / (p.Ci * p.Co), r = i - t * p.Ci * p.Co, ci = r / p.Co, o = r - ci * p.Co;
+        double s = 0.0;
+        for (int c = 0; c < p.Cm; ++c) s = fma((double)w1[c * p.Co + o], (double)w3[(t * p.Ci + ci) * p.Cm + c], s);
+        out[i] = (float)s;
+        out[n + (t * p.Co + o) * p.Ci + ci] = (float)s;
+    } else if (i < n + p.Co) {
+        const int o = i - n;
+        double s = p.b1 ? (double)p.b1[o] : 0.0;
+        if (p.b3)
+            for (int c = 0; c < p.Cm; ++c) s = fma((double)w1[c * p.Co + o], (double)p.b3[c], s);
+        out[2 * n + o] = (float)s;
+    }
+}
+
+struct HeadComposeBwdParams {
+    const float* w3[MRDIS_HEAD_MAXG];
+    const float* w1[MRDIS_HEAD_MAXG];
+    const float* b3;
+    const float* dout; long long stride;
+    float* dw3; float* dw1;
+    float* db3; float* db1;
+    int accumulate, G, Ci, Cm, Co;
+};
+
+__global__ __launch_bounds__(256) void head_compose_bwd_kernel(const HeadComposeBwdParams p) {
+    const int g = blockIdx.y;
+    int i = blockIdx.x * 256 + threadIdx.x;
+    const int n3 = 9 * p.Ci * p.Cm, n1 = p.Cm * p.Co, np = 9 * p.Ci * p.Co;
+    const float* __restrict__ w3 = p.w3[g];
+    const float* __restrict__ w1 = p.w1[g];
+    const float* __restrict__ dwp = p.dout + (long long)g * p.stride;
+    const float* __restrict__ dbp = dwp + 2 * np;
+    if (i < n3) {
+        const int c = i % p.Cm, r = i / p.Cm;
+        double s = 0.0;
+        for (int o = 0; o < p.Co; ++o) s = fma((double)w1[c * p.Co + o], (double)dwp[r * p.Co + o], s);
+        p.dw3[(long long)g * n3 + i] = (float)s;
+        return;
+    }
+    i -= n3;
+    if (i < n1) {
+        const int c = i / p.Co, o = i - c * p.Co;
+        double s = 0.0;
+        for (int r = 0; r < 9 * p.Ci; ++r) s = fma((double)dwp[r * p.Co + o], (double)w3[r * p.Cm + c], s);
+        if (p.b3) s = fma((double)dbp[o], (double)p.b3[c], s);
+        p.dw1[(long long)g * n1 + i] = (float)s;
+        return;
+    }
+    i -= n1;
+    if (g != 0) return;
+    if (i < p.Cm) {
+        if (p.db3 == nullptr) return;
+        double s = 0.0;
+        for (int k = 0; k < p.G; ++k) {
+            const float* d = p.dout + (long long)k * p.stride + 2 * np;
+            for (int o = 0; o < p.Co; ++o) s = fma((double)p.w1[k][i * p.Co + o], (double)d[o], s);
+        }
+        p.db3[i] = p.accumulate ? p.db3[i] + (float)s : (float)s;
+        return;
+    }
+    i -= p.Cm;
+    if (i < p.Co && p.db1 != nullptr) {
+        double s = 0.0;
+        for (int k = 0; k < p.G; ++k) s += (double)p.dout[(long long)k * p.stride + 2 * np + i];
+        p.db1[i] = p.accumulate ? p.db1[i] + (float)s : (float)s;
+    }
+}
+
+struct HeadDgradParams {
+    const float* dy; const float* w; float* dx;
+    int N, H, W, Co, lddy, lddx;
+    int tilesY, tilesX, ntiles;
+    unsigned dy_bytes;
+};
+
+namespace {
+constexpr int HD_TH = 8, HD_TW = 32, HD_RW = HD_TW + 2, HD_NPX = (HD_TH + 2) * HD_RW;
+constexpr int HD_PB = 48;
+constexpr int HD_IN_BYTES = HD_NPX * HD_PB;
+constexpr int HD_OP = 36;
+constexpr int HD_YR = 11;
+constexpr size_t HD_LDS = (size_t)HD_IN_BYTES + sizeof(float) * 4 * 64 * HD_OP;
+constexpr unsigned HD_OOB = 0xfffffff0u;
+}
+
+__global__ __launch_bounds__(256, 2) void head_dgrad_split6_kernel(const HeadDgradParams p) {
+    extern __shared__ __attribute__((aligned(16))) unsigned char smem_h[];
+    unsigned char* in = smem_h;
+    const int tid = threadIdx.x, lane = tid & 63, wave = tid >> 6, e = lane & 31, half = lane >> 5;
+    float* ow = reinterpret_cast<float*>(smem_h + HD_IN_BYTES) + wave * 64 * HD_OP;
+
+    bf16x8 a[5][3];
+#pragma unroll
+    for (int s = 0; s < 5; ++s)
+#pragma unroll
+        for (int j = 0; j < 8; ++j) {
+            const int g = 2 * s + half;
+            const float v = (g < 9 && j < p.Co) ? p.w[((8 - g) * p.Co + j) * 32 + e] : 0.f;
+            mrdis_split3(v, a[s][0], a[s][1], a[s][2], j);
+        }
+    const __amdgpu_buffer_rsrc_t rs_y = mrdis_buffer_rsrc(p.dy, p.dy_bytes);
+    const int npp = 256 / p.Co;
+    const int n_px = tid / p.Co, n_c = tid - n_px * p.Co;
+    const bool n_on = n_px < npp;
+    unsigned yr[HD_YR];
+    auto load_tile = [&](int tile) {
+        const bool on = tile < p.ntiles;
+        int t = tile;
+        const int tx = t % p.tilesX; t /= p.tilesX;
+        const int ty = t % p.tilesY;
+        const int n = t / p.tilesY;
+#pragma unroll
+        for (int it = 0; it < HD_YR; ++it) {
+            const int px = it * npp + n_px;
+            const int ly = px / HD_RW, lx = px - ly * HD_RW;
+            const int h = ty * HD_TH - 1 + ly, w_ = tx * HD_TW - 1 + lx;
+            const bool ok = on && n_on && px < HD_NPX && (unsigned)h < (unsigned)p.H && (unsigned)w_ < (unsigned)p.W;
+            yr[it] = __builtin_amdgcn_raw_buffer_load_b32(rs_y, (int)(ok ? 4u * (unsigned)(((n * p.H + h) * p.W + w_) * p.lddy + n_c) : HD_OOB), 0, 0);
+        }
+    };
+    auto store_tile = [&]() {
+#pragma unroll
+        for (int it = 0; it < HD_YR; ++it) {
+            const int px = it * npp + n_px;
+            if (!n_on || px >= HD_NPX) continue;
+            __bf16 hi, mid, lo; mrdis_split3(__uint_as_float(yr[it]), hi, mid, lo);
+            unsigned char* d = in + px * HD_PB + 2 * n_c;
+            *reinterpret_cast<__bf16*>(d) = hi; *reinterpret_cast<__bf16*>(d + 16) = mid; *reinterpret_cast<__bf16*>(d + 32) = lo;
+        }
+    };
+    int boff[2], goff[5];
+#pragma unroll
+    for (int t = 0; t < 2; ++t) boff[t] = ((2 * wave + t) * HD_RW + e) * HD_PB;
+#pragma unroll
+    for (int s = 0; s < 5; ++s) {
+        const int g = (2 * s + half) < 9 ? 2 * s + half : 8;
+        goff[s] = ((g / 3) * HD_RW + (g % 3)) * HD_PB;
+    }
+
+    for (int i = tid; i < HD_IN_BYTES / 16; i += 256) *reinterpret_cast<u32x4*>(in + 16 * i) = u32x4{0u, 0u, 0u, 0u};
+    int tile = mrdis_xcd_remap((int)blockIdx.x, (int)gridDim.x);
+    load_tile(tile);
+    __syncthreads();
+    store_tile();
+    __syncthreads();
+    for (; tile < p.ntiles; tile += gridDim.x) {
+        load_tile(tile + gridDim.x);
+        f32x16 acc[2], acs[2];
+#pragma unroll
+        for (int t = 0; t < 2; ++t)
+#pragma unroll
+            for (int r = 0; r < 16; ++r) { acc[t][r] = 0.f; acs[t][r] = 0.f; }
+#pragma unroll
+        for (int s = 0; s < 5; ++s) {
+            bf16x8 xh[2], xm[2], xl[2];
+#pragma unroll
+            for (int t = 0; t < 2; ++t) {
+                xh[t] = *reinterpret_cast<const bf16x8*>(in + boff[t] + goff[s]);
+                xm[t] = *reinterpret_cast<const bf16x8*>(in + boff[t] + goff[s] + 16);
+                xl[t] = *reinterpret_cast<const bf16x8*>(in + boff[t] + goff[s] + 32);
+            }
+#pragma unroll
+            for (int t = 0; t < 2; ++t) acs[t] = __builtin_amdgcn_mfma_f32_32x32x16_bf16(a[s][1], xm[t], acs[t], 0, 0, 0);
+#pragma unroll
+            for (int t = 0; t < 2; ++t) acs[t] = __builtin_amdgcn_mfma_f32_32x32x16_bf16(a[s][0], xl[t], acs[t], 0, 0, 0);
+#pragma unroll
+            for (int t = 0; t < 2; ++t) acs[t] = __builtin_amdgcn_mfma_f32_32x32x16_bf16(a[s][2], xh[t], acs[t], 0, 0, 0);
+#pragma unroll
+            for (int t = 0; t < 2; ++t) acs[t] = __builtin_amdgcn_mfma_f32_32x32x16_bf16(a[s][0], xm[t], acs[t], 0, 0, 0);
+#pragma unroll
+            for (int t = 0; t < 2; ++t) acs[t] = __builtin_amdgcn_mfma_f32_32x32x16_bf16(a[s][1], xh[t], acs[t], 0, 0, 0);
+#pragma unroll
+            for (int t = 0; t < 2; ++t) acc[t] = __builtin_amdgcn_mfma_f32_32x32x16_bf16(a[s][0], xh[t], acc[t], 0, 0, 0);
+        }
+        {
+            int t_ = tile;
+            const int tx = t_ % p.tilesX; t_ /= p.tilesX;
+            const int ty = t_ % p.tilesY;
+            const int n = t_ / p.tilesY;
+#pragma unroll
+            for (int t = 0; t < 2; ++t)
+#pragma unroll
+                for (int g4 = 0; g4 < 4; ++g4)
+                    *reinterpret_cast<f32x4*>(ow + (t * 32 + e) * HD_OP + 8 * g4 + 4 * half) =
+                        f32x4{acc[t][4 * g4] + acs[t][4 * g4], acc[t][4 * g4 + 1] + acs[t][4 * g4 + 1], acc[t][4 * g4 + 2] + acs[t][4 * g4 + 2], acc[t][4 * g4 + 3] + acs[t][4 * g4 + 3]};
+            __builtin_amdgcn_wave_barrier();
+#pragma unroll
+            for (int k = 0; k < 8; ++k) {
+                const int pp = 8 * k + (lane >> 3), q = lane & 7;
+                const int oy = ty * HD_TH + 2 * wave + (pp >> 5), ox = tx * HD_TW + (pp & 31);
+                const f32x4 v = *reinterpret_cast<const f32x4*>(ow + pp * HD_OP + 4 * q);
+                if (oy < p.H && ox < p.W) *reinterpret_cast<f32x4*>(p.dx + ((long long)(n * p.H + oy) * p.W + ox) * p.lddx + 4 * q) = v;
+            }
+            __builtin_amdgcn_wave_barrier();
+        }
+        __syncthreads();
+        store_tile();
+        __syncthreads();
+    }
+}
+
+static bool head_geometry_ok(long long npix, int Ci, int Co) {
+    if (Ci != 32 || Co < 1 || Co > 8) return false;
+    if (npix < 65536 || npix > 0x7fffffffLL / (4 * 64)) return false;
+    return !mrdis_opt(MRDIS_OPT_NOW16) && mrdis_opt(MRDIS_OPT_SPLIT6) == 1;
+}
+
+static int run_head_dgrad(const float* dy, int lddy, const float* w_tkc, float* dx, int lddx, int N, int H, int W, int Ci, int Co, hipStream_t s) {
+    if (!head_geometry_ok((long long)N * H * W, Ci, Co)) return MRDIS_EUNSUPPORTED;
+    if (lddy < Co || lddx < Ci) return MRDIS_EINVAL;
+    if (lddx % 4 != 0 || (((uintptr_t)dx) & 15) != 0 || (((uintptr_t)dy) & 3) != 0) return MRDIS_EALIGN;
+    const long long yb = 4LL * (((long long)N * H * W - 1) * lddy + Co);
+    if (yb >= 0x7fffffffLL) return MRDIS_EUNSUPPORTED;
+    HeadDgradParams p{};
+    p.dy = dy; p.w = w_tkc; p.dx = dx; p.N = N; p.H = H; p.W = W; p.Co = Co; p.lddy = lddy; p.lddx = lddx;
+    p.tilesY = mrdis_cdiv(H, HD_TH); p.tilesX = mrdis_cdiv(W, HD_TW);
+    const long long nt = (long long)N * p.tilesY * p.tilesX;
+    if (nt > 0x7fffffffLL) return MRDIS_EUNSUPPORTED;
+    p.ntiles = (int)nt; p.dy_bytes = (unsigned)yb;
+    int occ = mrdis_occupancy((const void*)head_dgrad_split6_kernel, 256, HD_LDS);
+    if (occ < 1) occ = 2;
+    if (occ > 3) occ = 3;
+    const long long cap = (long long)occ * mrdis_cu_count();
+    const int grid = nt < cap ? (int)nt : (int)cap;
+    mrdis_count(MRDIS_CNT_HEAD_DGRAD);
+    MRDIS_LAUNCH(head_dgrad_split6_kernel, dim3(grid), dim3(256), HD_LDS, s, p);
+    MRDIS_CHECK_LAUNCH();
+    return MRDIS_OK;
+}
+
+extern "C" {
+
+int mrdis_head_fold_applies(int N, int H, int W, int Ci, int Cm, int Co) {
+    if (N < 1 || H < 1 || W < 1 || Cm < 1 || Cm > 64) return 0;
+    return head_geometry_ok((long long)N * H * W, Ci, Co) ? 1 : 0;
+}
+
+long long mrdis_head_compose_floats(int Ci, int Co) { return 2LL * 9 * Ci * Co + 8; }
+
+int mrdis_head_compose_fwd(const void* const* w3_tck, const void* const* w1_tck, const float* b3, const float* b1, float* out,
+                           int G, int Ci, int Cm, int Co, void* stream) {
+    if (!w3_tck || !w1_tck || !out || G < 1 || G > MRDIS_HEAD_MAXG || Ci < 1 || Ci > 64 || Cm < 1 || Cm > 64 || Co < 1 || Co > 8) return MRDIS_EINVAL;
+    HeadComposeParams p{};
+    for (int g = 0; g < G; ++g) {
+        if (!w3_tck[g] || !w1_tck[g]) return MRDIS_EINVAL;
+        p.w3[g] = (const float*)w3_tck[g]; p.w1[g] = (const float*)w1_tck[g];
+    }
+    p.b3 = b3; p.b1 = b1; p.out = out; p.stride = mrdis_head_compose_floats(Ci, Co); p.Ci = Ci; p.Cm = Cm; p.Co = Co;
+    mrdis_count(MRDIS_CNT_HEAD_COMPOSE);
+    MRDIS_LAUNCH(head_compose_fwd_kernel, dim3(mrdis_cdiv(9 * Ci * Co + Co, 256), G), dim3(256), 0, (hipStream_t)stream, p);
+    MRDIS_CHECK_LAUNCH();
+    return MRDIS_OK;
+}
+
+int mrdis_head_compose_bwd(const float* dout, const void* const* w3_tck, const void* const* w1_tck, const float* b3, float* dw3_tck, float* dw1_tck,
+                           float* db3, float* db1, int accumulate_bias, int G, int Ci, int Cm, int Co, void* stream) {
+    if (!dout || !w3_tck || !w1_tck || !dw3_tck || !dw1_tck || G < 1 || G > MRDIS_HEAD_MAXG || Ci < 1 || Ci > 64 || Cm < 1 || Cm > 64 || Co < 1 || Co > 8)
+        return MRDIS_EINVAL;
+    HeadComposeBwdParams p{};
+    for (int g = 0; g < G; ++g) {
+        if (!w3_tck[g] || !w1_tck[g]) return MRDIS_EINVAL;
+        p.w3[g] = (const float*)w3_tck[g]; p.w1[g] = (const float*)w1_tck[g];
+    }
+    p.b3 = b3; p.dout = dout; p.stride = mrdis_head_compose_floats(Ci, Co); p.dw3 = dw3_tck; p.dw1 = dw1_tck; p.db3 = db3; p.db1 = db1;
+    p.accumulate = accumulate_bias ? 1 : 0; p.G = G; p.Ci = Ci; p.Cm = Cm; p.Co = Co;
+    mrdis_count(MRDIS_CNT_HEAD_COMPOSE);
+    MRDIS_LAUNCH(head_compose_bwd_kernel, dim3(mrdis_cdiv(9 * Ci * Cm + Cm * Co + Cm + Co, 256), G), dim3(256), 0, (hipStream_t)stream, p);
+    MRDIS_CHECK_LAUNCH();
+    return MRDIS_OK;
+}
+
+int mrdis_head_conv_fwd(const float* x, int ldx, const float* w_tck, const float* bias, float* y, int ldy, int N, int H, int W, int Ci, int Co, void* stream) {
+    if (!x || !w_tck || !y) return MRDIS_EINVAL;
+    if (!head_geometry_ok((long long)N * H * W, Ci, Co)) return MRDIS_EUNSUPPORTED;
+    return mrdis_run_c16_narrow(x, ldx, w_tck, bias, y, ldy, N, H, W, Ci, Co, (hipStream_t)stream);
+}
+
+int mrdis_head_conv_bwd_data(const float* dy, int lddy, const float* w_tkc, float* dx, int lddx, int N, int H, int W, int Ci, int Co, void* stream) {
+    if (!dy || !w_tkc || !dx) return MRDIS_EINVAL;
+    return run_head_dgrad(dy, lddy, w_tkc, dx, lddx, N, H, W, Ci, Co, (hipStream_t)stream);
+}
+
+size_t mrdis_head_conv_bwd_weight_workspace(int N, int H, int W, int Ci, int Co) {
+    if (!head_geometry_ok((long long)N * H * W, Ci, Co)) return 0;
+    return mrdis_wgrad16_narrow_workspace(N, H, W, Ci, Co);
+}
+
+int mrdis_head_conv_bwd_weight(const float* x, int ldx, const float* dy, int lddy, float* dw_tck, float* dbias, void* workspace, size_t workspace_bytes,
+                               int N, int H, int W, int Ci, int Co, void* stream) {
+    if (!x || !dy || !dw_tck || !workspace) return MRDIS_EINVAL;
+    if (!head_geometry_ok((long long)N * H * W, Ci, Co)) return MRDIS_EUNSUPPORTED;
+    return mrdis_run_wgrad16_narrow(x, ldx, dy, lddy, dw_tck, dbias, workspace, workspace_bytes, N, H, W, Ci, Co, (hipStream_t)stream);
+}
+
+}
diff --git a/representation-disentanglement_amd/csrc/mrdis_launchers.h b/representation-disentanglement_amd/csrc/mrdis_launchers.h
--- a/representation-disentanglement_amd/csrc/mrdis_launchers.h
+++ b/representation-disentanglement_amd/csrc/mrdis_launchers.h
@@ -66,8 +66,13 @@
 int mrdis_run_wgrad16_bf16(const void* x, int ldx, const void* dy, int lddy, float* dw_tck, float* dbias, void* workspace, size_t workspace_bytes,
                            int N, int H, int W, int Ci, int Co, int accumulate_bias, hipStream_t s);
 
+size_t mrdis_wgrad16_narrow_workspace(int N, int H, int W, int Ci, int Co);
+int mrdis_run_wgrad16_narrow(const float* x, int ldx, const float* dy, int lddy, float* dw_tck, float* dbias, void* workspace, size_t workspace_bytes,
+                             int N, int H, int W, int Ci, int Co, hipStream_t s);
+
 int mrdis_run_co4(const void* x, int ldx, const float* w, const float* bias, float* y, int ldy, int N, int H, int W, int Ci, int Co, int flip, int lrelu, hipStream_t s,
                   int x_bf16 = 0, int wld = 4);
 
 int mrdis_run_c16(const float* x, int ldx, const float* w_tck, const float* bias, float* y, int ldy, int N, int H, int W, int Ci, int Co, int lrelu, hipStream_t s);
 int mrdis_run_c16t_split6(const float* x, int ldx, const float* w_t_ci_co, float* y, int ldy, int N, int H, int W, int flip, hipStream_t s);
+int mrdis_run_c16_narrow(const float* x, int ldx, const float* w_tck, const float* bias, float* y, int ldy, int N, int H, int W, int Ci, int Co, hipStream_t s);
diff --git a/representation-disentanglement_amd/csrc/mrdis_wgrad16.hip b/representation-disentanglement_amd/csrc/mrdis_wgrad16.hip
--- a/representation-disentanglement_amd/csrc/mrdis_wgrad16.hip
+++ b/representation-disentanglement_amd/csrc/mrdis_wgrad16.hip
@@ -140,15 +140,17 @@
     int N, H, W, ldx, lddy;
     int tilesA, tilesB, numTiles, splits;
     unsigned x_bytes, dy_bytes;
+    int Co;
 };
 #define W6_TH 8
 #define W6_TW 32
 #define W6_YW (W6_TW + 2)
 #define W6_YPX ((W6_TH + 2) * W6_YW)
+template <bool NARROW>
 __global__ __launch_bounds__(256, 2) void wgrad16_split6_kernel(const Wgrad16SParams p) {
     constexpr int XPX = W6_TH * W6_TW;
     constexpr int XPLANE = XPX * 64, YPLANE = W6_YPX * 32;
-    constexpr int XR = 8, YR = 6;
+    constexpr int XR = 8, YR = NARROW ? 11 : 6;
     constexpr unsigned OOB = 0xfffffff0u;
     extern __shared__ __attribute__((aligned(16))) unsigned char smem6[];
     unsigned char* xs = smem6;
@@ -166,8 +168,16 @@
 #pragma unroll
     for (int t = 0; t < 9; ++t) { acc[t][0] = f32x4{0.f, 0.f, 0.f, 0.f}; acc[t][1] = f32x4{0.f, 0.f, 0.f, 0.f}; }
     float bs4[4] = {0.f, 0.f, 0.f, 0.f};
-
-    u32x4 xr[XR], yr[YR];
+    const int npp = NARROW ? 256 / p.Co : 0;
+    const int n_px = NARROW ? tid / p.Co : 0, n_c = NARROW ? tid - n_px * p.Co : 0;
+    const bool n_on = NARROW && n_px < npp;
+
+    u32x4 xr[XR], yr[NARROW ? 1 : YR];
+    unsigned yn[NARROW ? YR : 1];
+    if constexpr (NARROW) {
+        for (int i = tid; i < 3 * YPLANE / 16; i += 256) *reinterpret_cast<u32x4*>(ys + 16 * i) = u32x4{0u, 0u, 0u, 0u};
+        __syncthreads();
+    }
     auto load_box = [&](int box) {
         const bool on = box < p.numTiles;
         int tt = box;
@@ -182,6 +192,16 @@
             const bool ok = on && h < p.H && w_ < p.W;
             xr[it] = __builtin_amdgcn_raw_buffer_load_b128(rs_x, (int)(ok ? 4u * (unsigned)(((n * p.H + h) * p.W + w_) * p.ldx + 4 * q) : OOB), 0, 0);
         }
+        if constexpr (NARROW) {
+#pragma unroll
+            for (int it = 0; it < YR; ++it) {
+                const int px = it * npp + n_px;
+                const int ly = px / W6_YW, lx = px - ly * W6_YW;
+                const int h = a0 - 1 + ly, w_ = b0 - 1 + lx;
+                const bool ok = on && n_on && px < W6_YPX && (unsigned)h < (unsigned)p.H && (unsigned)w_ < (unsigned)p.W;
+                yn[it] = __builtin_amdgcn_raw_buffer_load_b32(rs_y, (int)(ok ? 4u * (unsigned)(((n * p.H + h) * p.W + w_) * p.lddy + n_c) : OOB), 0, 0);
+            }
+        } else {
 #pragma unroll
         for (int it = 0; it < YR; ++it) {
             const int idx = tid + 256 * it, px = idx >> 2, q = idx & 3;
@@ -190,6 +210,7 @@
             const bool ok = on && px < W6_YPX && (unsigned)h < (unsigned)p.H && (unsigned)w_ < (unsigned)p.W;
             yr[it] = __builtin_amdgcn_raw_buffer_load_b128(rs_y, (int)(ok ? 4u * (unsigned)(((n * p.H + h) * p.W + w_) * p.lddy + 4 * q) : OOB), 0, 0);
         }
+        }
     };
     auto split4 = [](const u32x4& v, bf16x4& hi, bf16x4& mid, bf16x4& lo) {
         const float f[4] = {__uint_as_float(v.x), __uint_as_float(v.y), __uint_as_float(v.z), __uint_as_float(v.w)};
@@ -203,6 +224,19 @@
             unsigned char* d = xs + px * 64 + 8 * q;
             *reinterpret_cast<bf16x4*>(d) = hi; *reinterpret_cast<bf16x4*>(d + XPLANE) = mid; *reinterpret_cast<bf16x4*>(d + 2 * XPLANE) = lo;
         }
+        if constexpr (NARROW) {
+#pragma unroll
+            for (int it = 0; it < YR; ++it) {
+                const int px = it * npp + n_px;
+                if (!n_on || px >= W6_YPX) continue;
+                const int ly = px / W6_YW, lx = px - ly * W6_YW;
+                const float v = __uint_as_float(yn[it]);
+                if (ly >= 1 && ly <= W6_TH && lx >= 1 && lx <= W6_TW) bs4[0] += v;
+                __bf16 hi, mid, lo; mrdis_split3(v, hi, mid, lo);
+                unsigned char* d = ys + px * 32 + 2 * n_c;
+                *reinterpret_cast<__bf16*>(d) = hi; *reinterpret_cast<__bf16*>(d + YPLANE) = mid; *reinterpret_cast<__bf16*>(d + 2 * YPLANE) = lo;
+            }
+        } else {
 #pragma unroll
         for (int it = 0; it < YR; ++it) {
             const int idx = tid + 256 * it, px = idx >> 2, q = idx & 3;
@@ -214,6 +248,7 @@
             bf16x4 hi, mid, lo; split4(yr[it], hi, mid, lo);
             unsigned char* d = ys + px * 32 + 8 * q;
             *reinterpret_cast<bf16x4*>(d) = hi; *reinterpret_cast<bf16x4*>(d + YPLANE) = mid; *reinterpret_cast<bf16x4*>(d + 2 * YPLANE) = lo;
+        }
         }
     };
     int box = split;
@@ -281,6 +316,15 @@
     }
     if (p.bias_slab != nullptr) {
         __syncthreads();
+        if constexpr (NARROW) {
+            red[tid] = bs4[0];
+            __syncthreads();
+            if (tid < p.Co) {
+                float t_ = 0.f;
+                for (int k = tid; k < npp * p.Co; k += p.Co) t_ += red[k];
+                p.bias_slab[(long long)split * 16 + tid] = t_;
+            }
+        } else {
 #pragma unroll
         for (int c = 0; c < 4; ++c) red[c * 256 + tid] = bs4[c];
         __syncthreads();
@@ -289,6 +333,7 @@
             float t_ = 0.f;
             for (int k = qd; k < 256; k += 4) t_ += red[c * 256 + k];
             p.bias_slab[(long long)split * 16 + tid] = t_;
+        }
         }
     }
 }
@@ -488,9 +533,9 @@
             q.numTiles = (int)nt6; q.splits = p.splits < q.numTiles ? p.splits : q.numTiles;
             q.x_bytes = (unsigned)xb; q.dy_bytes = (unsigned)yb;
             const size_t lds6 = 3 * (size_t)(W6_TH * W6_TW * 64) + 3 * (size_t)(W6_YPX * 32);
-            if (!mrdis_lds_optin((const void*)wgrad16_split6_kernel, 96 * 1024)) return MRDIS_ELAUNCH;
+            if (!mrdis_lds_optin((const void*)wgrad16_split6_kernel<false>, 96 * 1024)) return MRDIS_ELAUNCH;
             mrdis_count(MRDIS_CNT_SPLIT6_WGRAD16);
-            MRDIS_LAUNCH(wgrad16_split6_kernel, dim3(q.splits), dim3(256), lds6, s, q);
+            MRDIS_LAUNCH(wgrad16_split6_kernel<false>, dim3(q.splits), dim3(256), lds6, s, q);
             MRDIS_CHECK_LAUNCH();
             const long long nout6 = 9LL * Ci * Co + (dbias ? Co : 0);
             int SL6 = 1;
@@ -540,3 +585,47 @@
     MRDIS_CHECK_LAUNCH();
     return MRDIS_OK;
 }
+
+static bool plan_wgrad16_narrow(Wgrad16SParams& q, int N, int H, int W, int Ci, int Co) {
+    if (Ci != 32 || Co < 1 || Co > 8) return false;
+    if ((long long)N * H * W < 65536 || mrdis_opt(MRDIS_OPT_NOW16) || mrdis_opt(MRDIS_OPT_SPLIT6) != 1) return false;
+    q = Wgrad16SParams{};
+    q.N = N; q.H = H; q.W = W; q.Co = Co;
+    q.tilesA = mrdis_cdiv(H, W6_TH); q.tilesB = mrdis_cdiv(W, W6_TW);
+    const long long nt = (long long)N * q.tilesA * q.tilesB;
+    if (nt > 0x7fffffffLL) return false;
+    q.numTiles = (int)nt;
+    q.splits = q.numTiles < 512 ? q.numTiles : 512;
+    return true;
+}
+
+size_t mrdis_wgrad16_narrow_workspace(int N, int H, int W, int Ci, int Co) {
+    Wgrad16SParams q;
+    if (!plan_wgrad16_narrow(q, N, H, W, Ci, Co)) return 0;
+    return sizeof(float) * ((size_t)q.splits * 2 * 9 * 256 + (size_t)q.splits * 16) + 256;
+}
+
+int mrdis_run_wgrad16_narrow(const float* x, int ldx, const float* dy, int lddy, float* dw_tck, float* dbias, void* workspace, size_t workspace_bytes,
+                             int N, int H, int W, int Ci, int Co, hipStream_t s) {
+    Wgrad16SParams q;
+    if (!plan_wgrad16_narrow(q, N, H, W, Ci, Co)) return MRDIS_EUNSUPPORTED;
+    if (ldx % 4 != 0 || ldx < Ci || lddy < Co || (((uintptr_t)x) & 15) != 0 || (((uintptr_t)dy) & 3) != 0) return MRDIS_EUNSUPPORTED;
+    if (workspace_bytes < mrdis_wgrad16_narrow_workspace(N, H, W, Ci, Co)) return MRDIS_EWORKSPACE;
+    const long long xb = 4LL * (((long long)N * H * W - 1) * ldx + Ci), yb = 4LL * (((long long)N * H * W - 1) * lddy + Co);
+    if (xb >= 0x7fffffffLL || yb >= 0x7fffffffLL) return MRDIS_EUNSUPPORTED;
+    q.x = x; q.dy = dy; q.ldx = ldx; q.lddy = lddy;
+    q.slab = reinterpret_cast<float*>(workspace);
+    q.bias_slab = dbias ? q.slab + (size_t)q.splits * 2 * 9 * 256 : nullptr;
+    q.x_bytes = (unsigned)xb; q.dy_bytes = (unsigned)yb;
+    const size_t lds6 = 3 * (size_t)(W6_TH * W6_TW * 64) + 3 * (size_t)(W6_YPX * 32);
+    if (!mrdis_lds_optin((const void*)wgrad16_split6_kernel<true>, 96 * 1024)) return MRDIS_ELAUNCH;
+    mrdis_count(MRDIS_CNT_SPLIT6_WGRAD16);
+    MRDIS_LAUNCH(wgrad16_split6_kernel<true>, dim3(q.splits), dim3(256), lds6, s, q);
+    MRDIS_CHECK_LAUNCH();
+    const long long nout = 9LL * Ci * Co + (dbias ? Co : 0);
+    int SL = 1;
+    while (SL < 16 && SL * 8 <= q.splits) SL <<= 1;
+    MRDIS_LAUNCH(wgrad16_reduce_kernel, dim3(mrdis_cdiv(nout, 64)), dim3(64, SL), 0, s, q.slab, dw_tck, Ci, Co, 2, q.splits, q.bias_slab, dbias, 0);
+    MRDIS_CHECK_LAUNCH();
+    return MRDIS_OK;
+}
diff --git a/representation-disentanglement_amd/headfold.py b/representation-disentanglement_amd/headfold.py
--- /dev/null
+++ b/representation-disentanglement_amd/headfold.py
@@ -0,0 +1,102 @@
+import torch
+
+from . import hip
+
+HEAD_MAXG = 8
+
+
+def head_fold_applies(N, H, W, Ci, Cm, Co):
+    return bool(hip.load().mrdis_head_fold_applies(int(N), int(H), int(W), int(Ci), int(Cm), int(Co)))
+
+
+def head_compose_floats(Ci, Co):
+    return int(hip.load().mrdis_head_compose_floats(int(Ci), int(Co)))
+
+
+def _head_filters(what, w3s, w1s, b3, b1=None):
+    G = len(w3s)
+    if not 1 <= G <= HEAD_MAXG or len(w1s) != G: hip._refuse(what, 'arg', G, len(w1s))
+    T, Ci, Cm = w3s[0].shape
+    Co = w1s[0].shape[2]
+    dev = w3s[0].device
+    for a, b in zip(w3s, w1s):
+        if (a.dtype is not torch.float32 or b.dtype is not torch.float32 or tuple(a.shape) != (9, Ci, Cm) or tuple(b.shape) != (1, Cm, Co)
+                or not (a.is_contiguous() and b.is_contiguous()) or a.device != dev or b.device != dev): hip._refuse(what, 'filter dtype dense', a, b)
+    for v, n in ((b3, Cm), (b1, Co)):
+        if v is not None and (v.dtype is not torch.float32 or tuple(v.shape) != (n,) or not v.is_contiguous() or v.device != dev): hip._refuse(what, 'vec dtype', v)
+    if not (Ci <= 64 and Cm <= 64 and 1 <= Co <= 8): hip._refuse(what, 'arg', Ci, Cm, Co)
+    return G, Ci, Cm, Co
+
+
+def head_compose_fwd(w3s, w1s, b3, b1):
+    G, Ci, Cm, Co = _head_filters('head_compose_fwd', w3s, w1s, b3, b1)
+    out = torch.empty((G, head_compose_floats(Ci, Co)), dtype=torch.float32, device=w3s[0].device)
+    hip._chk(hip.load().mrdis_head_compose_fwd(hip._ptr_array(w3s), hip._ptr_array(w1s), hip._ptr(b3), hip._ptr(b1), hip._ptr(out), G, Ci, Cm, Co, hip._stream()), 'head_compose_fwd')
+    return out
+
+
+def head_compose_views(out, g, Ci, Co):
+    n = 9 * Ci * Co
+    row = out[g]
+    return row[:n].view(9, Ci, Co), row[n:2 * n].view(9, Co, Ci), row[2 * n:2 * n + Co]
+
+
+def head_compose_bwd(dout, w3s, w1s, b3, db3_sink=None, db1_sink=None, need_bias=True):
+    G, Ci, Cm, Co = _head_filters('head_compose_bwd', w3s, w1s, b3)
+    dev = w3s[0].device
+    if dout.dtype is not torch.float32 or tuple(dout.shape) != (G, head_compose_floats(Ci, Co)) or not dout.is_contiguous() or dout.device != dev: hip._refuse('head_compose_bwd', 'vec dtype dense', dout)
+    sinks = db3_sink is not None and db1_sink is not None
+    if sinks and (db3_sink.numel() != Cm or db1_sink.numel() != Co or not (db3_sink.is_contiguous() and db1_sink.is_contiguous())
+                  or db3_sink.dtype is not torch.float32 or db1_sink.dtype is not torch.float32): hip._refuse('head_compose_bwd', 'vec dtype dense', db3_sink, db1_sink)
+    dw3 = torch.empty((G, 9, Ci, Cm), dtype=torch.float32, device=dev)
+    dw1 = torch.empty((G, 1, Cm, Co), dtype=torch.float32, device=dev)
+    db3 = db1 = None
+    if need_bias and not sinks:
+        db3 = torch.empty(Cm, dtype=torch.float32, device=dev); db1 = torch.empty(Co, dtype=torch.float32, device=dev)
+    hip._chk(hip.load().mrdis_head_compose_bwd(hip._ptr(dout), hip._ptr_array(w3s), hip._ptr_array(w1s), hip._ptr(b3), hip._ptr(dw3), hip._ptr(dw1),
+                                       hip._ptr(db3_sink if sinks else db3), hip._ptr(db1_sink if sinks else db1), 1 if sinks else 0, G, Ci, Cm, Co, hip._stream()), 'head_compose_bwd')
+    return dw3, dw1, db3, db1
+
+
+def _head_views(what, wide, narrow, Ci, Co):
+    wv, ldw = hip.nhwc(wide)
+    nv, ldn = hip.nhwc(narrow)
+    N, C, H, W = wv.shape
+    if (wv.dtype is not torch.float32 or nv.dtype is not torch.float32 or C != Ci or tuple(nv.shape) != (N, Co, H, W) or wv.device != nv.device
+            or ldw % 4 != 0 or wv.data_ptr() % 16 != 0): hip._refuse(what, 'like dtype dense', wide, narrow)
+    return wv, ldw, nv, ldn, N, H, W
+
+
+def head_conv_fwd(x, w_tck, bias, out=None):
+    T, Ci, Co = w_tck.shape
+    if out is None:
+        out = hip.empty_nhwc(x.shape[0], Co, x.shape[2], x.shape[3], x.device)
+    xv, ldx, y, ldy, N, H, W = _head_views('head_conv_fwd', x, out, Ci, Co)
+    if y is not out or T != 9 or not w_tck.is_contiguous() or (bias is not None and bias.numel() < Co): hip._refuse('head_conv_fwd', 'filter out vec', out, w_tck, bias)
+    hip._chk(hip.load().mrdis_head_conv_fwd(hip._ptr(xv), ldx, hip._ptr(w_tck), hip._ptr(bias), hip._ptr(y), ldy, N, H, W, Ci, Co, hip._stream()), 'head_conv_fwd')
+    return out
+
+
+def head_conv_bwd_data(dy, w_tkc, out=None):
+    T, Co, Ci = w_tkc.shape
+    if out is None:
+        out = hip.empty_nhwc(dy.shape[0], Ci, dy.shape[2], dy.shape[3], dy.device)
+    dx, lddx, dyv, lddy, N, H, W = _head_views('head_conv_bwd_data', out, dy, Ci, Co)
+    if dx is not out or T != 9 or not w_tkc.is_contiguous(): hip._refuse('head_conv_bwd_data', 'filter out', out, w_tkc)
+    hip._chk(hip.load().mrdis_head_conv_bwd_data(hip._ptr(dyv), lddy, hip._ptr(w_tkc), hip._ptr(dx), lddx, N, H, W, Ci, Co, hip._stream()), 'head_conv_bwd_data')
+    return out
+
+
+def head_conv_bwd_weight(x, dy, dw_out=None, db_out=None, need_bias=True):
+    Ci, Co = x.shape[1], dy.shape[1]
+    xv, ldx, dyv, lddy, N, H, W = _head_views('head_conv_bwd_weight', x, dy, Ci, Co)
+    dw = dw_out if dw_out is not None else torch.empty((9, Ci, Co), dtype=torch.float32, device=x.device)
+    db = (db_out if db_out is not None else torch.empty(Co, dtype=torch.float32, device=x.device)) if need_bias else None
+    if (tuple(dw.shape) != (9, Ci, Co) or not dw.is_contiguous() or dw.dtype is not torch.float32
+            or (db is not None and (db.numel() != Co or not db.is_contiguous() or db.dtype is not torch.float32))): hip._refuse('head_conv_bwd_weight', 'out vec dtype dense', dw, db)
+    nb = hip._ws_bytes(hip.load().mrdis_head_conv_bwd_weight_workspace, N, H, W, Ci, Co)
+    if nb == 0:
+        raise hip.MrdisError('head_conv_bwd_weight: unsupported geometry')
+    ws = hip._ws(nb, x.device)
+    hip._chk(hip.load().mrdis_head_conv_bwd_weight(hip._ptr(xv), ldx, hip._ptr(dyv), lddy, hip._ptr(dw), hip._ptr(db), hip._ptr(ws), nb, N, H, W, Ci, Co, hip._stream()), 'head_conv_bwd_weight')
+    return dw, db
diff --git a/representation-disentanglement_amd/hip.py b/representation-disentanglement_amd/hip.py
--- a/representation-disentanglement_amd/hip.py
+++ b/representation-disentanglement_amd/hip.py
@@ -150,6 +150,14 @@
     'mrdis_prep_stats': (_I, [_P, _I, _L, _L, _L] + [_I] * 9 + [_c.c_double, _c.c_double, _P, _P, _Z, _P]),
     'mrdis_prep_write': (_I, [_P, _I, _L, _L, _L] + [_I] * 7 + [_c.c_double, _c.c_double, _P, _I, _I, _P, _P]),
     'mrdis_export_volume': (_I, [_P] + [_I] * 11 + [_P, _c.c_double, _P, _I, _P]),
+    'mrdis_head_fold_applies': (_I, [_I] * 6),
+    'mrdis_head_compose_floats': (_L, [_I, _I]),
+    'mrdis_head_compose_fwd': (_I, [_P, _P, _P, _P, _P, _I, _I, _I, _I, _P]),
+    'mrdis_head_compose_bwd': (_I, [_P, _P, _P, _P, _P, _P, _P, _P, _I, _I, _I, _I, _I, _P]),
+    'mrdis_head_conv_fwd': (_I, [_P, _I, _P, _P, _P, _I, _I, _I, _I, _I, _I, _P]),
+    'mrdis_head_conv_bwd_data': (_I, [_P, _I, _P, _P, _I, _I, _I, _I, _I, _I, _P]),
+    'mrdis_head_conv_bwd_weight_workspace': (_Z, [_I] * 5),
+    'mrdis_head_conv_bwd_weight': (_I, [_P, _I, _P, _I, _P, _P, _P, _Z, _I, _I, _I, _I, _I, _P]),
 }
 EXPORTED_SYMBOLS = tuple(_SIGS)
 
@@ -221,10 +229,11 @@
 LESION_FAMILIES = ('dilate', 'lesmatch', 'lesexpand')
 PREP_FAMILIES = ('prepstats', 'prepwrite')
 EXPORT_FAMILIES = ('export',)
+HEAD_FAMILIES = ('head_dgrad', 'head_compose')
 ELEM_FAMILIES = ('stat_vec', 'stat_scalar', 'stat_interp', 'spade_up2_onepass', 'spade_up2_twopass', 'bil_fwd_x2', 'bil_fwd_general',
                  'bil_bwd_x2', 'bil_bwd_tight3', 'bil_bwd_tight5', 'bil_bwd_general', 'elem_v1')
 LAUNCH_COUNTERS = (WINO_FAMILIES + VARIANT_FAMILIES + LATENT_FAMILIES + OUTDEC_FAMILIES + CONV3D_FAMILIES + DATA_FAMILIES + PATCH_FAMILIES + WARP_FAMILIES + LOSS3D_FAMILIES + SEGVOL_FAMILIES
-                    + SYNTH_FAMILIES + SEG2D_FAMILIES + FUSE_FAMILIES + SURFDIST_FAMILIES + CC_FAMILIES + PREP_FAMILIES + EXPORT_FAMILIES + LESION_FAMILIES)
+                    + SYNTH_FAMILIES + SEG2D_FAMILIES + FUSE_FAMILIES + SURFDIST_FAMILIES + CC_FAMILIES + PREP_FAMILIES + EXPORT_FAMILIES + LESION_FAMILIES + HEAD_FAMILIES)
 ALL_COUNTERS = LAUNCH_COUNTERS + ELEM_FAMILIES
 SYNTH_MAX_SRC = 8
 SEG2D_MAX_SETS = 16
diff --git a/representation-disentanglement_amd/model.py b/representation-disentanglement_amd/model.py
--- a/representation-disentanglement_amd/model.py
+++ b/representation-disentanglement_amd/model.py
@@ -367,6 +367,12 @@
         return ops.step_cache((id(self), 'gb', inputs_type.data_ptr(), inputs_type._version), fused)
 
     def forward(self, si, zi, inputs_type=None):
+        mix = self.modulated(si, zi, inputs_type)
+        if _groups(inputs_type):
+            return self.out(mix, inputs_type)
+        return self.out(mix, inputs_type) if self.is_cond else self.out(mix)
+
+    def modulated(self, si, zi, inputs_type=None):
         size = self.input_size
         src = si
         si = ops.step_cache(('bil', id(src), size), lambda: (src, ops.bilinear(src, size, False)))[1]
@@ -376,8 +382,7 @@
             si_out = ops.conv2d_grouped(si, [self.si_layers.mixed_uniform(t) for t in inputs_type], self.si_layers.bias, kh, kw, pad, share_x=True,
                                         co=self.si_layers.out_channels)
             fused = [self._fused_gb(t) for t in inputs_type]
-            mix = ops.gb_spade(si_out, zi, [f[0] for f in fused], fused[0][1], self.zi_layers.eps)
-            return self.out(mix, inputs_type)
+            return ops.gb_spade(si_out, zi, [f[0] for f in fused], fused[0][1], self.zi_layers.eps)
         t = (inputs_type,) if self.is_cond else ()
         si_out = self.si_layers(si, *t)
         if self.is_cond and (si_out.shape[0] == 1 or inputs_type.stride(0) == 0):
@@ -392,7 +397,7 @@
             gamma = self.gamma(si_out, *t)
             beta = self.beta(si_out, *t)
             mix = ops.instnorm_spade(zi, gamma, beta, self.zi_layers.eps)
-        return self.out(mix, *t)
+        return mix
 
 
 def _up2(x, norm=None):
@@ -442,9 +447,29 @@
     def forward(self, si, zi_sp4_input, inputs_type=None):
         x = self.sp4(si, zi_sp4_input, inputs_type)
         x = self.sp5(si, _up2(x, self.sp5.zi_layers), inputs_type)
-        x = self.sp6(si, _up2(x, self.sp6.zi_layers), inputs_type)
+        z = _up2(x, self.sp6.zi_layers)
+        if self._head_fold_ready(z, inputs_type):
+            mix = self.sp6.modulated(si, z, inputs_type)
+            labels = list(inputs_type) if _groups(inputs_type) else [inputs_type]
+            f3 = [self.sp6.out.mixed_uniform(t)[0] for t in labels]
+            f1 = [self.out.mixed_uniform(t)[0] for t in labels]
+            if ops.head_fold_applies(mix, len(labels), f3[0].shape[2], f1[0].shape[2]) and f3[0].shape[1] == mix.shape[1] and f1[0].shape[1] == f3[0].shape[2]:
+                return self.out_act(ops.head_fold(mix, f3, f1, self.sp6.out.bias, self.out.bias))
+            x = self.sp6.out(mix, inputs_type)
+        else:
+            x = self.sp6(si, z, inputs_type)
         x = self.out(x, inputs_type) if self.is_cond else self.out(x)
         return self.out_act(x)
+
+    def _head_fold_ready(self, z, inputs_type):
+        a, b = self.sp6.out, self.out
+        if not (ops._HEAD_FOLD and self.is_cond and ops.mix_cache_active() and torch.is_grad_enabled() and not ops.storage_bf16() and z.is_cuda):
+            return False
+        if not (a.kernel_size == (3, 3) and a.stride == (1, 1) and a.padding == (1, 1) and b.kernel_size == (1, 1) and b.stride == (1, 1) and b.padding == (0, 0)):
+            return False
+        if (a.bias is None) != (b.bias is None):
+            return False
+        return bool(_groups(inputs_type)) or (inputs_type is not None and (z.shape[0] == 1 or inputs_type.stride(0) == 0))
 
     def grouped_ok(self):
         blocks = (self.sp4, self.sp5, self.sp6)
@@ -477,6 +502,7 @@
 
     head = SPADENewShared.forward
     tail = SPADENewNotShared.forward
+    _head_fold_ready = SPADENewNotShared._head_fold_ready
 
     def forward(self, si, zi, inputs_type=None):
         return self.tail(si, self.head(si, zi, inputs_type), inputs_type)
diff --git a/representation-disentanglement_amd/ops.py b/representation-disentanglement_amd/ops.py
--- a/representation-disentanglement_amd/ops.py
+++ b/representation-disentanglement_amd/ops.py
@@ -6,6 +6,7 @@
 from torch.autograd import Function
 
 from . import hip
+from . import headfold
 
 
 class _MixExperts(Function):
@@ -889,6 +890,81 @@
     return mix
 
 
+_HEAD_FOLD = _os.environ.get('MRDIS_HEAD_FOLD', '1') != '0'
+
+
+def set_head_fold(enabled):
+    global _HEAD_FOLD
+    _HEAD_FOLD = bool(enabled)
+
+
+def head_fold_applies(mix, G, Cm, Co):
+    if not (_HEAD_FOLD and _COMPUTE_DTYPE == hip.DT_F32 and _MIX_CACHE is not None and torch.is_grad_enabled()):
+        return False
+    if type(mix) is not torch.Tensor or not mix.is_cuda or mix.dtype != torch.float32 or mix.dim() != 4 or mix.shape[0] % G or not 1 <= G <= headfold.HEAD_MAXG:
+        return False
+    return headfold.head_fold_applies(mix.shape[0] // G, mix.shape[2], mix.shape[3], mix.shape[1], Cm, Co)
+
+
+class _HeadFoldFn(Function):
+
+    @staticmethod
+    def forward(ctx, x, b3, b1, G, *filt):
+        w3s, w1s = list(filt[0::2]), list(filt[1::2])
+        B = x.shape[0] // G
+        Ci, Co = w3s[0].shape[1], w1s[0].shape[2]
+        comp = headfold.head_compose_fwd(w3s, w1s, b3, b1)
+        y = hip.empty_nhwc(G * B, Co, x.shape[2], x.shape[3], x.device)
+        for g in range(G):
+            w_tck, _, bias = headfold.head_compose_views(comp, g, Ci, Co)
+            headfold.head_conv_fwd(x[g * B:(g + 1) * B], w_tck, bias, out=y[g * B:(g + 1) * B])
+        ctx.meta = (G, B, Ci, Co)
+        ctx.dx_in_gb = bool(getattr(x, '_mrdis_want_dgb', False)) and _GB_INPLACE
+        ctx.biases = (b3, b1)
+        ctx.save_for_backward(x, comp, *filt)
+        return y
+
+    @staticmethod
+    def backward(ctx, dy):
+        G, B, Ci, Co = ctx.meta
+        x, comp = ctx.saved_tensors[:2]
+        filt = ctx.saved_tensors[2:]
+        w3s, w1s = list(filt[0::2]), list(filt[1::2])
+        b3, b1 = ctx.biases
+        H, W = x.shape[2], x.shape[3]
+        dxb = None
+        if ctx.needs_input_grad[0]:
+            if ctx.dx_in_gb:
+                gbuf = hip.empty_nhwc(G * B, 2 * Ci, H, W, x.device, x.dtype)
+                gbuf._mrdis_gb_private = True
+                dxb = gbuf[:, Ci:]
+            else:
+                dxb = hip.empty_nhwc(G * B, Ci, H, W, x.device, x.dtype)
+        dcomp = torch.empty_like(comp)
+        for g in range(G):
+            sl = slice(g * B, (g + 1) * B)
+            if dxb is not None:
+                headfold.head_conv_bwd_data(dy[sl], headfold.head_compose_views(comp, g, Ci, Co)[1], out=dxb[sl])
+            dw, _, db = headfold.head_compose_views(dcomp, g, Ci, Co)
+            headfold.head_conv_bwd_weight(x[sl], dy[sl], dw_out=dw, db_out=db, need_bias=True)
+        s3, s1 = _grad_sink(b3), _grad_sink(b1)
+        sinks = s3 is not None and s1 is not None
+        dw3, dw1, db3, db1 = headfold.head_compose_bwd(dcomp, w3s, w1s, b3, db3_sink=s3 if sinks else None, db1_sink=s1 if sinks else None,
+                                                       need_bias=b3 is not None or b1 is not None)
+        db3, db1 = (db3 if b3 is not None else None), (db1 if b1 is not None else None)
+        dws = []
+        for g in range(G):
+            dws += [dw3[g], dw1[g]]
+        return (dxb, db3, db1, None) + tuple(dws)
+
+
+def head_fold(x, filters3, filters1, b3, b1):
+    flat = []
+    for a, b in zip(filters3, filters1):
+        flat += [a, b]
+    return _HeadFoldFn.apply(x, b3, b1, len(filters3), *flat)
+
+
 def conv2d_grouped(x, filters, bias, kh, kw, pad, lrelu=False, share_x=False, co=None, stride=1):
     flat = []
     for a, b in filters:
```

After: 237.2. 0.954x the previous value.
